# alexfrom0815/IR-BPP

Hardware: AMD Instinct MI355X
Metric: env steps/sec (placements/sec) across N parallel bins (higher is better)
Workload: dtype f64

## Files before the change

include/irbpp.h:

```cpp
#ifndef IRBPP_H
#define IRBPP_H

#include <stdint.h>

#ifdef __cplusplus
extern "C" {
#endif

typedef struct irbpp_env irbpp_env;

typedef enum {
    IRBPP_OK = 0,
    IRBPP_ERR_ARG = -1,
    IRBPP_ERR_HIP = -2,
    IRBPP_ERR_STATE = -3,
    IRBPP_ERR_DEVICE = -4,
    IRBPP_ERR_NOMEM = -5
} irbpp_status;

typedef struct {
    int32_t num_bins;
    int32_t n_rot;
    int32_t selected;
    int32_t buffer_size;
    double  resolution_a;
    double  resolution_h;
    double  resolution_z;
    double  bin[3];
    double  scale_z;
    int32_t traj_start;
    int32_t global_offset;
    int32_t global_bins;
    int32_t device;
    int32_t stability;
    int32_t tuning;
    int32_t item_stream;
} irbpp_config;

#define IRBPP_TUNE_NO_BLOCK_PATH  1
#define IRBPP_TUNE_WIDE_KERNEL    2
#define IRBPP_TUNE_NARROW_KERNEL  4
#define IRBPP_TUNE_NO_BOX_PATH    8
#define IRBPP_TUNE_NO_ITEM_ORDER 16
#define IRBPP_TUNE_TRACE_CPW64   32
#define IRBPP_TUNE_TRACE_CPW32   64
#define IRBPP_TUNE_TRACE_CPW16  128
#define IRBPP_TUNE_INLINE_POLYGON 256
#define IRBPP_TUNE_NO_HEAVY_FIRST 512
#define IRBPP_TUNE_FUSED_APPLY 2048
#define IRBPP_TUNE_SPLIT_APPLY 4096
#define IRBPP_TUNE_BLOCK_EMIT 8192
#define IRBPP_TUNE_WAVE_EMIT 16384
#define IRBPP_TUNE_GRAPH 32768
#define IRBPP_TUNE_WG512 65536
#define IRBPP_TUNE_NO_WG512 131072
#define IRBPP_TUNE_TRACE_REFILL 262144
#define IRBPP_TUNE_NO_MIXED_PATH 524288
#define IRBPP_TUNE_CHAIN 1048576
#define IRBPP_TUNE_WG128 2097152
#define IRBPP_TUNE_RECT 4194304
#define IRBPP_TUNE_NO_SPECIALISED 1024

typedef struct {
    double*  reward_dev;
    uint8_t* done_dev;
    int32_t* counter_dev;
    double*  ratio_dev;
    double*  ep_reward_dev;
    int32_t* ep_len_dev;
    uint8_t* stable_dev;
    int32_t* err_dev;
} irbpp_step_out;

const char* irbpp_status_string(int status);
int irbpp_version(void);
const char* irbpp_source_hash(void);

int irbpp_create(const irbpp_config* cfg, irbpp_env** out);
int irbpp_destroy(irbpp_env* env);

int irbpp_load_shapes(irbpp_env* env, int32_t n_shapes,
                      const double* extents, const double* volumes,
                      const int32_t* dims, const int64_t* offsets, int64_t pool_len,
                      const double* height_top, const double* height_bottom,
                      const double* mask_top, const double* mask_bottom);

int irbpp_load_sequences(irbpp_env* env, const int32_t* ids, int32_t n_traj, int32_t length);

int irbpp_obs_len(const irbpp_env* env, int32_t which);

int irbpp_reset(irbpp_env* env, float* obs_dev, void* stream);

int irbpp_reset_bins(irbpp_env* env, const int32_t* bins_dev, int32_t count, float* obs_dev, void* stream);

int irbpp_step(irbpp_env* env, const int32_t* actions_dev, float* obs_dev,
               const irbpp_step_out* out, void* stream);

int irbpp_step_cells(irbpp_env* env, const int32_t* cells_dev, float* obs_dev,
                     const irbpp_step_out* out, void* stream);

int irbpp_heuristic_step(irbpp_env* env, int32_t method, int32_t dir_idx, float* obs_dev,
                         const irbpp_step_out* out, void* stream);

int irbpp_get_action_candidates(irbpp_env* env, const int32_t* order_actions_dev,
                                float* loc_obs_dev, void* stream);

int irbpp_get_all_possible_observation(irbpp_env* env, float* loc_obs_dev, void* stream);

int irbpp_policy_minz(irbpp_env* env, const float* loc_obs_dev, int32_t obs_stride,
                      int32_t* actions_dev, void* stream);

int irbpp_set_auto_policy(irbpp_env* env, int32_t* actions_dev);

int irbpp_register_obs_buffer(irbpp_env* env, float* obs_dev);
int irbpp_unregister_obs_buffer(irbpp_env* env, float* obs_dev);
int irbpp_invalidate_obs_buffer(irbpp_env* env, float* obs_dev, void* stream);

int irbpp_stream_cursors(irbpp_env* env, int32_t* cursors_dev, int32_t set, void* stream);
int irbpp_stream_write(irbpp_env* env, const int32_t* ids_dev, const int32_t* first_dev, const int32_t* count_dev,
                       int32_t width, void* stream);

typedef struct irbpp_itemgen irbpp_itemgen;
int irbpp_itemgen_create(uint32_t seed, int32_t n_groups, const int32_t* group_offsets, const int32_t* members,
                         int32_t n_members, irbpp_itemgen** out);
int irbpp_itemgen_draw(irbpp_itemgen* gen, int32_t count, int32_t* out_host);
int irbpp_itemgen_destroy(irbpp_itemgen* gen);


int irbpp_possible_position(irbpp_env* env, const int32_t* item_ids_dev,
                            double* posz_dev, uint8_t* mask_dev, void* stream);

int irbpp_heuristic_action(irbpp_env* env, int32_t method, int32_t dir_idx, int32_t* out_dev, void* stream);

int irbpp_shot_item(const double* verts_dev, const int32_t* faces_dev, int32_t n_faces, int32_t fx, int32_t fy,
                    double resolution_h, double shift, double extent_z, double* top_dev, double* bottom_dev,
                    double* mask_top_dev, double* mask_bottom_dev, int32_t* scratch_dev, void* stream);

int irbpp_convex_hull_actions(irbpp_env* env, int32_t n_grids, const double* posz_valid_dev,
                              const uint8_t* mask_dev, uint32_t* vertex_rows_dev, void* stream);

int irbpp_get_heightmaps(irbpp_env* env, double* hm_dev, void* stream);
int irbpp_set_heightmaps(irbpp_env* env, const double* hm_dev, void* stream);

int irbpp_episode_totals(irbpp_env* env, double* out_dev, void* stream);

typedef struct {
    int64_t key;
    double  r;
    double  ratio;
    int32_t counter;
    int32_t reserved;
} irbpp_episode_entry;
typedef struct {
    irbpp_episode_entry* ring_dev;
    irbpp_episode_entry* snapshot_dev;
    int32_t* rows_dev;
    int32_t* state_dev;
    int32_t window;
    int32_t history;
} irbpp_episode_window;
int irbpp_set_episode_window(irbpp_env* env, const irbpp_episode_window* window);
int irbpp_episode_metrics(const irbpp_episode_window* parts, int32_t n_parts, int32_t first_step, int32_t n_steps,
                          double* out_dev, void* stream);

int irbpp_set_placement_log(irbpp_env* env, uint32_t* meta_dev, double* z_dev, int32_t capacity);

int irbpp_sumtree_find(const float* tree_dev, int32_t n_env, int32_t capacity, const float* values_dev, int32_t draws,
                       float* prob_dev, int64_t* data_idx_dev, int64_t* tree_idx_dev, void* stream);
int irbpp_sumtree_sample(const float* tree_dev, const int64_t* index_dev, int32_t n_env, int32_t capacity, int32_t draws,
                         int32_t n_step, uint64_t seed, int32_t max_tries, float* prob_dev, int64_t* data_idx_dev,
                         int64_t* tree_idx_dev, int32_t* failed_dev, void* stream);

int irbpp_sumtree_update(float* tree_dev, float* max_dev, int32_t n_env, int32_t capacity, const int64_t* tree_idx_dev,
                         const float* priority_dev, int32_t leaves, const uint8_t* env_mask_dev, void* stream);
typedef struct {
    const float* states_dev; const int64_t* actions_dev; const float* rewards_dev; const uint8_t* nonterminals_dev;
    const float* tree_dev; const int64_t* index_dev; const uint8_t* full_dev; const float* scaling_dev;
    int32_t n_env, capacity, obs_len, n_step;
} irbpp_replay_view;
int irbpp_replay_gather(const irbpp_replay_view* view, int32_t draws, float beta, const int64_t* data_idx_dev,
                        const float* prob_dev, float* state_dev, int64_t* action_dev, float* return_dev,
                        float* next_state_dev, float* nonterminal_dev, float* weight_dev, void* stream);
typedef struct {
    float* states_dev; int64_t* actions_dev; float* rewards_dev; uint8_t* nonterminals_dev; int32_t* timesteps_dev;
    float* tree_dev; float* max_dev; int64_t* index_dev; uint8_t* full_dev; int32_t* t_dev;
    int32_t n_env, capacity, obs_len;
} irbpp_replay_store;
int irbpp_replay_append(const irbpp_replay_store* store, const float* state_dev, int64_t state_stride, const void* action_dev,
                        int32_t action_bytes, const void* reward_dev, int32_t reward_bytes, const uint8_t* terminal_dev,
                        const uint8_t* valid_dev, void* stream);
int irbpp_masked_argmax(const float* q_dev, int32_t q_stride, const float* obs_dev, int32_t obs_stride, int32_t selected,
                        int32_t n_env, int64_t* action_dev, void* stream);

int irbpp_debug_phase_cycles(irbpp_env* env, int64_t* cycles_dev);

int irbpp_debug_kernel_info(const irbpp_env* env, int32_t* lds_bytes, const char** kernel_name);
int irbpp_overlap_path(const irbpp_env* env);
int irbpp_debug_kernel_timing(irbpp_env* env, int32_t capacity);
int irbpp_debug_kernel_timing_every(irbpp_env* env, int32_t every);
int irbpp_debug_kernel_times(irbpp_env* env, float* ms_host, int32_t max_count, int32_t* count);

int irbpp_device_error(irbpp_env* env, void* stream, int32_t* flags_out);

#define IRBPP_DEVERR_LEVEL_RANGE   1
#define IRBPP_DEVERR_TRACE_GUARD   2
#define IRBPP_DEVERR_BAD_ITEM      4
#define IRBPP_DEVERR_BAD_BIN       8
#define IRBPP_DEVERR_CAPACITY     16
#define IRBPP_DEVERR_BAD_ACTION   64
#define IRBPP_DEVERR_STREAM_DRY   32

#ifdef __cplusplus
}
#endif
// ... 2 lines not shown
```

irbpp_amd/_lib.py:

```python
from __future__ import annotations

import ctypes as C
import os

from .build import LIB_PATH

c_i32_p = C.POINTER(C.c_int32)
c_f64_p = C.POINTER(C.c_double)


class IrbppConfig(C.Structure):
    _fields_ = [
        ("num_bins", C.c_int32), ("n_rot", C.c_int32), ("selected", C.c_int32), ("buffer_size", C.c_int32),
        ("resolution_a", C.c_double), ("resolution_h", C.c_double), ("resolution_z", C.c_double),
        ("bin", C.c_double * 3), ("scale_z", C.c_double),
        ("traj_start", C.c_int32), ("global_offset", C.c_int32), ("global_bins", C.c_int32),
        ("device", C.c_int32), ("stability", C.c_int32), ("tuning", C.c_int32), ("item_stream", C.c_int32),
    ]


TUNE_NO_BLOCK_PATH, TUNE_WIDE_KERNEL, TUNE_NARROW_KERNEL, TUNE_NO_BOX_PATH, TUNE_NO_ITEM_ORDER = 1, 2, 4, 8, 16
TUNE_TRACE_CPW64, TUNE_TRACE_CPW32, TUNE_TRACE_CPW16, TUNE_INLINE_POLYGON, TUNE_NO_HEAVY_FIRST = 32, 64, 128, 256, 512
TUNE_NO_SPECIALISED, TUNE_FUSED_APPLY, TUNE_SPLIT_APPLY, TUNE_BLOCK_EMIT, TUNE_WAVE_EMIT = 1024, 2048, 4096, 8192, 16384
TUNE_GRAPH, TUNE_WG512, TUNE_NO_WG512, TUNE_TRACE_REFILL, TUNE_NO_MIXED_PATH = 32768, 65536, 131072, 262144, 524288
TUNE_CHAIN, TUNE_WG128, TUNE_RECT = 1048576, 2097152, 4194304


class IrbppReplayView(C.Structure):
    _fields_ = [("states_dev", C.c_void_p), ("actions_dev", C.c_void_p), ("rewards_dev", C.c_void_p),
                ("nonterminals_dev", C.c_void_p), ("tree_dev", C.c_void_p), ("index_dev", C.c_void_p),
                ("full_dev", C.c_void_p), ("scaling_dev", C.c_void_p),
                ("n_env", C.c_int32), ("capacity", C.c_int32), ("obs_len", C.c_int32), ("n_step", C.c_int32)]


class IrbppReplayStore(C.Structure):
    _fields_ = [("states_dev", C.c_void_p), ("actions_dev", C.c_void_p), ("rewards_dev", C.c_void_p),
                ("nonterminals_dev", C.c_void_p), ("timesteps_dev", C.c_void_p), ("tree_dev", C.c_void_p),
                ("max_dev", C.c_void_p), ("index_dev", C.c_void_p), ("full_dev", C.c_void_p), ("t_dev", C.c_void_p),
                ("n_env", C.c_int32), ("capacity", C.c_int32), ("obs_len", C.c_int32)]


class IrbppEpisodeWindow(C.Structure):
    _fields_ = [("ring_dev", C.c_void_p), ("snapshot_dev", C.c_void_p), ("rows_dev", C.c_void_p), ("state_dev", C.c_void_p),
                ("window", C.c_int32), ("history", C.c_int32)]


class IrbppStepOut(C.Structure):
    _fields_ = [("reward_dev", C.c_void_p), ("done_dev", C.c_void_p), ("counter_dev", C.c_void_p),
                ("ratio_dev", C.c_void_p), ("ep_reward_dev", C.c_void_p), ("ep_len_dev", C.c_void_p),
                ("stable_dev", C.c_void_p), ("err_dev", C.c_void_p)]


SIGNATURES = {
    "irbpp_status_string": (C.c_char_p, [C.c_int]),
    "irbpp_version": (C.c_int, []),
    "irbpp_source_hash": (C.c_char_p, []),
    "irbpp_overlap_path": (C.c_int, [C.c_void_p]),
    "irbpp_create": (C.c_int, [C.POINTER(IrbppConfig), C.POINTER(C.c_void_p)]),
    "irbpp_destroy": (C.c_int, [C.c_void_p]),
    "irbpp_load_shapes": (C.c_int, [C.c_void_p, C.c_int32, c_f64_p, c_f64_p, c_i32_p, C.POINTER(C.c_int64),
                                    C.c_int64, c_f64_p, c_f64_p, c_f64_p, c_f64_p]),
    "irbpp_load_sequences": (C.c_int, [C.c_void_p, c_i32_p, C.c_int32, C.c_int32]),
    "irbpp_obs_len": (C.c_int, [C.c_void_p, C.c_int32]),
    "irbpp_reset": (C.c_int, [C.c_void_p, C.c_void_p, C.c_void_p]),
    "irbpp_reset_bins": (C.c_int, [C.c_void_p, C.c_void_p, C.c_int32, C.c_void_p, C.c_void_p]),
    "irbpp_step": (C.c_int, [C.c_void_p, C.c_void_p, C.c_void_p, C.POINTER(IrbppStepOut), C.c_void_p]),
    "irbpp_step_cells": (C.c_int, [C.c_void_p, C.c_void_p, C.c_void_p, C.POINTER(IrbppStepOut), C.c_void_p]),
    "irbpp_heuristic_step": (C.c_int, [C.c_void_p, C.c_int32, C.c_int32, C.c_void_p, C.POINTER(IrbppStepOut), C.c_void_p]),
    "irbpp_get_action_candidates": (C.c_int, [C.c_void_p, C.c_void_p, C.c_void_p, C.c_void_p]),
    "irbpp_get_all_possible_observation": (C.c_int, [C.c_void_p, C.c_void_p, C.c_void_p]),
    "irbpp_policy_minz": (C.c_int, [C.c_void_p, C.c_void_p, C.c_int32, C.c_void_p, C.c_void_p]),
    "irbpp_set_auto_policy": (C.c_int, [C.c_void_p, C.c_void_p]),
    "irbpp_register_obs_buffer": (C.c_int, [C.c_void_p, C.c_void_p]),
    "irbpp_unregister_obs_buffer": (C.c_int, [C.c_void_p, C.c_void_p]),
    "irbpp_invalidate_obs_buffer": (C.c_int, [C.c_void_p, C.c_void_p, C.c_void_p]),
    "irbpp_stream_cursors": (C.c_int, [C.c_void_p, C.c_void_p, C.c_int32, C.c_void_p]),
    "irbpp_stream_write": (C.c_int, [C.c_void_p, C.c_void_p, C.c_void_p, C.c_void_p, C.c_int32, C.c_void_p]),
    "irbpp_itemgen_create": (C.c_int, [C.c_uint32, C.c_int32, c_i32_p, c_i32_p, C.c_int32, C.POINTER(C.c_void_p)]),
    "irbpp_itemgen_draw": (C.c_int, [C.c_void_p, C.c_int32, c_i32_p]),
    "irbpp_itemgen_destroy": (C.c_int, [C.c_void_p]),
    "irbpp_possible_position": (C.c_int, [C.c_void_p, C.c_void_p, C.c_void_p, C.c_void_p, C.c_void_p]),
    "irbpp_heuristic_action": (C.c_int, [C.c_void_p, C.c_int32, C.c_int32, C.c_void_p, C.c_void_p]),
    "irbpp_shot_item": (C.c_int, [C.c_void_p, C.c_void_p, C.c_int32, C.c_int32, C.c_int32, C.c_double, C.c_double,
                                  C.c_double, C.c_void_p, C.c_void_p, C.c_void_p, C.c_void_p, C.c_void_p, C.c_void_p]),
    "irbpp_convex_hull_actions": (C.c_int, [C.c_void_p, C.c_int32, C.c_void_p, C.c_void_p, C.c_void_p, C.c_void_p]),
    "irbpp_get_heightmaps": (C.c_int, [C.c_void_p, C.c_void_p, C.c_void_p]),
    "irbpp_set_heightmaps": (C.c_int, [C.c_void_p, C.c_void_p, C.c_void_p]),
    "irbpp_episode_totals": (C.c_int, [C.c_void_p, C.c_void_p, C.c_void_p]),
    "irbpp_set_placement_log": (C.c_int, [C.c_void_p, C.c_void_p, C.c_void_p, C.c_int32]),
    "irbpp_set_episode_window": (C.c_int, [C.c_void_p, C.POINTER(IrbppEpisodeWindow)]),
    "irbpp_episode_metrics": (C.c_int, [C.POINTER(IrbppEpisodeWindow), C.c_int32, C.c_int32, C.c_int32, C.c_void_p, C.c_void_p]),
    "irbpp_sumtree_sample": (C.c_int, [C.c_void_p, C.c_void_p, C.c_int32, C.c_int32, C.c_int32, C.c_int32, C.c_uint64, C.c_int32,
                                       C.c_void_p, C.c_void_p, C.c_void_p, C.c_void_p, C.c_void_p]),
    "irbpp_sumtree_find": (C.c_int, [C.c_void_p, C.c_int32, C.c_int32, C.c_void_p, C.c_int32, C.c_void_p, C.c_void_p,
                                     C.c_void_p, C.c_void_p]),
    "irbpp_sumtree_update": (C.c_int, [C.c_void_p, C.c_void_p, C.c_int32, C.c_int32, C.c_void_p, C.c_void_p, C.c_int32,
                                       C.c_void_p, C.c_void_p]),
    "irbpp_replay_gather": (C.c_int, [C.POINTER(IrbppReplayView), C.c_int32, C.c_float, C.c_void_p, C.c_void_p, C.c_void_p,
                                      C.c_void_p, C.c_void_p, C.c_void_p, C.c_void_p, C.c_void_p, C.c_void_p]),
    "irbpp_replay_append": (C.c_int, [C.POINTER(IrbppReplayStore), C.c_void_p, C.c_int64, C.c_void_p, C.c_int32, C.c_void_p,
                                      C.c_int32, C.c_void_p, C.c_void_p, C.c_void_p]),
    "irbpp_masked_argmax": (C.c_int, [C.c_void_p, C.c_int32, C.c_void_p, C.c_int32, C.c_int32, C.c_int32, C.c_void_p,
                                      C.c_void_p]),
    "irbpp_debug_phase_cycles": (C.c_int, [C.c_void_p, C.c_void_p]),
    "irbpp_debug_kernel_info": (C.c_int, [C.c_void_p, C.POINTER(C.c_int32), C.POINTER(C.c_char_p)]),
    "irbpp_debug_kernel_timing": (C.c_int, [C.c_void_p, C.c_int32]),
    "irbpp_debug_kernel_timing_every": (C.c_int, [C.c_void_p, C.c_int32]),
    "irbpp_debug_kernel_times": (C.c_int, [C.c_void_p, C.POINTER(C.c_float), C.c_int32, C.POINTER(C.c_int32)]),
    "irbpp_device_error": (C.c_int, [C.c_void_p, C.c_void_p, c_i32_p]),
}

_lib = None


def load(path: str = "") -> C.CDLL:
    global _lib
    if _lib is not None:
        return _lib
    explicit = bool(path) or bool(os.environ.get("IRBPP_LIBRARY"))
    path = path or os.environ.get("IRBPP_LIBRARY", "") or LIB_PATH
    if not os.path.exists(path):
        raise RuntimeError(
            f"{path} not found: build it with `python -c 'import __graft_entry__ as g; g.build()'` "
            "(hipcc --offload-arch=gfx950). irbpp_amd has no CPU fallback.")
    import torch
    lib = C.CDLL(path)
    for name, (res, args) in SIGNATURES.items():
        fn = getattr(lib, name)
        fn.restype = res
        fn.argtypes = args
    if not explicit and not os.environ.get("IRBPP_ALLOW_STALE_LIBRARY"):
        from . import build
        have = lib.irbpp_source_hash().decode()
        try:
            want = build.source_hash()
        except OSError:
            want = have
        if have != want:
            raise RuntimeError(
                f"{path} was built from sources {have}, the sources in {build.CSRC} hash to {want}: rebuild with "
                "`python -c 'import __graft_entry__ as g; g.build()'` (IRBPP_ALLOW_STALE_LIBRARY=1 overrides)")
    _lib = lib
    return lib


class IrbppError(RuntimeError):
    pass


DEVERR_BITS = {1: "LEVEL_RANGE", 2: "TRACE_GUARD", 4: "BAD_ITEM", 8: "BAD_BIN", 16: "CAPACITY", 32: "STREAM_DRY", 64: "BAD_ACTION"}


def deverr_names(flags: int) -> str:
    return "|".join(name for bit, name in DEVERR_BITS.items() if flags & bit) or "0"


def check(status: int, what: str = "") -> None:
    if status != 0:
        msg = load().irbpp_status_string(status).decode()
        raise IrbppError(f"{what}: {msg} (status {status})")
```

irbpp_amd/build.py:

```python
from __future__ import annotations

import os
import shutil
import subprocess

PKG_DIR = os.path.dirname(os.path.abspath(__file__))
CSRC = os.path.join(PKG_DIR, "csrc")
LIB_PATH = os.path.join(PKG_DIR, "libirbpp_hip.so")
SOURCES = ["irbpp_capi.hip", "irbpp_kernels.hip", "irbpp_wide.hip", "irbpp_replay.hip", "irbpp_metrics.hip", "irbpp_metrics.h", "irbpp_device.h", "contours_device.h", "irbpp_itemgen.h",
           os.path.join("..", "..", "include", "irbpp.h")]
HIPCC_FLAGS = ["--offload-arch=gfx950", "-O3", "-std=c++17", "-ffp-contract=off", "-fno-honor-nans",
               "-shared", "-fPIC", "-Wno-unused-value"]


def source_hash() -> str:
    import hashlib
    h = hashlib.sha256(" ".join(HIPCC_FLAGS).encode())
    for name in sorted(SOURCES):
        with open(os.path.join(CSRC, name), "rb") as f:
            h.update(f.read())
    return h.hexdigest()[:16]


def _hipcc() -> str:
    for cand in (shutil.which("hipcc"), "/opt/rocm/bin/hipcc"):
        if cand and os.path.exists(cand):
            return cand
    raise RuntimeError("hipcc not found: the HIP library cannot be built on this machine")


def built_hash(path: str = LIB_PATH) -> str:
    try:
        with open(path, "rb") as f:
            blob = f.read()
    except OSError:
        return ""
    i = blob.find(b"irbpp-source-hash:")
    return blob[i + 18:i + 34].decode("ascii", "replace") if i >= 0 else ""


def needs_build(path: str = LIB_PATH) -> bool:
    return built_hash(path) != source_hash()


def build(force: bool = False, verbose: bool = False) -> str:
    out = LIB_PATH
    if not force and not needs_build(out):
        return out
    cmd = [_hipcc()] + HIPCC_FLAGS + [f'-DIRBPP_SOURCE_HASH="{source_hash()}"', os.path.join(CSRC, "irbpp_capi.hip"), "-o", out]
    if verbose:
        print(" ".join(cmd))
    res = subprocess.run(cmd, capture_output=True, text=True)
    if res.returncode != 0:
        raise RuntimeError("hipcc failed:\n" + res.stdout + res.stderr)
    from . import asmcheck
    try:
        chk = asmcheck.check_library(out)
    except (RuntimeError, OSError, subprocess.CalledProcessError) as e:
        if verbose:
            print(f"asmcheck skipped: {e}")
        return out
    if verbose:
        print(f"asmcheck: {chk['scalar_loads']} scalar loads in {chk['functions']} kernels, {len(chk['problems'])} hazards")
    if chk["problems"]:
        os.replace(out, out + ".rejected")
        raise RuntimeError("scalar-load hazard in the built library (kept as " + out + ".rejected):\n" + "\n".join(chk["problems"]))
    return out
```

irbpp_amd/csrc/irbpp_capi.hip:

```cpp
#include <hip/hip_runtime.h>
#include <math.h>
#include <stdint.h>
#include <stdio.h>
#include <stdlib.h>
#include <string.h>

#include <new>
#include <utility>
#include <vector>

#include "../../include/irbpp.h"
#include "irbpp_device.h"
#include "irbpp_kernels.hip"
#include "irbpp_wide.hip"
#include "irbpp_replay.hip"
#include "irbpp_metrics.hip"
#include "irbpp_itemgen.h"

using namespace irbpp;

struct irbpp_env {
    irbpp_config cfg;
    Params P;
    Tables T;
    State S;
    bool shapes_loaded = false, seq_loaded = false, was_reset = false;
    bool item_order = false;
    long long* phase_cycles = nullptr;
    int32_t* auto_actions = nullptr;
    int heavy_turn = 0;
    int32_t* err_mirror = nullptr;
    std::vector<std::pair<const float*, int32_t*>> obs_buffers;
    std::vector<hipEvent_t> timing;
    size_t timing_next = 0, timing_used = 0;
    int timing_every = 1, timing_phase = 0;
    std::vector<void*> allocs;
    char kernel_names[256] = {0};
    struct GraphEntry { std::vector<uint8_t> key; hipGraphExec_t exec; hipGraph_t graph; uint64_t used; };
    std::vector<GraphEntry> graphs;
    hipStream_t cap_stream = nullptr;
    uint64_t graph_clock = 0, graph_replays = 0;
    int obs_epoch = 0;
    irbpp_episode_window window{};
    int32_t* heur_cells = nullptr;
    bool grids_current = false;
};

#define HIP_TRY(expr)                                   \
    do {                                                \
        hipError_t _e = (expr);                         \
        if (_e != hipSuccess) return IRBPP_ERR_HIP;     \
    } while (0)

namespace {

template <typename T>
int dev_alloc(irbpp_env* env, T** out, size_t count) {
    void* p = nullptr;
    if (hipMalloc(&p, count * sizeof(T) > 0 ? count * sizeof(T) : sizeof(T)) != hipSuccess) return IRBPP_ERR_NOMEM;
    if (hipMemset(p, 0, count * sizeof(T)) != hipSuccess) { hipFree(p); return IRBPP_ERR_HIP; }
    env->allocs.push_back(p);
    *out = (T*)p;
    return IRBPP_OK;
}

template <typename T>
int dev_upload(irbpp_env* env, const T** out, const T* host, size_t count) {
    T* p = nullptr;
    int rc = dev_alloc(env, &p, count);
    if (rc != IRBPP_OK) return rc;
    if (count && hipMemcpy(p, host, count * sizeof(T), hipMemcpyHostToDevice) != hipSuccess) return IRBPP_ERR_HIP;
    *out = p;
    return IRBPP_OK;
}

inline double round6_host(double x) { return nearbyint(x * 1e6) / 1e6; }
constexpr int TRACE_SMALL_GRID = 8192;
constexpr int TRACE_CPW16_BINS = 0;
constexpr int TRACE_CPW32_BINS = 1024;
void layout_lds_host(Params& P) {
    int pad = 0;
#ifdef IRBPP_ABLATE
    if (const char* e = getenv("IRBPP_LDS_PAD")) pad = atoi(e);
#endif
    irbpp::layout_lds(P, pad);
}

int raise_lds_limits() {
    const void* kernels[] = {(const void*)irbpp_env_kernel_wide, (const void*)irbpp_env_kernel, (const void*)irbpp_env_kernel_box,
                             (const void*)irbpp_env_kernel_box8, (const void*)irbpp_env_kernel_generic,
                             (const void*)irbpp_env_kernel_generic8, (const void*)irbpp_env_kernel_mixed8, (const void*)irbpp_hull_kernel,
                             (const void*)irbpp_env_kernel_chain, (const void*)irbpp_wide_kernel,
#if !defined(IRBPP_NO_SPEC)
                             (const void*)irbpp_env_kernel_s1, (const void*)irbpp_env_kernel_s2, (const void*)irbpp_env_kernel_s3,
                             (const void*)irbpp_env_kernel_s4, (const void*)irbpp_env_kernel_s5, (const void*)irbpp_emit_kernel_s5,
                             (const void*)irbpp_env_kernel_chain_s1, (const void*)wg128::irbpp_env_kernel_s1_w128,
                             (const void*)irbpp_emit_kernel_s1, (const void*)irbpp_emit_kernel_s2,
                             (const void*)irbpp_emit_kernel_s3, (const void*)irbpp_emit_kernel_s4,
                             (const void*)irbpp_emit_wave_kernel_s1, (const void*)irbpp_emit_wave_kernel_s2, (const void*)irbpp_emit_wave_kernel_s5,
                             (const void*)wg512::irbpp_env_kernel_s4_w512, (const void*)wg512::irbpp_env_kernel_s4_w512c,
#endif
                             (const void*)wg512::irbpp_env_kernel_generic_w512,
                             (const void*)irbpp_emit_wave_kernel,
                             (const void*)irbpp_emit_kernel, (const void*)irbpp_heuristic_kernel};
    for (const void* k : kernels)
        if (hipFuncSetAttribute(k, hipFuncAttributeMaxDynamicSharedMemorySize, 160 * 1024) != hipSuccess) return IRBPP_ERR_HIP;
    return IRBPP_OK;
}

}

static int chain_extra_lds(const Params& P) {
    int npad = 64;
    while (npad < P.S) npad <<= 1;
    return align16(10 * npad > 1024 ? 10 * npad : 1024);
}
static bool all_block(const Params& P) { return P.block_b > 0 && P.block_rots == (1 << P.R) - 1; }
static bool lattice_or_box(const Params& P) { return all_block(P) || P.box != 0; }
static bool lattice_images(const Params& P) { return P.block_b > 0 || P.box != 0; }

static int trace_grid_cap(int N) {
    const int small = 4 * N < TRACE_SMALL_GRID ? 4 * N : TRACE_SMALL_GRID;
    return N > small ? N : small;
}

extern "C" {

const char* irbpp_status_string(int status) {
    switch (status) {
        case IRBPP_OK: return "ok";
        case IRBPP_ERR_ARG: return "bad argument or unsupported configuration";
        case IRBPP_ERR_HIP: return "HIP runtime error";
        case IRBPP_ERR_STATE: return "call out of order (load shapes and sequences, reset, then step)";
        case IRBPP_ERR_DEVICE: return "device-side error word set";
        case IRBPP_ERR_NOMEM: return "out of device memory";
        default: return "unknown status";
    }
}

int irbpp_version(void) { return 600; }

#ifndef IRBPP_SOURCE_HASH
#define IRBPP_SOURCE_HASH "unstamped"
#endif
const char* irbpp_source_hash(void) { static const char stamp[] = "irbpp-source-hash:" IRBPP_SOURCE_HASH; return stamp + 18; }

int irbpp_create(const irbpp_config* cfg, irbpp_env** out) {
    if (!cfg || !out) return IRBPP_ERR_ARG;
    if (cfg->num_bins > MAX_BINS) return IRBPP_ERR_ARG;
    if (cfg->num_bins < 1 || cfg->n_rot < 1 || cfg->n_rot > 8 || cfg->selected < 1 || cfg->selected > 1024 ||
        cfg->buffer_size < 1 || cfg->buffer_size > 16)
        return IRBPP_ERR_ARG;
    if (!(cfg->resolution_a > 0) || !(cfg->resolution_h > 0) || !(cfg->resolution_z > 0)) return IRBPP_ERR_ARG;
    irbpp_env* env = new (std::nothrow) irbpp_env();
    if (!env) return IRBPP_ERR_NOMEM;
    env->cfg = *cfg;
    memset(&env->T, 0, sizeof(Tables));
    memset(&env->S, 0, sizeof(State));
    Params& P = env->P;
    memset(&P, 0, sizeof(Params));
    P.N = cfg->num_bins;
    P.R = cfg->n_rot;
    P.S = cfg->selected;
    P.K = cfg->buffer_size;
    P.res_a = cfg->resolution_a;
    P.res_h = cfg->resolution_h;
    P.res_z = cfg->resolution_z;
    P.inv_res_z = 1.0 / cfg->resolution_z;
    for (int k = 0; k < 32; ++k) P.txs[k] = round6_host((double)k * cfg->resolution_a);
    P.bin_x = cfg->bin[0];
    P.bin_y = cfg->bin[1];
    P.bin_z = cfg->bin[2];
    P.bin_vol = cfg->bin[0] * cfg->bin[1] * cfg->bin[2];
    P.scale_z = cfg->scale_z;
    P.ibin_z = round6_host(cfg->bin[2] * cfg->scale_z);
    P.step = (int)(cfg->resolution_a / cfg->resolution_h);
    if ((double)P.step != cfg->resolution_a / cfg->resolution_h || P.step < 1) { delete env; return IRBPP_ERR_ARG; }
    P.Hx = (int)ceil(cfg->bin[0] / cfg->resolution_h);
    P.Hy = (int)ceil(cfg->bin[1] / cfg->resolution_h);
    P.Ax = (int)ceil(cfg->bin[0] / cfg->resolution_a);
    P.Ay = (int)ceil(cfg->bin[1] / cfg->resolution_a);
    P.Hc = P.Hx * P.Hy;
    P.AC = P.Ax * P.Ay;
    if (P.Ax > 32 || P.Ay > 32 || P.Ax < 1 || P.Ay < 1 || P.Hc > 128 * 128) { delete env; return IRBPP_ERR_ARG; }
    const double levels = floor(cfg->bin[2] / cfg->resolution_z + 1e-9);
    if (!(levels <= (double)MAX_LEVELS)) { delete env; return IRBPP_ERR_ARG; }
    const bool deep = levels > (double)TUNED_MAX_LEVELS;
    P.wide = (P.Ax > 16 || P.Ay > 16 || deep) ? 1 : 0;
    P.vrow = P.wide ? WIDE_VROW : 16;
    if (P.wide && (P.Hc > 64 * 64 || cfg->stability != 0)) { delete env; return IRBPP_ERR_ARG; }
    if (P.Hx != P.Ax * P.step || P.Hy != P.Ay * P.step) { delete env; return IRBPP_ERR_ARG; }
    P.traj_start = cfg->traj_start;
    P.goff = cfg->global_offset;
    P.gbins = cfg->global_bins > 0 ? cfg->global_bins : cfg->num_bins;
    P.obs_len1 = 5 * P.S + 9 + P.Hc;
    P.obs_len0 = P.K > 1 ? P.K + P.Hc : P.obs_len1;
#ifdef IRBPP_ABLATE
    if (const char* rep = getenv("IRBPP_DEBUG_REPEAT")) P.dbg_repeat = atoi(rep);
#endif
    P.split = 1;
    P.stability = cfg->stability < 0 ? 0 : (cfg->stability > 2 ? 2 : cfg->stability);
    P.rect = (cfg->tuning & IRBPP_TUNE_RECT) ? 1 : 0;
    P.wimg = P.R * (deep ? (((int)levels + 33 + 31) & ~31) : 64);
    P.seg_cap = P.wide ? 64 : 2 * ((P.N + NXCD - 1) / NXCD) * P.R * P.AC;
    P.round_cap = P.wide ? 16 : (P.N / NXCD + 64) * 16;
    layout_lds_host(P);
    if (P.lds_bytes_full > 160 * 1024 || (P.wide && wide_layout(P).bytes > 160 * 1024)) { delete env; return IRBPP_ERR_ARG; }

    if (hipSetDevice(cfg->device) != hipSuccess) { delete env; return IRBPP_ERR_HIP; }
    if (raise_lds_limits() != IRBPP_OK) { delete env; return IRBPP_ERR_HIP; }
    State& S = env->S;
    const size_t N = (size_t)P.N;
    int rc = IRBPP_OK;
#define ALLOC(field, count) if (rc == IRBPP_OK) rc = dev_alloc(env, &S.field, (count))
    ALLOC(hm, N * P.Hc);
    ALLOC(queue, N * P.K);
    ALLOC(cand, N * P.S);
    ALLOC(bs, N);
    ALLOC(totals, N * 4);
    ALLOC(order, N);
    ALLOC(err, 1);
    ALLOC(w_posz, N * P.R * P.AC);
    ALLOC(w_valid, N * P.R * P.vrow);
    ALLOC(w_vmask, N * P.R * 16);
    ALLOC(w_meta, N * WMETA);
    ALLOC(w_img, P.wide ? 16 : N * P.wimg * 16);
    ALLOC(w_imgrot, P.wide ? 16 : N * P.wimg);
    ALLOC(w_cand, (size_t)NXCD * P.seg_cap);
    ALLOC(w_big, P.wide ? N * wide_scratch_bytes(P) : (size_t)trace_grid_cap(P.N) * TRACE_WAVE_BYTES);
    ALLOC(w_total, NXCD * XCD_STRIDE);
    ALLOC(w_nround, NXCD * XCD_STRIDE);
    ALLOC(w_round, (size_t)NXCD * P.round_cap * ROUND_BYTES);
    P.heavy_cap = P.N >= 64 ? P.N / 8 : 0;
    P.heavy_thr = (P.S * 3) / 5;
    ALLOC(w_heavy, 2 * (size_t)(XCD_STRIDE + P.heavy_cap));
#undef ALLOC
    if (rc == IRBPP_OK) rc = dev_alloc(env, &env->heur_cells, N * 3);
    if (rc != IRBPP_OK) { irbpp_destroy(env); return rc; }
    {
        std::vector<int32_t> ident(N);
        for (size_t i = 0; i < N; ++i) ident[i] = (int32_t)i;
        if (hipMemcpy(S.order, ident.data(), N * sizeof(int32_t), hipMemcpyHostToDevice) != hipSuccess) { irbpp_destroy(env); return IRBPP_ERR_HIP; }
    }
    *out = env;
    return IRBPP_OK;
}

int irbpp_destroy(irbpp_env* env) {
    if (!env) return IRBPP_OK;
// ... 17 lines not shown
    const Params& P = env->P;
    HIP_TRY(hipSetDevice(env->cfg.device));
    const int R = P.R;
    std::vector<ShapeRot> sr((size_t)n_shapes * R);
    std::vector<Cell> bcell, tcell, blkcell;
    std::vector<GCell> gcell;
    for (int64_t i = 0; i < (int64_t)n_shapes * R; ++i) {
        const int64_t fx = dims[i * 2], fy = dims[i * 2 + 1];
        if (fx < 1 || fy < 1 || fx > 4096 || fy > 4096 || offsets[i] < 0 || offsets[i] + fx * fy > pool_len) return IRBPP_ERR_ARG;
    }
    int block_b = 0, block_rots = 0;
    if (!(env->cfg.tuning & IRBPP_TUNE_NO_BLOCK_PATH) && !P.wide) {
        int best_count = 0;
        for (int b = 8; b >= 2; --b) {
            if (b % P.step != 0 || (P.Hx - b) % P.step != 0 || (P.Hy - b) % P.step != 0) continue;
            int mask = 0;
            for (int r = 0; r < R; ++r) {
                bool ok = true;
                for (int64_t k = 0; k < n_shapes && ok; ++k) {
                    const int64_t i = k * R + r;
                    const int fx = dims[i * 2], fy = dims[i * 2 + 1];
                    if (fx % b != 0 || fy % b != 0) { ok = false; break; }
                    for (int ti = 0; ti < fx / b && ok; ++ti)
                        for (int tj = 0; tj < fy / b && ok; ++tj) {
                            const int64_t e0 = offsets[i] + (int64_t)(ti * b) * fy + tj * b;
                            for (int u = 0; u < b && ok; ++u)
                                for (int v = 0; v < b && ok; ++v) {
                                    const int64_t e = offsets[i] + (int64_t)(ti * b + u) * fy + tj * b + v;
                                    if (mask_bottom[e] != mask_bottom[e0] ||
                                        (mask_bottom[e0] != 0.0 && height_bottom[e] != height_bottom[e0]))
                                        ok = false;
                                }
                        }
                }
                if (ok) mask |= 1 << r;
            }
            const int count = __builtin_popcount((unsigned)mask);
            if (count > best_count) { best_count = count; block_b = b; block_rots = mask; }
            if (count == R) break;
        }
        if (block_rots != (1 << R) - 1 && (2 * best_count < R || (env->cfg.tuning & IRBPP_TUNE_NO_MIXED_PATH))) { block_b = 0; block_rots = 0; }
    }
    const bool mixed = block_b > 0 && block_rots != (1 << R) - 1;
    bool box = block_b == 0 && !(env->cfg.tuning & IRBPP_TUNE_NO_BOX_PATH) && !P.wide;
    for (int64_t i = 0; i < (int64_t)n_shapes * R && box; ++i) {
        const int fx = dims[i * 2], fy = dims[i * 2 + 1];
        const double* mb = mask_bottom + offsets[i];
        const double* hb = height_bottom + offsets[i];
        int bx = 0, by = 0;
        while (bx < fx && mb[(int64_t)bx * fy] != 0.0) ++bx;
        while (by < fy && mb[by] != 0.0) ++by;
        if (bx == 0 || by == 0) { box = false; break; }
        for (int ci = 0; ci < fx && box; ++ci)
            for (int cj = 0; cj < fy && box; ++cj) {
                const bool in = ci < bx && cj < by;
                if ((mb[(int64_t)ci * fy + cj] != 0.0) != in || (in && hb[(int64_t)ci * fy + cj] != hb[0])) box = false;
            }
    }
    const int mb_h = block_b ? (P.Hx - block_b) / P.step + 1 : 0, mb_w = block_b ? (P.Hy - block_b) / P.step + 1 : 0;
    for (int k = 0; k < n_shapes; ++k) {
        for (int r = 0; r < R; ++r) {
            const size_t i = (size_t)k * R + r;
            ShapeRot& s = sr[i];
            memset(&s, 0, sizeof(s));
            s.ext_x = extents[i * 3 + 0];
            s.ext_y = extents[i * 3 + 1];
            s.ext_z = extents[i * 3 + 2];
            const double bx = round6_host(s.ext_x), by = round6_host(s.ext_y);
            s.ext_z_r = round6_host(s.ext_z);
            s.fx = (int32_t)ceil(bx / P.res_h);
            s.fy = (int32_t)ceil(by / P.res_h);
            s.ax = (int32_t)ceil(bx / P.res_a);
            s.ay = (int32_t)ceil(by / P.res_a);
            const int64_t off = offsets[i];
            if (s.fx != dims[i * 2] || s.fy != dims[i * 2 + 1]) return IRBPP_ERR_ARG;
            if (s.fx < 1 || s.fy < 1 || s.fx > s.ax * P.step || s.fy > s.ay * P.step) return IRBPP_ERR_ARG;
            if (off < 0 || off + (int64_t)s.fx * s.fy > pool_len) return IRBPP_ERR_ARG;
            s.ob = (int32_t)bcell.size();
            s.ot = (int32_t)tcell.size();
            for (int ci = 0; ci < s.fx; ++ci) {
                for (int cj = 0; cj < s.fy; ++cj) {
                    const int64_t e = off + (int64_t)ci * s.fy + cj;
                    const double mt = mask_top[e], mb = mask_bottom[e];
                    if ((mt != 0.0 && mt != 1.0) || (mb != 0.0 && mb != 1.0)) return IRBPP_ERR_ARG;
                    const int32_t ij = ci | (cj << 16);
                    if (mb != 0.0) bcell.push_back(Cell{height_bottom[e], ij, ci * s.fy + cj});
                    else s.has_out = 1;
                    if (mt != 0.0) tcell.push_back(Cell{height_top[e], ij, ci * s.fy + cj});
                }
            }
            s.nb = (int32_t)bcell.size() - s.ob;
            s.nt = (int32_t)tcell.size() - s.ot;
            {
                double mass = 0.0, mx = 0.0, my = 0.0;
                for (int ci = 0; ci < s.fx; ++ci)
                    for (int cj = 0; cj < s.fy; ++cj) {
                        const int64_t e = off + (int64_t)ci * s.fy + cj;
                        if (mask_top[e] != 0.0 && mask_bottom[e] != 0.0) {
                            const double w = height_top[e] - height_bottom[e] > 0.0 ? height_top[e] - height_bottom[e] : 0.0;
                            mass += w; mx += w * (ci + 0.5); my += w * (cj + 0.5);
                        }
                    }
                s.com_x = mass > 0.0 ? mx / mass : 0.5 * s.fx;
                s.com_y = mass > 0.0 ? my / mass : 0.5 * s.fy;
            }
            s.oblk = (int32_t)blkcell.size();
            if (block_b && ((block_rots >> r) & 1))
                for (int ti = 0; ti < s.fx / block_b; ++ti)
                    for (int tj = 0; tj < s.fy / block_b; ++tj) {
                        const int64_t e0 = off + (int64_t)(ti * block_b) * s.fy + tj * block_b;
                        if (mask_bottom[e0] != 0.0)
                            blkcell.push_back(Cell{height_bottom[e0], (ti * block_b / P.step) * mb_w + tj * block_b / P.step, 0});
                    }
            s.nblk = (int32_t)blkcell.size() - s.oblk;
            if (!box && (!block_b || mixed))
                for (int e = 0; e < s.nb; ++e) {
                    const Cell& c = bcell[s.ob + e];
                    const int ci = c.ij & 0xFFFF, cj = c.ij >> 16;
                    const int off = ((ci % P.step) * P.step + cj % P.step) * P.AC + (ci / P.step) * P.Ay + cj / P.step;
                    gcell.push_back(GCell{c.v, off * 8, 0});
                }
            if (box) {
                while (s.bx < s.fx && mask_bottom[off + (int64_t)s.bx * s.fy] != 0.0) ++s.bx;
                while (s.by < s.fy && mask_bottom[off + s.by] != 0.0) ++s.by;
                s.bc = height_bottom[off];
            }
            if (s.nb == 0 && !s.has_out) return IRBPP_ERR_ARG;
        }
    }
    if (bcell.empty()) bcell.push_back(Cell{0.0, 0, 0});
    if (tcell.empty()) tcell.push_back(Cell{0.0, 0, 0});
    if (blkcell.empty()) blkcell.push_back(Cell{0.0, 0, 0});
    if (gcell.empty()) gcell.push_back(GCell{0.0, 0, 0});
    for (int i = 0; i < 8; ++i) gcell.push_back(GCell{0.0, 0, 0});
    Tables& T = env->T;
    int rc = dev_upload(env, &T.sr, sr.data(), sr.size());
    if (rc == IRBPP_OK) rc = dev_upload(env, &T.bcell, (const Cell*)bcell.data(), bcell.size());
    if (rc == IRBPP_OK) rc = dev_upload(env, &T.tcell, (const Cell*)tcell.data(), tcell.size());
    if (rc == IRBPP_OK) rc = dev_upload(env, &T.blkcell, (const Cell*)blkcell.data(), blkcell.size());
    if (rc == IRBPP_OK) rc = dev_upload(env, &T.gcell, (const GCell*)gcell.data(), gcell.size());
    if (rc == IRBPP_OK) rc = dev_upload(env, &T.volume, volumes, (size_t)n_shapes);
    if (rc != IRBPP_OK) return rc;
    T.n_shapes = n_shapes;
    if (block_b || box) {
        env->P.block_b = block_b;
        env->P.block_rots = block_rots;
        env->P.mb_h = mb_h;
        env->P.mb_w = mb_w;
        env->P.box = box ? 1 : 0;
        layout_lds_host(env->P);
        if (env->P.lds_bytes_full > 160 * 1024) return IRBPP_ERR_ARG;
        if (raise_lds_limits() != IRBPP_OK) return IRBPP_ERR_HIP;
    }
    env->item_order = (!block_b || mixed) && !box && gcell.size() * sizeof(GCell) > (size_t)8 << 20 && env->P.N % NXCD == 0 &&
                      env->P.N >= 64 * NXCD && env->P.K == 1 && !(env->cfg.tuning & IRBPP_TUNE_NO_ITEM_ORDER);
    env->shapes_loaded = true;
    return IRBPP_OK;
}

int irbpp_load_sequences(irbpp_env* env, const int32_t* ids, int32_t n_traj, int32_t length) {
    if (!env || !ids || n_traj < 1 || length < 1) return IRBPP_ERR_ARG;
    if (env->seq_loaded) return IRBPP_ERR_STATE;
    HIP_TRY(hipSetDevice(env->cfg.device));
    int rc = dev_upload(env, &env->T.seq, ids, (size_t)n_traj * length);
    if (rc != IRBPP_OK) return rc;
    env->T.n_traj = n_traj;
    env->T.seq_len = length;
    env->T.stream = env->cfg.item_stream ? 1 : 0;
    env->seq_loaded = true;
    return IRBPP_OK;
}

int irbpp_stream_cursors(irbpp_env* env, int32_t* cursors_dev, int32_t set, void* stream) {
    if (!env || !cursors_dev) return IRBPP_ERR_ARG;
    if (!env->cfg.item_stream || !env->seq_loaded) return IRBPP_ERR_STATE;
    hipLaunchKernelGGL(irbpp_stream_cursor_kernel, dim3((env->P.N + 255) / 256), dim3(256), 0, (hipStream_t)stream, env->S.bs,
                       cursors_dev, env->P.N, set);
    return hipGetLastError() == hipSuccess ? IRBPP_OK : IRBPP_ERR_HIP;
}

int irbpp_stream_write(irbpp_env* env, const int32_t* ids_dev, const int32_t* first_dev, const int32_t* count_dev, int32_t width,
                       void* stream) {
    if (!env || !ids_dev || !first_dev || !count_dev || width < 0) return IRBPP_ERR_ARG;
    if (!env->cfg.item_stream || !env->seq_loaded) return IRBPP_ERR_STATE;
    if (width > env->T.seq_len) return IRBPP_ERR_ARG;
    if (width == 0) return IRBPP_OK;
    env->err_mirror = nullptr;
    const long long n = (long long)env->T.n_traj * width;
    hipLaunchKernelGGL(irbpp_stream_write_kernel, dim3((unsigned)((n + 255) / 256)), dim3(256), 0, (hipStream_t)stream,
                       const_cast<int32_t*>(env->T.seq), env->T.n_traj, env->T.seq_len, ids_dev, first_dev, count_dev, width);
    return hipGetLastError() == hipSuccess ? IRBPP_OK : IRBPP_ERR_HIP;
}

int irbpp_obs_len(const irbpp_env* env, int32_t which) {
    if (!env) return IRBPP_ERR_ARG;
    return which == 0 ? env->P.obs_len0 : env->P.obs_len1;
}

typedef void (*env_kernel_fn)(const Params, const Tables, const State, const StepIO, const int);
struct EnvKernel { env_kernel_fn fn; const char* name; int threads = 256; };
static int pick_spec(const irbpp_env* env) {
#if defined(IRBPP_NO_SPEC) || defined(IRBPP_ABLATE)
    return 0;
#else
    if (env->cfg.tuning & (IRBPP_TUNE_NO_SPECIALISED | IRBPP_TUNE_WIDE_KERNEL | IRBPP_TUNE_NARROW_KERNEL)) return 0;
    static const Params spec[N_SPECS] = {Params{}, spec_params(SPEC_KEYS[1]), spec_params(SPEC_KEYS[2]), spec_params(SPEC_KEYS[3]),
                                         spec_params(SPEC_KEYS[4]), spec_params(SPEC_KEYS[5])};
    static_assert(N_SPECS == 6, "one table entry and one kernel per SPEC_KEYS row");
    for (int i = 1; i < N_SPECS; ++i)
        if (spec_matches(env->P, spec[i])) return i;
    return 0;
#endif
}

static bool split_apply(const irbpp_env* env, int n) {
    if (env->P.stability != 0 || (env->cfg.tuning & IRBPP_TUNE_FUSED_APPLY)) return false;
    if (env->cfg.tuning & IRBPP_TUNE_SPLIT_APPLY) return true;
    if (env->P.K > 1) return true;
    const int per_cu = (160 * 1024) / (env->P.lds_bytes > 0 ? env->P.lds_bytes : 1);
    if (per_cu < 8) return false;
    const bool lists = !lattice_or_box(env->P);
    return n >= (lists ? 4 : 2) * 256 * 8;
}

static EnvKernel pick_env_kernel(const irbpp_env* env) {
    const Params& P = env->P;
    const int t = env->cfg.tuning;
    const bool lds_allows_8 = 8 * P.lds_bytes <= 160 * 1024;
    const bool generic = P.block_b == 0 && !P.box;
    const bool mixed = P.block_b > 0 && !all_block(P);
#if !defined(IRBPP_NO_SPEC) && !defined(IRBPP_ABLATE)
    if (generic && (t & IRBPP_TUNE_NARROW_KERNEL) && (t & IRBPP_TUNE_WG512) && spec_matches(P, spec_params(SPEC_KEYS[4])))
        return {wg512::irbpp_env_kernel_s4_w512c, "irbpp_env_kernel_s4_w512c", 512};
#endif
    const bool wg512 = generic && !(t & (IRBPP_TUNE_NO_WG512 | IRBPP_TUNE_WIDE_KERNEL | IRBPP_TUNE_NARROW_KERNEL)) &&
                       ((t & IRBPP_TUNE_WG512) || 5 * P.lds_bytes > 160 * 1024);
#if !defined(IRBPP_NO_SPEC) && !defined(IRBPP_ABLATE)
    if (wg512 && pick_spec(env) == 4)
        return P.N >= 4096 ? EnvKernel{wg512::irbpp_env_kernel_s4_w512c, "irbpp_env_kernel_s4_w512c", 512}
                           : EnvKernel{wg512::irbpp_env_kernel_s4_w512, "irbpp_env_kernel_s4_w512", 512};
#endif
    if (wg512 && (pick_spec(env) == 0 || (t & IRBPP_TUNE_WG512)))
        return {wg512::irbpp_env_kernel_generic_w512, "irbpp_env_kernel_generic_w512", 512};
#if !defined(IRBPP_NO_SPEC) && !defined(IRBPP_ABLATE)
    if ((t & IRBPP_TUNE_WG128) && pick_spec(env) == 1)
        return {wg128::irbpp_env_kernel_s1_w128, "irbpp_env_kernel_s1_w128", 128};
    switch (pick_spec(env)) {
        case 1: return {irbpp_env_kernel_s1, "irbpp_env_kernel_s1"};
        case 2: return {irbpp_env_kernel_s2, "irbpp_env_kernel_s2"};
        case 3: return {irbpp_env_kernel_s3, "irbpp_env_kernel_s3"};
        case 4: return {irbpp_env_kernel_s4, "irbpp_env_kernel_s4"};
        case 5: return {irbpp_env_kernel_s5, "irbpp_env_kernel_s5"};
        default: break;
    }
#endif
    if (mixed) return (t & IRBPP_TUNE_WIDE_KERNEL) ? EnvKernel{irbpp_env_kernel_wide, "irbpp_env_kernel_wide"} : EnvKernel{irbpp_env_kernel_mixed8, "irbpp_env_kernel_mixed8"};
    if (P.block_b > 0) {
        if ((t & IRBPP_TUNE_WIDE_KERNEL) || 6 * P.lds_bytes > 150 * 1024) return {irbpp_env_kernel_wide, "irbpp_env_kernel_wide"};
        return {irbpp_env_kernel, "irbpp_env_kernel"};
    }
    if (P.box) {
        if (t & IRBPP_TUNE_WIDE_KERNEL) return {irbpp_env_kernel_box, "irbpp_env_kernel_box"};
        if ((t & IRBPP_TUNE_NARROW_KERNEL) || lds_allows_8) return {irbpp_env_kernel_box8, "irbpp_env_kernel_box8"};
        return {irbpp_env_kernel_box, "irbpp_env_kernel_box"};
    }
    if (t & IRBPP_TUNE_WIDE_KERNEL) return {irbpp_env_kernel_generic, "irbpp_env_kernel_generic"};
    if ((t & IRBPP_TUNE_NARROW_KERNEL) || lds_allows_8) return {irbpp_env_kernel_generic8, "irbpp_env_kernel_generic8"};
    return {irbpp_env_kernel_generic, "irbpp_env_kernel_generic"};
}

static int pick_trace_cpw(const irbpp_env* env, int n) {
    const int t = env->cfg.tuning;
    if (t & IRBPP_TUNE_TRACE_CPW64) return 64;
    if (t & IRBPP_TUNE_TRACE_CPW32) return 32;
    if (t & IRBPP_TUNE_TRACE_CPW16) return 16;
    if (t & IRBPP_TUNE_TRACE_REFILL) return TRACE_REFILL_BATCH;
    return n <= TRACE_CPW16_BINS ? 16 : (n <= TRACE_CPW32_BINS ? 32 : 64);
}

static bool chain_launch(const irbpp_env* env, int n) {
    const int t = env->cfg.tuning;
    (void)n;
    if (!(t & IRBPP_TUNE_CHAIN) || env->P.stability != 0) return false;
    if (t & (IRBPP_TUNE_TRACE_CPW64 | IRBPP_TUNE_TRACE_CPW32 | IRBPP_TUNE_TRACE_CPW16 | IRBPP_TUNE_TRACE_REFILL | IRBPP_TUNE_INLINE_POLYGON |
             IRBPP_TUNE_BLOCK_EMIT | IRBPP_TUNE_WAVE_EMIT | IRBPP_TUNE_SPLIT_APPLY | IRBPP_TUNE_GRAPH | IRBPP_TUNE_WG512 | IRBPP_TUNE_NARROW_KERNEL))
        return false;
    if (env->P.lds_bytes > 32 * 1024) return false;
    return true;
}

static void launch_apply(irbpp_env* env, StepIO io, int mode, hipStream_t st, int n, int key) {
    if (key == KEY_HEUR && io.heur_method == 4) {
        StepIO sel = io;
        sel.heur_out = env->heur_cells;
        hipLaunchKernelGGL(irbpp_heuristic_kernel, dim3(env->P.N), dim3(256), env->P.lds_bytes_full, st, env->P, env->T, env->S, sel);
        io.actions = env->heur_cells;
        key = KEY_CELLS;
    }
    const bool wg = env->P.K > 1 && n < 2048;
    env_kernel_fn fn = wg ? irbpp_apply_wg_kernel : irbpp_apply_kernel;
    if (key == KEY_CELLS) fn = wg ? irbpp_apply_cells_wg_kernel : irbpp_apply_cells_kernel;
    if (key == KEY_HEUR) fn = wg ? irbpp_apply_heur_wg_kernel : irbpp_apply_heur_kernel;
    hipLaunchKernelGGL(fn, wg ? dim3(n) : dim3((n + 3) / 4), dim3(256), 0, st, env->P, env->T, env->S, io, mode);
}

static void launch_group(irbpp_env* env, StepIO io, int mode, hipStream_t st, int first, int n, int key = KEY_CAND) {
    io.block_off = first;
    io.n_slots = n;
    io.auto_action = env->auto_actions;
    io.use_order = 0;
    if (mode == MODE_STEP && env->item_order && first == 0 && n == env->P.N) {
        hipLaunchKernelGGL(irbpp_item_order_kernel, dim3(1), dim3(1024), 0, st, env->T, env->S, n);
        io.use_order = 1;
    }
    io.obs_rows = nullptr;
    const bool observes = mode == MODE_CANDS || ((mode == MODE_RESET || mode == MODE_STEP) && env->P.K == 1);
    for (auto& rb : env->obs_buffers)
        if (rb.first == io.obs) {
            if (observes && !(mode == MODE_RESET && io.bin_list != nullptr)) io.obs_rows = rb.second;
            else hipMemsetAsync(rb.second, 0xFF, (size_t)env->P.N * sizeof(int32_t), st);
        }
    if (env->P.wide) {
        int wmode = mode;
        if (mode == MODE_STEP) {
            launch_apply(env, io, mode, st, n, key);
            if (env->P.K > 1) return;
            wmode = MODE_OBSERVE;
        }
        hipLaunchKernelGGL(irbpp_wide_kernel, dim3(n), dim3(256), wide_layout(env->P).bytes, st, env->P, env->T, env->S, io, wmode);
        return;
    }
    const bool chain = observes && mode != MODE_POSSIBLE && chain_launch(env, n);
    const bool split = env->P.split && observes && !chain;
    const bool heavy_first = split && env->P.heavy_cap > 0 && !lattice_images(env->P) && io.bin_list == nullptr &&
                             !(env->cfg.tuning & IRBPP_TUNE_NO_HEAVY_FIRST);
    io.heavy_turn = heavy_first ? env->heavy_turn : -1;
    if (heavy_first) env->heavy_turn ^= 1;
    int env_mode = mode;
    if (chain && !(mode == MODE_STEP && env->P.K > 1)) {
        const bool s1 = pick_spec(env) == 1;
        hipLaunchKernelGGL(s1 ? irbpp_env_kernel_chain_s1 : irbpp_env_kernel_chain, dim3(n), dim3(256), env->P.lds_bytes + chain_extra_lds(env->P), st,
                           env->P, env->T, env->S, io, mode);
        return;
    }
    if (mode == MODE_STEP && (key != KEY_CAND || split_apply(env, n))) {
        launch_apply(env, io, mode, st, n, key);
        env_mode = MODE_OBSERVE;
    }
    if (!(env_mode == MODE_OBSERVE && env->P.K > 1)) {
        const EnvKernel ek = pick_env_kernel(env);
        hipLaunchKernelGGL(ek.fn, dim3(n), dim3(ek.threads), env->P.lds_bytes, st, env->P, env->T, env->S, io, env_mode);
    }
    if (split) {
        const int cpw = pick_trace_cpw(env, n), pgrid = 2 * n;
        const int tune = env->cfg.tuning;
        const bool inline_polygon = (tune & IRBPP_TUNE_INLINE_POLYGON) != 0;
        Params Pt = env->P;
        if (inline_polygon) Pt.round_cap = 0;
        int tgrid = cpw > 64 ? (n * 64 + cpw - 1) / cpw : n * (64 / cpw);
        if (tgrid > trace_grid_cap(env->P.N)) tgrid = trace_grid_cap(env->P.N);
        auto trace_fn = cpw > 64 ? irbpp_trace_kernel_refill : cpw == 64 ? irbpp_trace_kernel : (cpw == 32 ? irbpp_trace_kernel_c32 : irbpp_trace_kernel_c16);
        hipLaunchKernelGGL(trace_fn, dim3(tgrid), dim3(64), 0, st, Pt, env->S, env->phase_cycles);
#ifdef IRBPP_AB_POLY_ACCOUNT
        if (!inline_polygon) hipLaunchKernelGGL(irbpp_polygon_kernel, dim3(pgrid), dim3(64), 0, st, env->P, env->S, env->phase_cycles);
#else
        if (!inline_polygon) hipLaunchKernelGGL(irbpp_polygon_kernel, dim3(pgrid), dim3(64), 0, st, env->P, env->S);
#endif
        const bool wave_emit = lattice_images(env->P) && !heavy_first && !(env->cfg.tuning & IRBPP_TUNE_BLOCK_EMIT) &&
                               (n >= 2048 || (env->cfg.tuning & IRBPP_TUNE_WAVE_EMIT));
        env_kernel_fn emit_fn = wave_emit ? irbpp_emit_wave_kernel : irbpp_emit_kernel;
#if !defined(IRBPP_NO_SPEC) && !defined(IRBPP_ABLATE)
        switch (pick_spec(env)) {
            case 1: emit_fn = wave_emit ? irbpp_emit_wave_kernel_s1 : irbpp_emit_kernel_s1; break;
            case 2: emit_fn = wave_emit ? irbpp_emit_wave_kernel_s2 : irbpp_emit_kernel_s2; break;
            case 3: emit_fn = irbpp_emit_kernel_s3; break;
            case 4: emit_fn = irbpp_emit_kernel_s4; break;
            case 5: emit_fn = wave_emit ? irbpp_emit_wave_kernel_s5 : irbpp_emit_kernel_s5; break;
            default: break;
        }
#endif
        const int egrid = wave_emit ? (n + 3) / 4 : n + (heavy_first ? env->P.heavy_cap : 0);
        hipLaunchKernelGGL(emit_fn, dim3(egrid), dim3(256), env->P.emit_lds_bytes, st, env->P, env->T, env->S, io, mode);
    }
}

constexpr int GRAPH_CACHE = 24;
static void drop_graphs(irbpp_env* env) {
    for (auto& g : env->graphs) { if (g.exec) hipGraphExecDestroy(g.exec); if (g.graph) hipGraphDestroy(g.graph); }
    env->graphs.clear();
}
static bool graph_wanted(const irbpp_env* env, int) { return (env->cfg.tuning & IRBPP_TUNE_GRAPH) != 0; }

static int launch_env(irbpp_env* env, StepIO io, int mode, void* stream, int grid = 0, int key = KEY_CAND) {
    if (grid <= 0) grid = env->P.N;
    if (key == KEY_HEUR && grid != env->P.N) return IRBPP_ERR_ARG;
    io.phase_cycles = env->phase_cycles;
    hipStream_t st = (hipStream_t)stream;
    size_t pairs = env->timing.size() / 2;
    const size_t slot = env->timing_next;
    if (pairs && (env->timing_phase++ % env->timing_every) != 0) pairs = 0;
    if (pairs) hipEventRecord(env->timing[2 * slot], st);
    bool launched = false;
    if (graph_wanted(env, grid) && (mode == MODE_STEP || mode == MODE_CANDS) && key == KEY_CAND) {
        hipStreamCaptureStatus cs = hipStreamCaptureStatusNone;
        if (hipStreamIsCapturing(st, &cs) != hipSuccess) cs = hipStreamCaptureStatusActive;
        if (cs == hipStreamCaptureStatusNone) {
            struct Key { StepIO io; int mode, grid, heavy_turn, obs_epoch; int32_t* auto_actions; } k;
            memset(&k, 0, sizeof k);
            k.io = io; k.mode = mode; k.grid = grid; k.heavy_turn = env->heavy_turn; k.obs_epoch = env->obs_epoch;
            k.auto_actions = env->auto_actions;
            const uint8_t* kb = (const uint8_t*)&k;
            irbpp_env::GraphEntry* hit = nullptr;
            for (auto& g : env->graphs)
                if (g.key.size() == sizeof k && memcmp(g.key.data(), kb, sizeof k) == 0) { hit = &g; break; }
            if (hit == nullptr) {
                if (env->graphs.size() >= (size_t)GRAPH_CACHE) {
                    size_t lru = 0;
                    for (size_t i = 1; i < env->graphs.size(); ++i) if (env->graphs[i].used < env->graphs[lru].used) lru = i;
                    if (env->graphs[lru].exec) hipGraphExecDestroy(env->graphs[lru].exec);
                    if (env->graphs[lru].graph) hipGraphDestroy(env->graphs[lru].graph);
                    env->graphs.erase(env->graphs.begin() + lru);
                }
                env->graphs.push_back({std::vector<uint8_t>(kb, kb + sizeof k), nullptr, nullptr, ++env->graph_clock});
            } else {
                hit->used = ++env->graph_clock;
                const int turn_before = env->heavy_turn;
                if (hit->exec == nullptr) {
                    if (env->cap_stream == nullptr && hipStreamCreateWithFlags(&env->cap_stream, hipStreamNonBlocking) != hipSuccess)
                        env->cap_stream = nullptr;
                    if (env->cap_stream != nullptr && hipStreamBeginCapture(env->cap_stream, hipStreamCaptureModeRelaxed) == hipSuccess) {
                        launch_group(env, io, mode, env->cap_stream, 0, grid);
                        hipGraph_t graph = nullptr;
                        if (hipStreamEndCapture(env->cap_stream, &graph) == hipSuccess && graph != nullptr &&
                            hipGraphInstantiate(&hit->exec, graph, nullptr, nullptr, 0) == hipSuccess) {
                            hit->graph = graph;
                        } else {
                            if (graph) hipGraphDestroy(graph);
                            hit->exec = nullptr;
                        }
                        env->heavy_turn = turn_before;
                        (void)hipGetLastError();
                    }
                }
                if (hit->exec != nullptr && hipGraphLaunch(hit->exec, st) == hipSuccess) {
                    launched = true;
                    ++env->graph_replays;
                    const bool observes = mode == MODE_CANDS || (mode == MODE_STEP && env->P.K == 1);
                    const bool heavy_first = env->P.split && observes && env->P.heavy_cap > 0 && !lattice_images(env->P) &&
                                             io.bin_list == nullptr && !(env->cfg.tuning & IRBPP_TUNE_NO_HEAVY_FIRST);
                    if (heavy_first) env->heavy_turn ^= 1;
                }
            }
        }
    }
    if (!launched) launch_group(env, io, mode, st, 0, grid, key);
    if (pairs) {
        hipEventRecord(env->timing[2 * slot + 1], st);
        env->timing_next = (slot + 1) % pairs;
        if (env->timing_used < pairs) env->timing_used++;
    }
    if (hipGetLastError() != hipSuccess) return IRBPP_ERR_HIP;
    if (io.bin_list == nullptr && mode != MODE_POSSIBLE)
        env->grids_current = mode == MODE_CANDS || env->P.K == 1;
    return IRBPP_OK;
}

int irbpp_reset(irbpp_env* env, float* obs_dev, void* stream) {
    if (!env || !obs_dev) return IRBPP_ERR_ARG;
    if (!env->shapes_loaded || !env->seq_loaded) return IRBPP_ERR_STATE;
    StepIO io;
    memset(&io, 0, sizeof(io));
    io.obs = obs_dev;
    io.obs_stride = env->P.obs_len0;
    io.reset_next = env->was_reset ? 1 : 0;
    env->err_mirror = nullptr;
    const int rc = launch_env(env, io, MODE_RESET, stream);
    if (rc == IRBPP_OK) env->was_reset = true;
    return rc;
}

int irbpp_reset_bins(irbpp_env* env, const int32_t* bins_dev, int32_t count, float* obs_dev, void* stream) {
    if (!env || count < 0 || count > env->P.N || (count > 0 && (!bins_dev || !obs_dev))) return IRBPP_ERR_ARG;
    if (!env->was_reset) return IRBPP_ERR_STATE;
    if (count == 0) return IRBPP_OK;
    StepIO io;
    memset(&io, 0, sizeof(io));
    io.obs = obs_dev;
    io.obs_stride = env->P.obs_len0;
    io.bin_list = bins_dev;
    env->err_mirror = nullptr;
    return launch_env(env, io, MODE_RESET, stream, count);
}

static int step_common(irbpp_env* env, const int32_t* actions_dev, float* obs_dev, const irbpp_step_out* out, void* stream, int key,
                       int method = 0, int dir_idx = 0) {
    const bool windowed = env->window.window > 0;
    if (windowed && (!out || !out->done_dev || !out->ep_reward_dev || !out->ratio_dev || !out->counter_dev)) return IRBPP_ERR_ARG;
    StepIO io;
    memset(&io, 0, sizeof(io));
    io.actions = actions_dev;
    io.heur_method = method;
    io.heur_dir = dir_idx;
    io.obs = obs_dev;
    io.obs_stride = env->P.obs_len0;
    if (out) {
        io.reward = out->reward_dev;
        io.done = out->done_dev;
        io.counter = out->counter_dev;
        io.ratio = out->ratio_dev;
        io.ep_reward = out->ep_reward_dev;
        io.ep_len = out->ep_len_dev;
        io.stable = out->stable_dev;
        io.err_out = out->err_dev;
        if (out->err_dev != env->err_mirror) {
            if (out->err_dev != nullptr)
                HIP_TRY(hipMemcpyAsync(out->err_dev, env->S.err, sizeof(int32_t), hipMemcpyDeviceToDevice, (hipStream_t)stream));
            env->err_mirror = out->err_dev;
        }
    } else {
        env->err_mirror = nullptr;
    }
    const int rc = launch_env(env, io, MODE_STEP, stream, 0, key);
    if (rc != IRBPP_OK || !windowed) return rc;
    const irbpp_episode_window& w = env->window;
    hipLaunchKernelGGL(irbpp_window_update_kernel, dim3(1), dim3(WINDOW_UPDATE_THREADS), 0, (hipStream_t)stream, out->done_dev,
                       out->ep_reward_dev, out->ratio_dev, out->counter_dev, env->P.N, env->cfg.global_offset, w.ring_dev,
                       w.snapshot_dev, w.rows_dev, w.state_dev, w.window, w.history);
    return hipGetLastError() == hipSuccess ? IRBPP_OK : IRBPP_ERR_HIP;
}

int irbpp_step(irbpp_env* env, const int32_t* actions_dev, float* obs_dev, const irbpp_step_out* out, void* stream) {
    if (!env || !actions_dev || !obs_dev) return IRBPP_ERR_ARG;
    if (!env->was_reset) return IRBPP_ERR_STATE;
    return step_common(env, actions_dev, obs_dev, out, stream, KEY_CAND);
}

static bool applies_in_transition(const irbpp_env* env) {
    return env->P.stability != 0 || (env->cfg.tuning & IRBPP_TUNE_FUSED_APPLY) || chain_launch(env, env->P.N);
}

int irbpp_step_cells(irbpp_env* env, const int32_t* cells_dev, float* obs_dev, const irbpp_step_out* out, void* stream) {
    if (!env || !cells_dev || !obs_dev || applies_in_transition(env)) return IRBPP_ERR_ARG;
    if (!env->was_reset) return IRBPP_ERR_STATE;
    return step_common(env, cells_dev, obs_dev, out, stream, KEY_CELLS);
}

int irbpp_heuristic_step(irbpp_env* env, int32_t method, int32_t dir_idx, float* obs_dev, const irbpp_step_out* out, void* stream) {
    if (!env || !obs_dev || method < 1 || method > 4 || dir_idx < 0 || dir_idx > 3 || applies_in_transition(env)) return IRBPP_ERR_ARG;
    if (method == 4 && env->P.wide) return IRBPP_ERR_ARG;
    if (!env->was_reset || !env->grids_current) return IRBPP_ERR_STATE;
    return step_common(env, nullptr, obs_dev, out, stream, KEY_HEUR, method, dir_idx);
}

int irbpp_get_action_candidates(irbpp_env* env, const int32_t* order_actions_dev, float* loc_obs_dev, void* stream) {
    if (!env || !order_actions_dev || !loc_obs_dev) return IRBPP_ERR_ARG;
    if (!env->was_reset) return IRBPP_ERR_STATE;
    if (env->P.K < 2) return IRBPP_ERR_ARG;
    StepIO io;
    memset(&io, 0, sizeof(io));
    io.actions = order_actions_dev;
    io.obs = loc_obs_dev;
    io.obs_stride = env->P.obs_len1;
    io.err_out = env->err_mirror;
    return launch_env(env, io, MODE_CANDS, stream);
}

int irbpp_get_all_possible_observation(irbpp_env* env, float* loc_obs_dev, void* stream) {
    if (!env || !loc_obs_dev) return IRBPP_ERR_ARG;
    if (!env->was_reset) return IRBPP_ERR_STATE;
    if (env->P.K < 2) return IRBPP_ERR_ARG;
    for (int j = 0; j < env->P.K; ++j) {
        StepIO io;
        memset(&io, 0, sizeof(io));
        io.fixed_slot = j + 1;
        io.obs = loc_obs_dev + (size_t)j * env->P.obs_len1;
        io.obs_stride = env->P.K * env->P.obs_len1;
        io.err_out = env->err_mirror;
        const int rc = launch_env(env, io, MODE_CANDS, stream);
        if (rc != IRBPP_OK) return rc;
    }
    return IRBPP_OK;
}

int irbpp_policy_minz(irbpp_env* env, const float* loc_obs_dev, int32_t obs_stride, int32_t* actions_dev, void* stream) {
    if (!env || !loc_obs_dev || !actions_dev || obs_stride < 5 * env->P.S) return IRBPP_ERR_ARG;
    const int waves_per_block = 4;
    const int grid = (env->P.N + waves_per_block - 1) / waves_per_block;
    hipLaunchKernelGGL(irbpp_policy_minz_kernel, dim3(grid), dim3(256), 0, (hipStream_t)stream, loc_obs_dev,
                       obs_stride, env->P.S, env->P.N, actions_dev);
    return hipGetLastError() == hipSuccess ? IRBPP_OK : IRBPP_ERR_HIP;
}

int irbpp_set_auto_policy(irbpp_env* env, int32_t* actions_dev) {
    if (!env) return IRBPP_ERR_ARG;
    env->auto_actions = actions_dev;
    return IRBPP_OK;
}

int irbpp_register_obs_buffer(irbpp_env* env, float* obs_dev) {
    if (!env || !obs_dev) return IRBPP_ERR_ARG;
    HIP_TRY(hipSetDevice(env->cfg.device));
    env->obs_epoch++;
    for (auto& rb : env->obs_buffers)
        if (rb.first == obs_dev) {
            HIP_TRY(hipMemset(rb.second, 0xFF, (size_t)env->P.N * sizeof(int32_t)));
            return IRBPP_OK;
        }
    int32_t* rows = nullptr;
    for (auto& rb : env->obs_buffers)
        if (rb.first == nullptr && rows == nullptr) { rows = rb.second; rb.first = obs_dev; }
    if (rows == nullptr) {
        if (env->obs_buffers.size() >= 8) return IRBPP_ERR_ARG;
        int rc = dev_alloc(env, &rows, (size_t)env->P.N);
        if (rc != IRBPP_OK) return rc;
        env->obs_buffers.emplace_back(obs_dev, rows);
    }
    HIP_TRY(hipMemset(rows, 0xFF, (size_t)env->P.N * sizeof(int32_t)));
    return IRBPP_OK;
}

int irbpp_unregister_obs_buffer(irbpp_env* env, float* obs_dev) {
    if (!env || !obs_dev) return IRBPP_ERR_ARG;
    env->obs_epoch++;
    for (auto& rb : env->obs_buffers)
        if (rb.first == obs_dev) { rb.first = nullptr; return IRBPP_OK; }
    return IRBPP_ERR_ARG;
}

int irbpp_invalidate_obs_buffer(irbpp_env* env, float* obs_dev, void* stream) {
    if (!env) return IRBPP_ERR_ARG;
    bool found = obs_dev == nullptr;
    for (auto& rb : env->obs_buffers)
        if (rb.first != nullptr && (obs_dev == nullptr || rb.first == obs_dev)) {
            HIP_TRY(hipMemsetAsync(rb.second, 0xFF, (size_t)env->P.N * sizeof(int32_t), (hipStream_t)stream));
            found = true;
        }
    return found ? IRBPP_OK : IRBPP_ERR_ARG;
}

int irbpp_possible_position(irbpp_env* env, const int32_t* item_ids_dev, double* posz_dev, uint8_t* mask_dev, void* stream) {
    if (!env || !item_ids_dev || !posz_dev || !mask_dev || env->P.wide) return IRBPP_ERR_ARG;
    if (!env->shapes_loaded) return IRBPP_ERR_STATE;
    StepIO io;
    memset(&io, 0, sizeof(io));
    io.actions = item_ids_dev;
    io.posz_out = posz_dev;
    io.mask_out = mask_dev;
    return launch_env(env, io, MODE_POSSIBLE, stream);
}

int irbpp_heuristic_action(irbpp_env* env, int32_t method, int32_t dir_idx, int32_t* out_dev, void* stream) {
    if (!env || !out_dev || method < 1 || method > 4 || dir_idx < 0 || dir_idx > 3 || env->P.wide) return IRBPP_ERR_ARG;
    if (!env->was_reset) return IRBPP_ERR_STATE;
    StepIO io;
    memset(&io, 0, sizeof(io));
    io.heur_out = out_dev;
    io.heur_method = method;
    io.heur_dir = dir_idx;
    hipLaunchKernelGGL(irbpp_heuristic_kernel, dim3(env->P.N), dim3(256), env->P.lds_bytes_full, (hipStream_t)stream, env->P,
                       env->T, env->S, io);
    return hipGetLastError() == hipSuccess ? IRBPP_OK : IRBPP_ERR_HIP;
}

int irbpp_shot_item(const double* verts_dev, const int32_t* faces_dev, int32_t n_faces, int32_t fx, int32_t fy,
                    double resolution_h, double shift, double extent_z, double* top_dev, double* bottom_dev,
                    double* mask_top_dev, double* mask_bottom_dev, int32_t* scratch_dev, void* stream) {
    if (!verts_dev || !faces_dev || n_faces < 1 || fx < 1 || fy < 1 || !top_dev || !bottom_dev || !mask_top_dev ||
        !mask_bottom_dev || !scratch_dev)
        return IRBPP_ERR_ARG;
    HIP_TRY(hipMemsetAsync(scratch_dev, 0, sizeof(int32_t), (hipStream_t)stream));
    const int n = fx * fy, grid = (n + 255) / 256;
    hipLaunchKernelGGL(irbpp_shot_item_kernel, dim3(grid), dim3(256), 0, (hipStream_t)stream, verts_dev, faces_dev,
                       n_faces, fx, fy, resolution_h, shift, top_dev, bottom_dev, mask_top_dev, mask_bottom_dev,
                       scratch_dev);
    hipLaunchKernelGGL(irbpp_shot_item_fallback_kernel, dim3(grid), dim3(256), 0, (hipStream_t)stream, n, extent_z,
                       top_dev, bottom_dev, mask_top_dev, mask_bottom_dev, scratch_dev);
    return hipGetLastError() == hipSuccess ? IRBPP_OK : IRBPP_ERR_HIP;
}

int irbpp_convex_hull_actions(irbpp_env* env, int32_t n_grids, const double* posz_valid_dev, const uint8_t* mask_dev,
                              uint32_t* vertex_rows_dev, void* stream) {
    if (!env || n_grids < 1 || !posz_valid_dev || !mask_dev || !vertex_rows_dev || env->P.wide) return IRBPP_ERR_ARG;
    hipLaunchKernelGGL(irbpp_hull_kernel, dim3(n_grids), dim3(256), env->P.lds_bytes, (hipStream_t)stream, env->P,
                       env->S, posz_valid_dev, mask_dev, vertex_rows_dev);
    return hipGetLastError() == hipSuccess ? IRBPP_OK : IRBPP_ERR_HIP;
}

int irbpp_get_heightmaps(irbpp_env* env, double* hm_dev, void* stream) {
    if (!env || !hm_dev) return IRBPP_ERR_ARG;
    HIP_TRY(hipMemcpyAsync(hm_dev, env->S.hm, (size_t)env->P.N * env->P.Hc * sizeof(double), hipMemcpyDeviceToDevice,
                           (hipStream_t)stream));
    return IRBPP_OK;
}

int irbpp_set_heightmaps(irbpp_env* env, const double* hm_dev, void* stream) {
    if (!env || !hm_dev) return IRBPP_ERR_ARG;
    HIP_TRY(hipMemcpyAsync(env->S.hm, hm_dev, (size_t)env->P.N * env->P.Hc * sizeof(double), hipMemcpyDeviceToDevice,
                           (hipStream_t)stream));
    HIP_TRY(hipMemsetAsync(env->S.w_valid, 0, (size_t)env->P.N * env->P.R * env->P.vrow * sizeof(uint32_t), (hipStream_t)stream));
    env->grids_current = false;
    return IRBPP_OK;
}

int irbpp_episode_totals(irbpp_env* env, double* out_dev, void* stream) {
    if (!env || !out_dev) return IRBPP_ERR_ARG;
    hipLaunchKernelGGL(irbpp_totals_kernel, dim3(1), dim3(256), 0, (hipStream_t)stream, env->S.totals, env->P.N, out_dev);
    return hipGetLastError() == hipSuccess ? IRBPP_OK : IRBPP_ERR_HIP;
}

int irbpp_set_placement_log(irbpp_env* env, uint32_t* meta_dev, double* z_dev, int32_t capacity) {
    if (!env || capacity < 0 || ((meta_dev == nullptr) != (z_dev == nullptr))) return IRBPP_ERR_ARG;
    drop_graphs(env);
    env->S.log_meta = meta_dev;
    env->S.log_z = z_dev;
    env->S.log_cap = meta_dev ? capacity : 0;
    return IRBPP_OK;
}

int irbpp_set_episode_window(irbpp_env* env, const irbpp_episode_window* w) {
    if (!env) return IRBPP_ERR_ARG;
    if (w == nullptr) { env->window = irbpp_episode_window{}; return IRBPP_OK; }
    if (!w->ring_dev || !w->snapshot_dev || !w->rows_dev || !w->state_dev || w->window < 1 || w->window > WINDOW_MAX ||
        w->history < 1)
        return IRBPP_ERR_ARG;
    env->window = *w;
    return IRBPP_OK;
}

int irbpp_episode_metrics(const irbpp_episode_window* parts, int32_t n_parts, int32_t first_step, int32_t n_steps,
                          double* out_dev, void* stream) {
    if (!parts || !out_dev || n_parts < 1 || n_parts > WINDOW_PARTS_MAX || first_step < 1) return IRBPP_ERR_ARG;
    WindowParts wp;
    memset(&wp, 0, sizeof wp);
    wp.P = n_parts;
    wp.W = parts[0].window;
    wp.H = parts[0].history;
    if (wp.W < 1 || wp.W > WINDOW_MAX || wp.H < 1 || n_steps < 1 || n_steps > wp.H) return IRBPP_ERR_ARG;
    for (int p = 0; p < n_parts; ++p) {
        if (!parts[p].snapshot_dev || !parts[p].rows_dev || !parts[p].state_dev || parts[p].window != wp.W ||
            parts[p].history != wp.H)
            return IRBPP_ERR_ARG;
        wp.snap[p] = parts[p].snapshot_dev;
        wp.rows[p] = parts[p].rows_dev;
        wp.state[p] = parts[p].state_dev;
    }
    hipLaunchKernelGGL(irbpp_window_metrics_kernel, dim3(n_steps), dim3(64), (size_t)3 * wp.W * sizeof(double), (hipStream_t)stream,
                       wp, first_step, out_dev);
    return hipGetLastError() == hipSuccess ? IRBPP_OK : IRBPP_ERR_HIP;
}

int irbpp_sumtree_find(const float* tree_dev, int32_t n_env, int32_t capacity, const float* values_dev, int32_t draws,
                       float* prob_dev, int64_t* data_idx_dev, int64_t* tree_idx_dev, void* stream) {
    if (!tree_dev || !values_dev || !prob_dev || !data_idx_dev || !tree_idx_dev || n_env < 1 || capacity < 1 || draws < 1)
        return IRBPP_ERR_ARG;
    const int n = n_env * draws;
    hipLaunchKernelGGL(irbpp_sumtree_find_kernel, dim3((n + 255) / 256), dim3(256), 0, (hipStream_t)stream, tree_dev, n_env,
                       capacity, values_dev, draws, prob_dev, data_idx_dev, tree_idx_dev);
    return hipGetLastError() == hipSuccess ? IRBPP_OK : IRBPP_ERR_HIP;
}

int irbpp_sumtree_sample(const float* tree_dev, const int64_t* index_dev, int32_t n_env, int32_t capacity, int32_t draws,
                         int32_t n_step, uint64_t seed, int32_t max_tries, float* prob_dev, int64_t* data_idx_dev,
                         int64_t* tree_idx_dev, int32_t* failed_dev, void* stream) {
    if (!tree_dev || !index_dev || !prob_dev || !data_idx_dev || !tree_idx_dev || !failed_dev || n_env < 1 || capacity < 1 ||
        draws < 1 || n_step < 0 || max_tries < 1)
        return IRBPP_ERR_ARG;
    const int n = n_env * draws;
    hipLaunchKernelGGL(irbpp_sumtree_sample_kernel, dim3((n + 255) / 256), dim3(256), 0, (hipStream_t)stream, tree_dev, index_dev,
                       n_env, capacity, draws, n_step, seed, max_tries, prob_dev, data_idx_dev, tree_idx_dev, failed_dev);
    return hipGetLastError() == hipSuccess ? IRBPP_OK : IRBPP_ERR_HIP;
}

int irbpp_sumtree_update(float* tree_dev, float* max_dev, int32_t n_env, int32_t capacity, const int64_t* tree_idx_dev,
                         const float* priority_dev, int32_t leaves, const uint8_t* env_mask_dev, void* stream) {
    if (!tree_dev || !max_dev || !tree_idx_dev || !priority_dev || n_env < 1 || capacity < 1 || leaves < 1) return IRBPP_ERR_ARG;
    if (2 * capacity - 1 > SUMTREE_LDS) return IRBPP_ERR_ARG;
    hipLaunchKernelGGL(irbpp_sumtree_update_kernel, dim3(n_env), dim3(64), (size_t)(2 * capacity - 1) * sizeof(float), (hipStream_t)stream, tree_dev, max_dev, capacity,
                       tree_idx_dev, priority_dev, leaves, env_mask_dev);
    return hipGetLastError() == hipSuccess ? IRBPP_OK : IRBPP_ERR_HIP;
}

int irbpp_masked_argmax(const float* q_dev, int32_t q_stride, const float* obs_dev, int32_t obs_stride, int32_t selected,
                        int32_t n_env, int64_t* action_dev, void* stream) {
    if (!q_dev || !obs_dev || !action_dev || n_env < 1 || selected < 1 || q_stride < selected || obs_stride < 5 * selected)
        return IRBPP_ERR_ARG;
    hipLaunchKernelGGL(irbpp_masked_argmax_kernel, dim3((n_env + 3) / 4), dim3(256), 0, (hipStream_t)stream, q_dev, q_stride,
                       obs_dev, obs_stride, selected, n_env, action_dev);
    return hipGetLastError() == hipSuccess ? IRBPP_OK : IRBPP_ERR_HIP;
}

int irbpp_replay_gather(const irbpp_replay_view* v, int32_t draws, float beta, const int64_t* data_idx_dev, const float* prob_dev,
                        float* state_dev, int64_t* action_dev, float* return_dev, float* next_state_dev, float* nonterminal_dev,
                        float* weight_dev, void* stream) {
    if (!v || !v->states_dev || !v->actions_dev || !v->rewards_dev || !v->nonterminals_dev || !v->tree_dev || !v->index_dev ||
        !v->full_dev || !v->scaling_dev || v->n_env < 1 || v->capacity < 1 || v->obs_len < 1 || v->n_step < 1 || draws < 1 ||
        draws > 256 || !data_idx_dev || !prob_dev || !state_dev || !action_dev || !return_dev || !next_state_dev ||
        !nonterminal_dev || !weight_dev)
        return IRBPP_ERR_ARG;
    hipLaunchKernelGGL(irbpp_replay_gather_kernel, dim3(v->n_env), dim3(256), 0, (hipStream_t)stream, v->states_dev, v->actions_dev,
                       v->rewards_dev, v->nonterminals_dev, v->tree_dev, v->index_dev, v->full_dev, v->scaling_dev, v->capacity,
                       v->obs_len, v->n_step, draws, beta, data_idx_dev, prob_dev, state_dev, action_dev, return_dev,
                       next_state_dev, nonterminal_dev, weight_dev);
    return hipGetLastError() == hipSuccess ? IRBPP_OK : IRBPP_ERR_HIP;
}

int irbpp_replay_append(const irbpp_replay_store* m, const float* state_dev, int64_t state_stride, const void* action_dev,
                        int32_t action_bytes, const void* reward_dev, int32_t reward_bytes, const uint8_t* terminal_dev,
                        const uint8_t* valid_dev, void* stream) {
    if (!m || !m->states_dev || !m->actions_dev || !m->rewards_dev || !m->nonterminals_dev || !m->timesteps_dev || !m->tree_dev ||
        !m->max_dev || !m->index_dev || !m->full_dev || !m->t_dev || m->n_env < 1 || m->capacity < 1 || m->obs_len < 1 ||
        !state_dev || state_stride < m->obs_len || !action_dev || (action_bytes != 4 && action_bytes != 8) || !reward_dev ||
        (reward_bytes != 4 && reward_bytes != 8) || !terminal_dev)
        return IRBPP_ERR_ARG;
    hipLaunchKernelGGL(irbpp_replay_append_kernel, dim3(m->n_env), dim3(256), 0, (hipStream_t)stream, m->states_dev, m->actions_dev,
                       m->rewards_dev, m->nonterminals_dev, m->timesteps_dev, m->tree_dev, m->max_dev, m->index_dev, m->full_dev,
                       m->t_dev, m->capacity, m->obs_len, state_dev, (long long)state_stride, action_dev, action_bytes, reward_dev,
                       reward_bytes, terminal_dev, valid_dev);
    return hipGetLastError() == hipSuccess ? IRBPP_OK : IRBPP_ERR_HIP;
}

int irbpp_debug_phase_cycles(irbpp_env* env, int64_t* cycles_dev) {
    if (!env) return IRBPP_ERR_ARG;
    drop_graphs(env);
    env->phase_cycles = (long long*)cycles_dev;
    return IRBPP_OK;
}

int irbpp_debug_kernel_info(const irbpp_env* env, int32_t* lds_bytes, const char** kernel_name) {
    if (!env || !lds_bytes || !kernel_name) return IRBPP_ERR_ARG;
    *lds_bytes = env->P.lds_bytes;
    const int n = env->P.N, spec = pick_spec(env);
    const bool lattice = lattice_images(env->P);
    const bool wave_emit = lattice && !(env->cfg.tuning & IRBPP_TUNE_BLOCK_EMIT) && (n >= 2048 || (env->cfg.tuning & IRBPP_TUNE_WAVE_EMIT));
    const int cpw = pick_trace_cpw(env, n);
    char emit[48];
    snprintf(emit, sizeof emit, "%s%s", wave_emit ? "irbpp_emit_wave_kernel" : "irbpp_emit_kernel",
             spec == 1 ? "_s1" : spec == 2 ? "_s2" : (spec == 3 && !wave_emit) ? "_s3" : (spec == 4 && !wave_emit) ? "_s4" : spec == 5 ? "_s5" : "");
    snprintf(const_cast<irbpp_env*>(env)->kernel_names, sizeof env->kernel_names, "%s + irbpp_trace_kernel%s + irbpp_polygon_kernel + %s%s",
             pick_env_kernel(env).name, cpw > 64 ? "_refill" : cpw == 64 ? "" : (cpw == 32 ? "_c32" : "_c16"), emit,
             !split_apply(env, n) ? "" : (env->P.K > 1 ? (n < 2048 ? " (step: irbpp_apply_wg_kernel alone)" : " (step: irbpp_apply_kernel alone)")
                                                       : " (step: irbpp_apply_kernel in front, transition kernel in MODE_OBSERVE)"));
    if (env->P.wide) {
        const int levels = (int)floor(env->P.bin_z / env->P.res_z + 1e-9);
        char why[48] = "";
        if (levels > TUNED_MAX_LEVELS) snprintf(why, sizeof why, ", %d height levels", levels);
        snprintf(const_cast<irbpp_env*>(env)->kernel_names, sizeof env->kernel_names, "irbpp_wide_kernel alone (action grid of %d x %d cells%s)%s", env->P.Ax,
                 env->P.Ay, why, env->P.K > 1 ? " (step: the apply kernel alone)" : " (step: irbpp_apply_kernel in front)");
    }
    else if (chain_launch(env, n)) {
        const bool s1 = spec == 1;
        snprintf(const_cast<irbpp_env*>(env)->kernel_names, sizeof env->kernel_names, "%s alone (observation finished in the bin's workgroup)%s",
                 s1 ? "irbpp_env_kernel_chain_s1" : "irbpp_env_kernel_chain", env->P.K > 1 ? " (step: irbpp_apply_wg_kernel alone)" : "");
    }
// ... 54 lines not shown
```

irbpp_amd/csrc/irbpp_device.h:

```cpp
#pragma once
#include <hip/hip_runtime.h>
#include <stdint.h>

namespace irbpp {

#ifndef IRBPP_CONTOUR_IPT
#define IRBPP_CONTOUR_IPT 2
#endif
constexpr int CONTOUR_IPT = IRBPP_CONTOUR_IPT;

constexpr int WMETA = 8;
constexpr int NXCD = 8;
constexpr int XCD_STRIDE = 64;
#ifndef IRBPP_TRACE_P
#define IRBPP_TRACE_P 2
#endif
constexpr int ROUND_POINTS = 64 * IRBPP_TRACE_P, ROUND_BYTES = ROUND_POINTS * 7;
constexpr int MAX_BINS = 1 << 20;
constexpr int TUNED_MAX_LEVELS = 31;
constexpr int MAX_LEVELS = 222;

struct ShapeRot {
    int32_t fx, fy;
    int32_t ax, ay;
    int32_t nb, nt;
    int32_t ob, ot;
    int32_t has_out;
    int32_t pad;
    int32_t nblk, oblk;
    int32_t bx, by;
    double bc;
    double ext_x, ext_y, ext_z;
    double ext_z_r;
    double com_x, com_y;
};

struct Cell {
    double v;
    int32_t ij;
    int32_t pad;
};

struct alignas(16) GCell { double b; int32_t off; int32_t pad; };

struct Tables {
    const ShapeRot* sr;
    const Cell* bcell;
    const Cell* tcell;
    const Cell* blkcell;
    const GCell* gcell;
    const double* volume;
    const int32_t* seq;
    int32_t n_shapes, n_traj, seq_len;
    int32_t stream;
};

struct alignas(64) BinState {
    int32_t cursor;
    int32_t episode;
    int32_t cur_item;
    int32_t nvalid;
    int32_t order_action;
    int32_t item_idx;
    int32_t ep_len;
    int32_t traj_row;
    double ratio_acc;
    double ep_reward;
    int32_t nrows;
    int32_t pad0;
    double pad1[1];
};

struct State {
    double* hm;
    int32_t* queue;
    uint32_t* cand;
    BinState* bs;
    double* totals;
    uint32_t* log_meta;
    double* log_z;
    int32_t log_cap;
    int32_t* order;
    int32_t* err;
    double* w_posz;
    uint32_t* w_valid;
    uint32_t* w_vmask;
    int32_t* w_meta;
    uint16_t* w_img;
    uint8_t* w_imgrot;
    uint2* w_cand;
    uint8_t* w_big;
    uint8_t* w_round;
    int32_t* w_nround;
    int32_t* w_heavy;
    int32_t* w_total;
};

struct Params {
    int32_t N, Hx, Hy, Hc, Ax, Ay, AC, step, R, S, K;
    double res_a, res_h, res_z, inv_res_z;
    double txs[32];
    double bin_x, bin_y, bin_z, bin_vol;
    double scale_z, ibin_z;
    int32_t traj_start, goff, gbins;
    int32_t obs_len0, obs_len1;
    int32_t pp, LX, LY, PL, tile_words;
    uint32_t mg_pp, mg_ly;
    int32_t g_ysh;
    int32_t box, o_m1;
    int32_t o_vbits;
    int32_t o_sr;
    int32_t o_hm, o_posz, o_lev, o_present, o_taskidx, o_tasklist, o_img, o_clist, o_vmask, o_scratch, o_red, o_dps;
    int32_t nslot, slot_cap, slot_bytes, scratch_bytes, lds_bytes;
    int32_t lds_bytes_full;
    int32_t e_vmask, e_red, e_hist, e_keys, emit_lds_bytes;
    int32_t ew_bytes, e_need;
    int32_t big_slot_bytes;
    int32_t block_b, mb_w, mb_h, o_mb, o_c2;
    int32_t block_rots;
    uint32_t mg_hy, mg_step, mg_ay, mg_ax, mg_ac, mg_mbw;
    int32_t dbg_repeat;
    int32_t split;
    int32_t wimg;
    int32_t seg_cap;
    int32_t round_cap;
    int32_t heavy_cap, heavy_thr;
    int32_t stability;
    int32_t wide;
    int32_t vrow;
    int32_t rect;
};

constexpr int32_t align16(int32_t v) { return (v + 15) & ~15; }
constexpr uint32_t div_magic(int32_t d) { return d >= 2 ? (uint32_t)((1ull << 32) / (uint64_t)d + 1ull) : 0u; }

constexpr void layout_lds(Params& P, int32_t pad = 0) {
    P.mg_hy = div_magic(P.Hy);
    P.mg_step = div_magic(P.step);
    P.mg_ay = div_magic(P.Ay);
    P.mg_ax = div_magic(P.Ax);
    P.mg_ac = div_magic(P.AC);
    P.mg_mbw = div_magic(P.mb_w);
    P.pp = P.step;
    P.LX = P.Ax;
    P.LY = P.Ay;
    P.PL = P.LX * P.LY;
    P.tile_words = P.pp * P.pp * P.PL;
    P.mg_pp = div_magic(P.pp);
    P.mg_ly = div_magic(P.LY);
    P.g_ysh = 0;
    while ((1 << P.g_ysh) < P.Ay) ++P.g_ysh;
    P.nslot = 64;
    P.slot_cap = 64;
    P.slot_bytes = P.slot_cap + 4;
    int32_t off = 0;
    P.o_sr = off;        off += align16(P.R * (int32_t)sizeof(ShapeRot));
    P.o_lev = off;       off += align16(P.R * P.AC);
    P.o_present = off;   off += align16(P.R * 8);
    P.o_taskidx = off;   off += align16(P.R * 64 * 2);
    P.o_tasklist = off;  off += align16(P.R * 64 * 2);
    const int32_t img_bytes = align16(2 * CONTOUR_IPT * 16 * 16 * 2);
    P.o_img = off;       off += img_bytes;
    const int32_t mb_bytes = align16(P.mb_w * P.mb_h * 8);
    if (mb_bytes <= img_bytes) P.o_mb = P.o_img;
    else { P.o_mb = off; off += mb_bytes; }
    P.o_c2 = off;        off += mb_bytes ? align16(P.AC * 8) : 0;
    P.o_vmask = off;     off += align16(P.R * 16 * 4);
    P.o_vbits = P.o_taskidx;
    P.o_m1 = off;        off += P.box ? align16(P.Hx * P.Ay * 8) : 0;
    P.o_red = off;       off += 256;
    const int32_t slots = align16(P.nslot * P.slot_bytes);
    const int32_t dps = 4 * 64 * 4 + 4 * 64;
    int32_t scratch = slots + dps + 512;
    const int32_t keys = (P.R * P.AC + P.S) * 4 + 64;
    if (scratch < keys) scratch = keys;
    if (scratch < P.tile_words * 8) scratch = P.tile_words * 8;
    if (scratch < 2 * CONTOUR_IPT * 16 * 16 * 2 + 512) scratch = 2 * CONTOUR_IPT * 16 * 16 * 2 + 512;
    P.scratch_bytes = align16(scratch);
    P.o_hm = off;
    P.o_scratch = off;
    P.o_dps = off + slots;
    P.o_clist = off + P.scratch_bytes - 512;
    P.big_slot_bytes = P.scratch_bytes - 512;
    off += P.scratch_bytes;
    off += align16(pad);
    P.lds_bytes = off;
    P.o_posz = off;
    P.lds_bytes_full = off + align16(P.R * P.AC * 8);
    int32_t e = 0;
    P.e_vmask = e;  e += align16(P.R * 16 * 4);
    P.e_red = e;    e += 256;
    {
        int32_t npad = 64;
        while (npad < P.S) npad <<= 1;
        P.e_hist = e;   e += align16(10 * npad > 1024 ? 10 * npad : 1024);
    }
    P.e_keys = e;   e += align16(keys);
    P.ew_bytes = align16((P.R * 16 + P.S + 64) * 4);
    if (e < 4 * P.ew_bytes) e = 4 * P.ew_bytes;
    P.e_need = e;   e += 16;
    P.emit_lds_bytes = e;
}

struct SpecKey { int32_t Ax, Ay, step, R, S, block_b, box, block_rots; };
constexpr Params spec_params(const SpecKey& k) {
    Params P{};
    P.Ax = k.Ax; P.Ay = k.Ay; P.step = k.step; P.R = k.R; P.S = k.S;
    P.Hx = k.Ax * k.step; P.Hy = k.Ay * k.step; P.Hc = P.Hx * P.Hy; P.AC = k.Ax * k.Ay;
    P.block_b = k.block_b; P.box = k.box; P.block_rots = k.block_rots;
    P.mb_h = k.block_b ? (P.Hx - k.block_b) / k.step + 1 : 0;
    P.mb_w = k.block_b ? (P.Hy - k.block_b) / k.step + 1 : 0;
    P.split = 1;
    P.stability = 0;
    P.wide = 0;
    P.vrow = 16;
    P.dbg_repeat = 0;
    P.wimg = k.R * 64;
    P.heavy_thr = (k.S * 3) / 5;
    P.obs_len1 = 5 * k.S + 9 + P.Hc;
    layout_lds(P);
    return P;
}
#define IRBPP_PINNED_FIELDS(X)                                                                                          \
    X(Hx) X(Hy) X(Hc) X(Ax) X(Ay) X(AC) X(step) X(R) X(S) X(pp) X(LX) X(LY) X(PL) X(tile_words) X(mg_pp) X(mg_ly)      \
    X(g_ysh) X(box) X(o_m1) X(o_vbits) X(o_sr) X(o_hm) X(o_posz) X(o_lev) X(o_present) X(o_taskidx) X(o_tasklist)      \
    X(o_img) X(o_clist) X(o_vmask) X(o_scratch) X(o_red) X(o_dps) X(nslot) X(slot_cap) X(slot_bytes) X(scratch_bytes)  \
    X(lds_bytes) X(lds_bytes_full) X(e_vmask) X(e_red) X(e_hist) X(e_keys) X(emit_lds_bytes) X(ew_bytes) X(e_need) X(big_slot_bytes)         \
    X(block_b) X(block_rots) X(mb_w) X(mb_h) X(o_mb) X(o_c2) X(mg_hy) X(mg_step) X(mg_ay) X(mg_ax) X(mg_ac) X(mg_mbw) X(dbg_repeat)  \
    X(split) X(wimg) X(heavy_thr) X(stability) X(obs_len1) X(wide) X(vrow)
constexpr bool spec_matches(const Params& P, const Params& C) {
#define IRBPP_X(f) if (P.f != C.f) return false;
    IRBPP_PINNED_FIELDS(IRBPP_X)
#undef IRBPP_X
    return true;
}
constexpr SpecKey SPEC_KEYS[] = {
    {0, 0, 0, 0, 0, 0, 0, 0},
    {16, 16, 2, 4, 500, 4, 0, 0x0F},
    {16, 16, 2, 2, 500, 0, 1, 0},
    {16, 16, 2, 8, 500, 0, 0, 0},
    {16, 16, 4, 8, 500, 0, 0, 0},
    {16, 16, 2, 8, 500, 4, 0, 0x0F},
};
constexpr int N_SPECS = (int)(sizeof(SPEC_KEYS) / sizeof(SPEC_KEYS[0]));
template <int SPEC>
__host__ __device__ __forceinline__ Params specialise(const Params& P) {
    if constexpr (SPEC == 0) {
        return P;
    } else {
        constexpr Params C = spec_params(SPEC_KEYS[SPEC]);
        Params Q = P;
#define IRBPP_X(f) Q.f = C.f;
        IRBPP_PINNED_FIELDS(IRBPP_X)
#undef IRBPP_X
        return Q;
    }
}

enum Mode : int32_t {
    MODE_RESET = 0,
    MODE_STEP = 1,
    MODE_CANDS = 2,
    MODE_POSSIBLE = 3,
    MODE_OBSERVE = 4
};

struct StepIO {
    const int32_t* actions;
    float* obs;
    int32_t obs_stride;
    double* reward;
    uint8_t* done;
    int32_t* counter;
    double* ratio;
    double* ep_reward;
    int32_t* ep_len;
    uint8_t* stable;
    double* posz_out;
    uint8_t* mask_out;
    long long* phase_cycles;
    int32_t* heur_out;
    int32_t heur_method;
    int32_t heur_dir;
    const int32_t* bin_list;
    int32_t reset_next;
    int32_t* obs_rows;
    int32_t* auto_action;
    int32_t* err_out;
    int32_t use_order;
    int32_t block_off;
    int32_t heavy_turn;
    int32_t n_slots;
    int32_t fixed_slot;
};

}
```

irbpp_amd/csrc/irbpp_kernels.hip:

```cpp
#include <hip/hip_runtime.h>
#include <math.h>
#include <stdint.h>

#include "contours_device.h"
#include "irbpp_device.h"
#include "../../include/irbpp.h"

#ifndef IRBPP_PASS
#define IRBPP_PASS 1
#endif

#undef IRBPP_HERE
#undef IRBPP_PASS_NS
#if IRBPP_PASS == 1
#define IRBPP_HERE ::irbpp::
#elif IRBPP_PASS == 2
#define IRBPP_HERE ::irbpp::wg512::
#define IRBPP_PASS_NS wg512
#else
#define IRBPP_HERE ::irbpp::wg128::
#define IRBPP_PASS_NS wg128
#endif

namespace irbpp {
// ... 532 lines not shown
            --sp;
            continue;
        }
        int n2 = cn / 2;
        n2 -= n2 % 8;
        if (cp == 2) {
            ret = cl + ret;
            --sp;
            continue;
        }
        const int child = cp == 0 ? n2 : cn - n2;
#pragma unroll
        for (int d = 0; d < DEPTH; ++d) {
            if (d == sp) { phase[d] = cp + 1; if (cp == 1) left[d] = ret; }
            if (d == sp + 1) { fn[d] = child; phase[d] = 0; }
        }
        ++sp;
    }
    return ret;
}

__device__ inline double heuristic_score(const Params& P, const Tables& T, const StepIO& io, const Lds& L,
                                         const ShapeRot& sr, int r, int X, int Y) {
    const double z = L.posz[r * P.AC + X * P.Ay + Y];
    if (!(z < 1e3)) return 1e6;
    const bool xf = (io.heur_dir & 2) != 0, yf = (io.heur_dir & 1) != 0;
    const double cx = xf ? (double)(P.Ax - X) : (double)X, cy = yf ? (double)(P.Ay - Y) : (double)Y;
    double score;
    switch (io.heur_method) {
        case 1: score = z; break;
        case 2: score = (cx + cy) * P.res_a + 100.0 * z; break;
        case 3: score = cx + cy; break;
        default: {
            score = (cx + cy) * P.res_a;
            const Cell* top = T.tcell + sr.ot;
            const int fy = sr.fy, nt = sr.nt;
            int e = 0, i = 0, j = 0, cur = 0;
            int next_in = nt > 0 ? top[0].pad : -1;
            auto next = [&]() -> double {
                const double h = L.hm[tile_rc(P, X * P.step + i, Y * P.step + j)];
                double v = 0.0;
                if (e == next_in) {
                    v = top[cur].v + z;
                    ++cur;
                    next_in = cur < nt ? top[cur].pad : -1;
                }
                ++e;
                if (++j == fy) { j = 0; ++i; }
                return fmax(v, h);
            };
            score += np_pairwise_sum(next, sr.fx * sr.fy) * 100.0;
        }
    }
    return round6(score);
}

__device__ __forceinline__ uint32_t wave_or_to_lane63(uint32_t x) {
    int v = (int)x;
    v |= __builtin_amdgcn_update_dpp(0, v, 0x111, 0xF, 0xF, false);
    v |= __builtin_amdgcn_update_dpp(0, v, 0x112, 0xF, 0xF, false);
    v |= __builtin_amdgcn_update_dpp(0, v, 0x114, 0xF, 0xF, false);
    v |= __builtin_amdgcn_update_dpp(0, v, 0x118, 0xF, 0xF, false);
    v |= __builtin_amdgcn_update_dpp(0, v, 0x142, 0xA, 0xF, false);
    v |= __builtin_amdgcn_update_dpp(0, v, 0x143, 0xC, 0xF, false);
    return (uint32_t)v;
}

typedef int32_t gcell_words __attribute__((ext_vector_type(4)));
typedef const __attribute__((address_space(4))) gcell_words* ConstGCellPtr;
__device__ __forceinline__ double gcell_b(const gcell_words c) { return __hiloint2double(c.y, c.x); }

enum OverlapPath : int { PATH_ANY = 0, PATH_BLOCK = 1, PATH_BOX = 2, PATH_GENERIC = 3,
                         PATH_MIXED = 4 };
constexpr int GENERIC_TICKET = 40;
typedef int32_t gcell_quad __attribute__((ext_vector_type(16)));
__device__ __forceinline__ gcell_quad gcell_request(ConstGCellPtr p) {
    gcell_quad q;
    asm volatile("s_load_dwordx16 %0, %1, 0x0" : "=&s"(q) : "s"(p));
    return q;
}
template <int G>
__device__ __forceinline__ void gcell_await(gcell_quad& q, double (&a0)[G], double (&a1)[G]) {
    if (G == 1) asm volatile("s_waitcnt lgkmcnt(0)" : "+s"(q), "+v"(a0[0]), "+v"(a1[0]));
    else if (G == 2) asm volatile("s_waitcnt lgkmcnt(0)" : "+s"(q), "+v"(a0[0]), "+v"(a1[0]), "+v"(a0[G > 1 ? 1 : 0]), "+v"(a1[G > 1 ? 1 : 0]));
    else asm volatile("s_waitcnt lgkmcnt(0)" : "+s"(q), "+v"(a0[0]), "+v"(a1[0]), "+v"(a0[G > 1 ? 1 : 0]), "+v"(a1[G > 1 ? 1 : 0]),
                      "+v"(a0[G > 2 ? 2 : 0]), "+v"(a1[G > 2 ? 2 : 0]));
}
template <int G, int STRIDE>
__device__ __forceinline__ double gcell_height(const char* const (&hb)[G], int g, int off) {
#if defined(__HIP_DEVICE_COMPILE__)
    if (STRIDE > 0) {
        typedef const volatile __attribute__((address_space(3))) double* LdsF64;
        return *(LdsF64)((uint32_t)(uintptr_t)hb[0] + off + g * STRIDE);
    }
#endif
    return *(const double*)(hb[STRIDE > 0 ? 0 : g] + off + (STRIDE > 0 ? g * STRIDE : 0));
}
template <int G, int STRIDE>
__device__ __forceinline__ void gcell_quad_apply(const gcell_quad& q, const char* const (&hb)[G], double (&a0)[G], double (&a1)[G]) {
    double h0[G], h1[G], h2[G], h3[G];
#pragma unroll
    for (int g = 0; g < G; ++g) {
        h0[g] = gcell_height<G, STRIDE>(hb, g, q[2]); h1[g] = gcell_height<G, STRIDE>(hb, g, q[6]);
        h2[g] = gcell_height<G, STRIDE>(hb, g, q[10]); h3[g] = gcell_height<G, STRIDE>(hb, g, q[14]);
    }
#pragma unroll
    for (int g = 0; g < G; ++g) {
        a0[g] = fmax(a0[g], h0[g] - __hiloint2double(q[1], q[0]));
        a1[g] = fmax(a1[g], h1[g] - __hiloint2double(q[5], q[4]));
    }
#pragma unroll
    for (int g = 0; g < G; ++g) {
        a0[g] = fmax(a0[g], h2[g] - __hiloint2double(q[9], q[8]));
        a1[g] = fmax(a1[g], h3[g] - __hiloint2double(q[13], q[12]));
    }
}
template <int G, int STRIDE>
__device__ inline void gcell_walk(ConstGCellPtr gc, int nb, const char* const (&hb)[G], double init, double (&z)[G]) {
    double a0[G], a1[G];
#pragma unroll
    for (int g = 0; g < G; ++g) a0[g] = a1[g] = init;
    gcell_quad A = gcell_request(gc), B;
    gcell_await<G>(A, a0, a1);
    int e = 0;
    bool in_a = true;
    while (e + 4 <= nb) {
        B = gcell_request(gc + e + 4);
        gcell_quad_apply<G, STRIDE>(A, hb, a0, a1);
        gcell_await<G>(B, a0, a1);
        e += 4;
        in_a = false;
        if (e + 4 > nb) break;
        A = gcell_request(gc + e + 4);
        gcell_quad_apply<G, STRIDE>(B, hb, a0, a1);
        gcell_await<G>(A, a0, a1);
        e += 4;
        in_a = true;
    }
    if (e < nb) {
        const gcell_quad q = in_a ? A : B;
        const int left = nb - e;
#pragma unroll
        for (int g = 0; g < G; ++g) {
            a0[g] = fmax(a0[g], gcell_height<G, STRIDE>(hb, g, q[2]) - __hiloint2double(q[1], q[0]));
            if (left > 1) a1[g] = fmax(a1[g], gcell_height<G, STRIDE>(hb, g, q[6]) - __hiloint2double(q[5], q[4]));
            if (left > 2) a0[g] = fmax(a0[g], gcell_height<G, STRIDE>(hb, g, q[10]) - __hiloint2double(q[9], q[8]));
        }
    }
#pragma unroll
    for (int g = 0; g < G; ++g) z[g] = fmax(a0[g], a1[g]);
}

#endif
template <int PATH>
__device__ inline int overlap_test(const Params& P, const Tables& T, const State& S, const StepIO& io,
                                   const Lds& L, int b, int item, bool debug_out, double* zdst, bool sr_staged, bool dense) {
    const bool use_block = PATH == PATH_BLOCK || PATH == PATH_MIXED || (PATH == PATH_ANY && P.block_b > 0);
    const bool use_box = PATH == PATH_BOX || (PATH == PATH_ANY && P.box != 0);
    const uint32_t rots_all = (1u << P.R) - 1u;
    const uint32_t brots = PATH == PATH_BLOCK ? rots_all : ((PATH == PATH_MIXED || PATH == PATH_ANY) ? (uint32_t)P.block_rots : 0u);
    const bool use_lists = PATH == PATH_GENERIC || PATH == PATH_MIXED || (PATH == PATH_ANY && !use_box && brots != rots_all);
    const int tid = threadIdx.x;
    const int R = P.R, AC = P.AC, Ax = P.Ax, Ay = P.Ay;
    constexpr int SRW = sizeof(ShapeRot) / 4;
    int* srw = L.sr;
    if (item >= 0 && !sr_staged)
#pragma unroll 1
        for (int t = tid; t < R * SRW; t += BLOCK) srw[t] = ((const int*)(T.sr + (size_t)item * R))[t];
    for (int rep = 0; rep < IRBPP_REPS(13); ++rep) {
    if (tid < R) L.present[tid] = 0ull;
    if (tid == 0) L.redi[GENERIC_TICKET] = WAVES;
#pragma unroll 1
    for (int i = tid; i < R * 16; i += BLOCK) { L.vmask[i] = 0u; L.vbits[i] = 0u; }
#pragma unroll 1
    for (int i = tid; i < (R * AC + 3) / 4; i += BLOCK) ((uint32_t*)L.lev)[i] = 0xFFFFFFFFu;
    }
    if (dense) for (int i = tid; i < R * AC; i += BLOCK) zdst[i] = 1e3;
    int bl_first = 0, bl_total = 0;
    Cell bl_entry = {};
    if (use_block)
    for (int rep = 0; rep < IRBPP_REPS(6); ++rep) {
        if (rep) __syncthreads();
        const int planes = P.pp * P.pp, mq = P.block_b / P.step;
#pragma unroll 1
        for (int t = tid; t < AC; t += BLOCK) {
            double m = L.hm[t];
            for (int pl = 1; pl < planes; ++pl) m = fmax(m, L.hm[pl * P.PL + t]);
            L.c2[t] = m;
        }
        __syncthreads();
        if (rep == 0 && item >= 0) {
            const ShapeRot* sa = (const ShapeRot*)srw;
            bl_first = __builtin_amdgcn_readfirstlane(sa->oblk);
            bl_total = __builtin_amdgcn_readfirstlane(sa[R - 1].oblk) + __builtin_amdgcn_readfirstlane(sa[R - 1].nblk) - bl_first;
            if (bl_total <= AC / 2 && tid < bl_total) bl_entry = T.blkcell[bl_first + tid];
        }
#pragma unroll 1
        for (int t = tid; t < P.mb_h * P.mb_w; t += BLOCK) {
            const int pi = fdiv(t, P.mb_w, P.mg_mbw), pj = t - pi * P.mb_w;
            const double* c = L.c2 + pi * Ay + pj;
            double m = -1e300;
            for (int i = 0; i < mq; ++i)
                for (int j = 0; j < mq; ++j) m = fmax(m, c[i * Ay + j]);
            L.mb[t] = m;
        }
    }
    __syncthreads();
    const bool bl_lds = use_block && item >= 0 && bl_total <= AC / 2;
    typedef int32_t bl_words __attribute__((ext_vector_type(4)));
    bl_words* const bl = (bl_words*)L.c2;
    if (bl_lds) {
        if (tid < bl_total) {
            bl_words w;
            w.x = __double2loint(bl_entry.v); w.y = __double2hiint(bl_entry.v); w.z = bl_entry.ij * 8; w.w = 0;
            bl[tid] = w;
        }
        __syncthreads();
    }

    const int lane = tid & 63, wave = __builtin_amdgcn_readfirstlane(tid >> 6);
    int my_valid = 0;
    if (use_block || use_box) {
    constexpr int CELLS = BLOCK >= 256 ? 1 : 256 / BLOCK;
    if (CELLS > 1 && use_box) __builtin_trap();
#pragma unroll 1
    for (int ci = 0; ci < CELLS; ++ci) {
    const int cell = CELLS == 1 ? tid : tid + ci * BLOCK;
    const int X = fdiv(cell, Ay, P.mg_ay), Y = cell - X * Ay;
    double zs[8];
    bool vs[8];
    if (use_box) {
        double* const m1 = L.m1;
#pragma unroll
        for (int r = 0; r < 8; ++r) {
            zs[r] = 1e3;
            vs[r] = false;
            if (r >= R || item < 0) continue;
            const ShapeRot* sp = (const ShapeRot*)srw + r;
            const int s_ax = __builtin_amdgcn_readfirstlane(sp->ax), s_ay = __builtin_amdgcn_readfirstlane(sp->ay);
            const int bx = __builtin_amdgcn_readfirstlane(sp->bx), by = __builtin_amdgcn_readfirstlane(sp->by);
            const int has_out = __builtin_amdgcn_readfirstlane(sp->has_out);
            const double ext_z_r = sp->ext_z_r, bc = sp->bc;
            for (int idx = tid; idx < P.Hx * Ay; idx += BLOCK) {
                const int i = fdiv(idx, Ay, P.mg_ay), yy = idx - i * Ay;
                if (yy <= Ay - s_ay) {
                    const double* rowp = L.hm + tile_row_part(P, i);
                    double m = -1e300;
                    for (int j = 0; j < by; ++j) m = fmax(m, rowp[tile_col_part(P, yy * P.step + j)]);
                    m1[idx] = m;
                }
            }
            __syncthreads();
            const bool in_range = cell < AC && X <= Ax - s_ax && Y <= Ay - s_ay;
            if (in_range) {
                const double* colp = m1 + X * P.step * Ay + Y;
                double m = -1e300;
                for (int i = 0; i < bx; ++i) m = fmax(m, colp[i * Ay]);
                m = m - bc;
                if (has_out) m = fmax(m, 0.0);
                zs[r] = m;
                vs[r] = round6_scaled(m + ext_z_r - P.bin_z) <= 0.0;
            }
            __syncthreads();
        }
    } else {
    int ncell_next = 0, off_next = 0;
    Cell pre = {};
    if (bl_lds) {
    for (int rep = 0; rep < IRBPP_REPS(2); ++rep) {
#pragma unroll
    for (int r = 0; r < 8; ++r) {
        zs[r] = 1e3;
        vs[r] = false;
        if (r >= R || !((brots >> r) & 1u)) continue;
        const ShapeRot* sp = (const ShapeRot*)srw + r;
        const int s_ax = __builtin_amdgcn_readfirstlane(sp->ax), s_ay = __builtin_amdgcn_readfirstlane(sp->ay);
        const int has_out = __builtin_amdgcn_readfirstlane(sp->has_out);
        const int ne = __builtin_amdgcn_readfirstlane(sp->nblk), e0 = __builtin_amdgcn_readfirstlane(sp->oblk) - bl_first;
        const double ext_z_r = sp->ext_z_r;
        const bool in_range = cell < AC && X <= Ax - s_ax && Y <= Ay - s_ay;
        if (in_range) {
            const char* const hb = (const char*)(L.mb + X * P.mb_w + Y);
            const bl_words* const be = bl + e0;
            double m = has_out ? 0.0 : -1e300;
            int u = 0;
            for (; u + 4 <= ne; u += 4) {
                bl_words q[4];
                double hv[4];
#pragma unroll
                for (int k = 0; k < 4; ++k) q[k] = be[u + k];
#pragma unroll
                for (int k = 0; k < 4; ++k) hv[k] = *(const double*)(hb + q[k].z);
#pragma unroll
                for (int k = 0; k < 4; ++k) m = fmax(m, hv[k] - __hiloint2double(q[k].y, q[k].x));
            }
            for (; u < ne; ++u) {
                const bl_words q = be[u];
                m = fmax(m, *(const double*)(hb + q.z) - __hiloint2double(q.y, q.x));
            }
            zs[r] = m;
            vs[r] = round6_scaled(m + ext_z_r - P.bin_z) <= 0.0;
        }
    }
    }
    } else
    for (int rep = 0; rep < IRBPP_REPS(2); ++rep) {
    if (item >= 0) {
        const ShapeRot* s0 = (const ShapeRot*)srw;
        ncell_next = __builtin_amdgcn_readfirstlane(s0->nblk);
        off_next = __builtin_amdgcn_readfirstlane(s0->oblk);
        const Cell* c0 = T.blkcell + off_next;
        if (ncell_next > 0) pre = c0[lane < ncell_next ? lane : ncell_next - 1];
    }
#pragma unroll
    for (int r = 0; r < 8; ++r) {
        zs[r] = 1e3;
        vs[r] = false;
        if (r >= R || item < 0) continue;
        const ShapeRot* sp = (const ShapeRot*)srw + r;
        const int s_ax = __builtin_amdgcn_readfirstlane(sp->ax), s_ay = __builtin_amdgcn_readfirstlane(sp->ay);
        const int has_out = __builtin_amdgcn_readfirstlane(sp->has_out);
        const double ext_z_r = sp->ext_z_r;
        const int ncell = ((brots >> r) & 1u) ? ncell_next : 0, off0 = off_next;
        Cell c = pre;
        if (r + 1 < R) {
            const ShapeRot* sn = sp + 1;
            ncell_next = __builtin_amdgcn_readfirstlane(sn->nblk);
            off_next = __builtin_amdgcn_readfirstlane(sn->oblk);
            const Cell* cn = T.blkcell + off_next;
            if (ncell_next > 0) pre = cn[lane < ncell_next ? lane : ncell_next - 1];
        }
        const bool in_range = cell < AC && X <= Ax - s_ax && Y <= Ay - s_ay;
        const double* h0 = L.mb + X * P.mb_w + Y;
        double m = has_out ? 0.0 : -1e300;
        const Cell* cells = T.blkcell + off0;
        for (int base = 0; base < ncell; base += 64) {
            if (base > 0) {
                const int idx = base + lane < ncell ? base + lane : ncell - 1;
                c = cells[idx];
            }
            const int cnt = ncell - base < 64 ? ncell - base : 64;
// ... 63 lines not shown
        if (rows_align) {
            const unsigned long long bal = __ballot(valid && cell < AC);
            if (Y == 0 && cell < AC) L.vbits[r * 16 + X] = (uint32_t)(bal >> (lane & ~(Ay - 1))) & ((1u << Ay) - 1u);
        }
    }
#pragma unroll
    for (int r = 0; r < 8; ++r) {
        if (r >= R || (!use_box && !((brots >> r) & 1u))) continue;
        const int code = level_code[r];
        unsigned long long todo = __ballot(code != 255), bits = 0ull;
        while (todo) {
            const int c = __builtin_amdgcn_readlane(code, __ffsll((long long)todo) - 1);
            bits |= 1ull << c;
            todo &= ~__ballot(code == c);
        }
        if ((tid & 63) == 0 && bits) atomicOr(&L.present[r], bits);
    }
    }
    }
    }
    if (use_lists) {
    const int ysh = P.g_ysh, rpw = 64 >> ysh;
    const int rs = lane >> ysh, Y = lane & ((1 << ysh) - 1);
    const bool rows_whole = (1 << ysh) == Ay;
    int my_grp = 0;
    if (lane < R && item >= 0 && !((brots >> lane) & 1u)) {
        const ShapeRot* sp = (const ShapeRot*)srw + lane;
        const int wx = Ax - sp->ax + 1, wy = Ay - sp->ay + 1;
        if (wx > 0 && wy > 0) my_grp = (wx + rpw - 1) >> (6 - ysh);
    }
    const int t3 = my_grp > 3 ? 2 : (my_grp > 0 ? 1 : 0), t2 = (my_grp + 1) >> 1;
    const int n3 = __builtin_amdgcn_readlane(wave_inclusive_sum(t3), 63), n2 = __builtin_amdgcn_readlane(wave_inclusive_sum(t2), 63);
    const int gmax = n3 >= WAVES ? 3 : (n2 >= WAVES ? 2 : 1);
    const int my_tasks = gmax == 3 ? t3 : (gmax == 2 ? t2 : my_grp);
    const int my_incl = wave_inclusive_sum(my_tasks), my_first = my_incl - my_tasks;
    const int ntask = __builtin_amdgcn_readlane(my_incl, 63);
    auto task_rotation = [&](int t) {
        return __popcll(__ballot(lane >= 1 && lane < 8 && t >= my_first));
    };
    int pref = 0;
    uint32_t task_lo = 0u, task_hi = 0u;
    auto task_finish = [&](int r, int X, int s_ax, int s_ay, double ext_z_r, double z) {
        const bool in_range = X <= Ax - s_ax && Y <= Ay - s_ay;
        const bool valid = in_range && round6_scaled(z + ext_z_r - P.bin_z) <= 0.0;
        const int cell = X * Ay + Y;
        if (debug_out && in_range) {
            const KernArgsPtr ka = cold_args();
            ka->io.posz_out[((size_t)b * R + r) * AC + cell] = z;
            ka->io.mask_out[((size_t)b * R + r) * AC + cell] = valid ? 1 : 0;
        }
        uint32_t bits_lo = 0u, bits_hi = 0u;
        if (valid) {
            if (!debug_out) zdst[r * AC + cell] = z;
            const int li = np_floor_divide_int(z, P.res_z, P.inv_res_z);
            if (li != -1) {
                const int idx = li + 32;
                if (idx < 0 || idx > 63) raise_error(S, IRBPP_DEVERR_LEVEL_RANGE);
                else {
                    L.lev[r * AC + cell] = (uint8_t)idx;
                    if (idx < 32) bits_lo = 1u << idx; else bits_hi = 1u << (idx - 32);
                }
            }
            ++my_valid;
        }
        const unsigned long long bal = __ballot(valid);
        if (Y == 0 && X < Ax) L.vbits[r * 16 + X] = (uint32_t)(bal >> (rs << ysh)) & ((1u << Ay) - 1u);
        task_lo |= bits_lo;
        task_hi |= bits_hi;
    };
    auto task_presence = [&](int r) {
        const uint32_t lo = wave_or_to_lane63(task_lo), hi = wave_or_to_lane63(task_hi);
        if (lane == 63) {
            uint32_t* pw = (uint32_t*)&L.present[r];
            if (lo) atomicOr(pw, lo);
            if (hi) atomicOr(pw + 1, hi);
        }
        task_lo = task_hi = 0u;
    };
    auto prefetch_list = [&](int ob, int nb) {
        const char* lv = (const char*)(T.gcell + ob);
        for (int o = lane * 128; o < nb * 16; o += 64 * 128) pref |= *(const int*)(lv + o);
    };
    for (int t = wave, mine = 0; ; ++mine) {
        if (mine > 0) {
            int tk = 0;
            if (lane == 0) tk = atomicAdd(&L.redi[GENERIC_TICKET], 1);
            t = __builtin_amdgcn_readfirstlane(tk);
        }
        if (t >= ntask) break;
        const int r = task_rotation(t);
        const int tq = t - __builtin_amdgcn_readlane(my_first, r), ng = __builtin_amdgcn_readlane(my_grp, r);
        const int nt = __builtin_amdgcn_readlane(my_tasks, r);
        const int base = nt == 1 ? ng : (nt == ng ? 1 : ng >> 1), rem = ng - base * nt;
        const int G = base + (tq < rem ? 1 : 0), g0 = tq * base + (tq < rem ? tq : rem);
        const ShapeRot* sp = (const ShapeRot*)srw + r;
        const int s_ax = __builtin_amdgcn_readfirstlane(sp->ax), s_ay = __builtin_amdgcn_readfirstlane(sp->ay);
        const int has_out = __builtin_amdgcn_readfirstlane(sp->has_out);
        const int nb = __builtin_amdgcn_readfirstlane(sp->nb), ob = __builtin_amdgcn_readfirstlane(sp->ob);
        const double ext_z_r = sp->ext_z_r;
        const ConstGCellPtr gc = (ConstGCellPtr)(unsigned long long)(T.gcell + ob);
        if (mine == 0) prefetch_list(ob, nb);
        if (t + WAVES < ntask) {
            const int rn = task_rotation(t + WAVES);
            if (rn != r) {
                const ShapeRot* sn = (const ShapeRot*)srw + rn;
                prefetch_list(__builtin_amdgcn_readfirstlane(sn->ob), __builtin_amdgcn_readfirstlane(sn->nb));
            }
        }
        const double init = has_out ? 0.0 : -1e300;
        const int yc = Y < Ay ? Y : Ay - 1;
        const int X0 = g0 * rpw + rs;
        auto lane_base = [&](int X) { return (const char*)(L.hm + (X < Ax ? X : Ax - 1) * Ay + yc); };
        double z[3];
        if (rows_whole) {
            const char* h1[1] = {(const char*)(L.hm + X0 * Ay + Y)};
            const char* h2[2] = {h1[0], nullptr};
            const char* h3[3] = {h1[0], nullptr, nullptr};
            if (G == 1) gcell_walk<1, 512>(gc, nb, h1, init, (double(&)[1])z[0]);
            else if (G == 2) gcell_walk<2, 512>(gc, nb, h2, init, (double(&)[2])z[0]);
            else gcell_walk<3, 512>(gc, nb, h3, init, z);
        } else {
            const char* h1[1] = {lane_base(X0)};
            const char* h2[2] = {h1[0], lane_base(X0 + rpw)};
            const char* h3[3] = {h1[0], h2[1], lane_base(X0 + 2 * rpw)};
            if (G == 1) gcell_walk<1, 0>(gc, nb, h1, init, (double(&)[1])z[0]);
            else if (G == 2) gcell_walk<2, 0>(gc, nb, h2, init, (double(&)[2])z[0]);
            else gcell_walk<3, 0>(gc, nb, h3, init, z);
        }
        task_finish(r, X0, s_ax, s_ay, ext_z_r, z[0]);
        if (G > 1) task_finish(r, X0 + rpw, s_ax, s_ay, ext_z_r, z[1]);
        if (G > 2) task_finish(r, X0 + 2 * rpw, s_ax, s_ay, ext_z_r, z[2]);
        task_presence(r);
    }
    asm volatile("" :: "v"(pref));
    if (debug_out)
        for (int i = tid; i < R * AC; i += BLOCK) {
            const int r = fdiv(i, AC, P.mg_ac), cell = i - r * AC, X = fdiv(cell, Ay, P.mg_ay), Y = cell - X * Ay;
            const ShapeRot* sp = (const ShapeRot*)srw + r;
            if (((brots >> r) & 1u) == 0u && (item < 0 || X > Ax - sp->ax || Y > Ay - sp->ay)) {
                const KernArgsPtr ka = cold_args();
                ka->io.posz_out[((size_t)b * R + r) * AC + cell] = 1e3;
                ka->io.mask_out[((size_t)b * R + r) * AC + cell] = 0;
            }
        }
    }
    return block_sum_int(my_valid, L.redi);
}

__device__ inline void emit_observation(const Params& P, const State& S, const StepIO& io, const Lds& L, int b, int item,
                                        int nvalid, float* obs, const double* zsrc, const uint32_t* gvalid);
template <int IPT>
__device__ inline void split_handover(const Params& P, const State& S, const Lds& L, int b, int slot, int item, int nvalid);

template <int PATH, bool CHAIN = false>
__device__ inline void observe_location(const Params& P, const Tables& T, const State& S, const StepIO& io,
                                        const Lds& L, int b, int item, float* obs, bool debug_out, bool sr_staged,
                                        unsigned char* chain_lds = nullptr) {
    item = __builtin_amdgcn_readfirstlane(item);
    const int tid = threadIdx.x;
    const int R = P.R, AC = P.AC, Ax = P.Ax, Ay = P.Ay;
    const int X = fdiv(tid, Ay, P.mg_ay), Y = tid - X * Ay;
    const int nvalid = IRBPP_HERE overlap_test<PATH>(P, T, S, io, L, b, item, debug_out, S.w_posz + (size_t)b * R * AC, sr_staged, false);
    if (debug_out) return;
    if (tid < 9) obs[5 * P.S + tid] = tid == 0 ? (float)item : 0.0f;
    for (int rep = 0; rep < IRBPP_REPS(8); ++rep)
    for (TileWalk w = IRBPP_HERE tile_walk_begin(P, tid); w.lin < P.Hc; tile_walk_next(w)) obs[5 * P.S + 9 + w.lin] = (float)L.hm[tile_walk_index(P, w)];
    __syncthreads();
    stamp(io, b, 2);

    if (io.phase_cycles && tid == 0)
        for (int k = 5; k < PHASE_ROW; ++k)
            if (k < 8 || k > 10) io.phase_cycles[(size_t)b * PHASE_ROW + k] = 0;
    if constexpr (CHAIN) {
        {
            uint32_t* gb = S.w_valid + (size_t)b * P.R * 16;
#pragma unroll 1
            for (int i = tid; i < P.R * 16; i += BLOCK) gb[i] = L.vbits[i];
        }
        __syncthreads();
        ::irbpp::contour_stage(P, S, L, nullptr);
        __builtin_amdgcn_fence(__ATOMIC_RELEASE, "workgroup");
        __syncthreads();
        __builtin_amdgcn_fence(__ATOMIC_ACQUIRE, "workgroup");
        Lds Le = L;
        Le.img = (uint16_t*)chain_lds;
        ::irbpp::emit_observation(P, S, io, Le, b, item, nvalid, obs, S.w_posz + (size_t)b * R * AC, S.w_valid + (size_t)b * R * 16);
        return;
    }
    IRBPP_HERE split_handover<(CONTOUR_IPT * 256) / BLOCK>(P, S, L, b, (int)blockIdx.x + io.block_off, item, nvalid);
    if (io.phase_cycles && tid == 0)
        io.phase_cycles[(size_t)b * PHASE_ROW + 5] = (long long)clock64() - io.phase_cycles[(size_t)b * PHASE_ROW + 2];
}

#if IRBPP_PASS == 1
__device__ __forceinline__ unsigned long long sortable_f64(double v) {
    const unsigned long long b = (unsigned long long)__double_as_longlong(v);
    return (b >> 63) ? ~b : (b | 0x8000000000000000ull);
}
constexpr int SEL_PER_THREAD = (8 * 256 + BLOCK - 1) / BLOCK;

template <typename KEY>
__device__ inline void select_smallest(const Params& P, const Lds& L, const double* zsrc, const uint32_t* vbits, int n, int want,
                                       const KEY& key, uint32_t* out, uint32_t* sel, uint32_t* hist) {
    const int tid = threadIdx.x;
    auto value = [&](uint32_t k) {
        const uint32_t r = k >> 16, x = (k >> 8) & 255u, y = k & 255u;
        if (vbits != nullptr && !((vbits[r * 16 + x] >> y) & 1u)) return 1e3;
        return zsrc[r * P.AC + x * P.Ay + y];
    };
    unsigned long long sk[SEL_PER_THREAD];
    uint32_t ky[SEL_PER_THREAD];
#pragma unroll
    for (int k = 0; k < SEL_PER_THREAD; ++k) {
        const int e = tid + k * BLOCK;
        ky[k] = e < n ? key(e) : 0u;
        sk[k] = e < n ? sortable_f64(value(ky[k])) : ~0ull;
    }
    unsigned long long prefix = 0ull;
    int remaining = want;
    for (int d = 7; d >= 0; --d) {
        hist[tid] = 0u;
        __syncthreads();
#pragma unroll
        for (int k = 0; k < SEL_PER_THREAD; ++k) {
            if (k * BLOCK >= n) continue;
            const int e = tid + k * BLOCK;
            const bool in = e < n && (d == 7 || (sk[k] >> (8 * (d + 1))) == prefix);
            const int digit = (int)((uint32_t)(sk[k] >> (8 * d)) & 255u);
            const unsigned long long act = __ballot(in);
            if (act == 0ull) continue;
            const int c0 = __builtin_amdgcn_readlane(digit, __ffsll((long long)act) - 1);
            if (__ballot(in && digit != c0) == 0ull) {
                if ((tid & 63) == __ffsll((long long)act) - 1) atomicAdd(&hist[c0], (uint32_t)__popcll(act));
            } else if (in) {
                atomicAdd(&hist[digit], 1u);
            }
        }
        __syncthreads();
        if (tid < 64) {
            int c[4], sum = 0;
#pragma unroll
            for (int i = 0; i < 4; ++i) { c[i] = (int)hist[tid * 4 + i]; sum += c[i]; }
            const int incl = wave_inclusive_sum(sum);
            int run = incl - sum;
            if (run < remaining && remaining <= incl) {
#pragma unroll
                for (int i = 0; i < 4; ++i) {
                    if (run < remaining && remaining <= run + c[i]) { L.redi[32] = tid * 4 + i; L.redi[33] = remaining - run; }
                    run += c[i];
                }
            }
        }
        __syncthreads();
        prefix = (prefix << 8) | (unsigned long long)(uint32_t)L.redi[32];
        remaining = L.redi[33];
    }
    int nsel = 0, neq = 0;
#pragma unroll
    for (int k = 0; k < SEL_PER_THREAD; ++k) {
        if (k * BLOCK < n) {
            const int e = tid + k * BLOCK;
            const bool eq = e < n && sk[k] == prefix;
            int teq;
            const int eqb = block_scan_flag(eq, L.redi, teq);
            const bool take = e < n && (sk[k] < prefix || (eq && neq + eqb < remaining));
            int tsel;
            const int pos = block_scan_flag(take, L.redi, tsel);
            if (take) sel[nsel + pos] = ky[k];
            nsel += tsel;
            neq += teq;
        }
    }
    __syncthreads();
    int npad = 64;
    while (npad < want) npad <<= 1;
    uint32_t* const khi = hist;
    uint32_t* const klo = hist + npad;
    uint16_t* const kps = (uint16_t*)(hist + 2 * npad);
    for (int i = tid; i < npad; i += BLOCK) {
        unsigned long long v = ~0ull;
        if (i < want) v = sortable_f64(value(sel[i]));
        khi[i] = (uint32_t)(v >> 32);
        klo[i] = (uint32_t)v;
        kps[i] = (uint16_t)(i < want ? i : 0xFFFF);
    }
    __syncthreads();
    for (int k = 2; k <= npad; k <<= 1)
        for (int j = k >> 1; j > 0; j >>= 1) {
            const int sh = __ffs(j) - 1;
            for (int t = tid; t < (npad >> 1); t += BLOCK) {
                const int i = ((t >> sh) << (sh + 1)) | (t & (j - 1)), l = i | j;
                const uint32_t ah = khi[i], al = klo[i], bh = khi[l], bl = klo[l];
                const uint32_t ap = kps[i], bp = kps[l];
                const bool a_gt_b = ah > bh || (ah == bh && (al > bl || (al == bl && ap > bp)));
                if (a_gt_b == ((i & k) == 0)) {
                    khi[i] = bh; klo[i] = bl; kps[i] = (uint16_t)bp;
                    khi[l] = ah; klo[l] = al; kps[l] = (uint16_t)ap;
                }
            }
            const int j_next = j > 1 ? (j >> 1) : k;
            if (j >= 128 || j_next >= 128 || (j == 1 && k == npad)) __syncthreads();
            else IRBPP_WAVE_SYNC();
        }
    for (int r = tid; r < want; r += BLOCK) out[r] = sel[kps[r]];
    __syncthreads();
}

#ifdef IRBPP_AB_EMIT_ACCOUNT
#define IRBPP_EMIT_STAMP(k) do { if (io.phase_cycles && threadIdx.x == 0) io.phase_cycles[(size_t)b * PHASE_ROW + (k)] = (long long)clock64(); } while (0)
#else
#define IRBPP_EMIT_STAMP(k) do {} while (0)
#endif
__device__ inline void emit_observation(const Params& P, const State& S, const StepIO& io, const Lds& L, int b, int item,
                                        int nvalid, float* obs, const double* zsrc, const uint32_t* gvalid) {
    const int tid = threadIdx.x;
    const int R = P.R, AC = P.AC, Ax = P.Ax, Ay = P.Ay;
    const int X = fdiv(tid, Ay, P.mg_ay), Y = tid - X * Ay;
    const int prev_rows = io.obs_rows != nullptr ? io.obs_rows[b] : -1;
    if (tid == 0) ((unsigned long long*)L.redd)[7] = ~0ull;
    uint32_t* keys = (uint32_t*)L.scratch;
// ... 795 lines not shown
                ++n_dp;
            }
            if (inline_dp && n_rounds > 0 && at < round_cap) {
                const int lim = at + n_rounds < round_cap ? n_rounds : round_cap - at;
                for (int i = 0; i < lim; ++i)
#pragma unroll
                    for (int u = 0; u < PP; ++u) rec0[(size_t)i * ROUND_BYTES + 64 * PP + u * 64 + lane] = 0;
            }
            n_dp_total += n_dp;
            IRBPP_WAVE_SYNC();
        };
        prefetch();
        int guard = 16384;
        for (;;) {
            const unsigned long long walking = __ballot(w.run != 0u);
            const int idle = 64 - __popcll(walking);
            if ((idle >= THR && nxt < nb) || walking == 0ull) {
                flush();
                if (nxt >= nb) break;
                const int rank = (int)__builtin_amdgcn_mbcnt_hi((uint32_t)(~walking >> 32), __builtin_amdgcn_mbcnt_lo((uint32_t)~walking, 0u));
                const bool take = w.run == 0u && nxt + rank < nb;
                const uint32_t ex = (uint32_t)__shfl((int)pf_e.x, rank), ey = (uint32_t)__shfl((int)pf_e.y, rank);
                const uint32_t rot = (uint32_t)__shfl((int)pf_rot, rank);
                uint32_t wd[8];
                wd[0] = (uint32_t)__shfl((int)pf0.x, rank); wd[1] = (uint32_t)__shfl((int)pf0.y, rank);
                wd[2] = (uint32_t)__shfl((int)pf0.z, rank); wd[3] = (uint32_t)__shfl((int)pf0.w, rank);
                wd[4] = (uint32_t)__shfl((int)pf1.x, rank); wd[5] = (uint32_t)__shfl((int)pf1.y, rank);
                wd[6] = (uint32_t)__shfl((int)pf1.z, rank); wd[7] = (uint32_t)__shfl((int)pf1.w, rank);
                if (take) {
                    x0 = (int)(ey & 15u);
                    y0 = (int)((ey >> 4) & 15u);
                    rk = (int)ex * P.R + (int)rot;
                    uint32_t r[16], c[16];
#pragma unroll
                    for (int q = 0; q < 8; ++q) {
                        r[2 * q] = c[2 * q] = wd[q] & 0xFFFFu;
                        r[2 * q + 1] = c[2 * q + 1] = wd[q] >> 16;
                    }
                    transpose16(c);
                    frames_store(fr, r, c);
                    walk_start(w, fr, x0, y0, my_slot, LCAP, true, WT);
                }
                nxt += idle < nb - nxt ? idle : nb - nxt;
                ++refills;
                if (nxt < nb) prefetch();
                continue;
            }
            if (w.run != 0u) walk_iter(w, fr, my_slot, LCAP, my_spill, TRACE_SPILL, WT);
            if (--guard == 0) { if (lane == 0) atomicOr(S.err, IRBPP_DEVERR_TRACE_GUARD); break; }
        }
        if (prof && lane == 0) {
            const int b0 = (int)cl[0].x;
            long long* row = prof + (size_t)b0 * PHASE_ROW;
            const long long t_end = (long long)clock64();
            row[11] = t_end - t_start;
            row[12] = 0;
            row[13] = t_end - t_start;
            row[14] = (long long)refills | ((long long)(16384 - guard) << 16);
            row[15] = 1 | ((long long)n_dp_total << 20) | ((long long)nb << 40);
        }
        IRBPP_WAVE_SYNC();
    }
}
extern "C" __global__ void __launch_bounds__(64) irbpp_trace_kernel_refill(const Params P, const State S, long long* prof) {
    trace_refill_body<TRACE_REFILL_BATCH, TRACE_REFILL_THR>(P, S, prof);
}

extern "C" __global__ void __launch_bounds__(64) irbpp_trace_kernel(const Params P, const State S, long long* prof) { trace_body<64>(P, S, prof); }
extern "C" __global__ void __launch_bounds__(64) irbpp_trace_kernel_c32(const Params P, const State S, long long* prof) { trace_body<32>(P, S, prof); }
extern "C" __global__ void __launch_bounds__(64) irbpp_trace_kernel_c16(const Params P, const State S, long long* prof) { trace_body<16>(P, S, prof); }

extern "C" __global__ void __launch_bounds__(64)
irbpp_polygon_kernel(const Params P, const State S
#ifdef IRBPP_AB_POLY_ACCOUNT
                     , long long* prof
#endif
                     ) {
    constexpr int PP = TRACE_P;
#ifdef IRBPP_AB_POLY_ACCOUNT
    long long acct[8] = {0, 0, 0, 0, 0, 0, 0, 0};
    long long* const ac = prof ? acct : nullptr;
    const long long t_begin = (long long)clock64(), w_begin = (long long)wall_clock64();
    long long t_first_loaded = 0, cyc_hops = 0, cyc_dp = 0, cyc_rank = 0, cyc_tail = 0, rounds_done = 0;
#endif
    __shared__ uint32_t dps[64 * PP];
    __shared__ uint8_t dpscratch[64 * PP];
    __shared__ __attribute__((aligned(16))) uint8_t lpts[64 * PP];
    const int lane = threadIdx.x;
    const int round_cap = P.round_cap;
    int seg_n[NXCD], seg_first[NXCD + 1];
    seg_first[0] = 0;
#pragma unroll
    for (int s = 0; s < NXCD; ++s) {
        const int n = S.w_nround[s * XCD_STRIDE];
        seg_n[s] = n < round_cap ? n : round_cap;
        seg_first[s + 1] = seg_first[s] + seg_n[s];
    }
    for (int rd = blockIdx.x; rd < seg_first[NXCD]; rd += gridDim.x) {
        int seg = 0;
#pragma unroll
        for (int s = 1; s < NXCD; ++s) seg += rd >= seg_first[s] ? 1 : 0;
        int first = 0;
#pragma unroll
        for (int s = 0; s < NXCD; ++s) if (s == seg) first = seg_first[s];
        const uint8_t* const rec = S.w_round + ((size_t)seg * round_cap + (rd - first)) * ROUND_BYTES;
        bool live[PP];
        int pv[PP], jj[PP], nn[PP], sbq[PP], prk[PP];
        const uint8_t* pts[PP];
#pragma unroll
        for (int u = 0; u < PP; ++u) {
            const int q = u * 64 + lane;
            pv[u] = rec[q];
            nn[u] = rec[64 * PP + q];
            sbq[u] = rec[2 * 64 * PP + q];
            prk[u] = (int)((const uint32_t*)(rec + 3 * 64 * PP))[q];
            lpts[q] = (uint8_t)pv[u];
        }
        IRBPP_WAVE_SYNC();
#pragma unroll
        for (int u = 0; u < PP; ++u) {
            live[u] = nn[u] > 0;
            jj[u] = u * 64 + lane - sbq[u];
            if (!live[u]) { nn[u] = 1; sbq[u] = 0; jj[u] = 0; pv[u] = 0; }
            pts[u] = lpts + sbq[u];
        }
#ifdef IRBPP_AB_POLY_ACCOUNT
        const long long t_in = (long long)clock64();
        if (rounds_done == 0) t_first_loaded = t_in - t_begin;
        acct[1] = acct[2] = acct[3] = 0;
        approx_convex_segmented<PP>(lane, live, pv, jj, nn, sbq, pts, prk, dps, dpscratch, S.w_vmask, ac);
        const long long t_out = (long long)clock64();
        cyc_hops += acct[1] - t_in; cyc_dp += acct[2] - acct[1]; cyc_rank += acct[3] - acct[2]; cyc_tail += t_out - acct[3];
        ++rounds_done;
#else
        approx_convex_segmented<PP>(lane, live, pv, jj, nn, sbq, pts, prk, dps, dpscratch, S.w_vmask);
#endif
        IRBPP_WAVE_SYNC();
    }
#ifdef IRBPP_AB_POLY_ACCOUNT
    if (prof && lane == 0 && (int)blockIdx.x < P.N) {
        long long* row = prof + (size_t)blockIdx.x * PHASE_ROW;
        row[11] = (long long)clock64() - t_begin;
        row[12] = t_first_loaded | (((long long)(__builtin_amdgcn_s_getreg((31 << 11) | 20) & (NXCD - 1))) << 32);
        row[10] = w_begin;
        row[9] = (long long)wall_clock64();
        row[13] = cyc_hops | (cyc_dp << 32);
        row[14] = cyc_rank | (cyc_tail << 32);
        row[15] = rounds_done | (acct[5] << 8) | (acct[6] << 24);
    }
#endif
}

#endif
template <int PATH, int SPEC, bool FUSED, bool CHAIN = false>
__device__ __forceinline__ void env_transition(const Params& P_run, const Tables& T, const State& S, const StepIO& io,
                                               const int mode, unsigned char* smem);

#if IRBPP_PASS == 1
#ifndef IRBPP_ENV_WAVES
#define IRBPP_ENV_WAVES 8
#endif
#define IRBPP_ENV_KERNEL(NAME, PATH, SPEC, ATTR)                                                                        \
    extern "C" __global__ void __launch_bounds__(BLOCK) ATTR                                                           \
    NAME(const Params P, const Tables T, const State S, const StepIO io, const int mode) {                             \
        extern __shared__ __attribute__((aligned(16))) unsigned char smem[];                                           \
        env_transition<PATH, SPEC, true>(P, T, S, io, mode, smem);                                                     \
    }
#define IRBPP_CAPPED __attribute__((amdgpu_waves_per_eu(IRBPP_ENV_WAVES, IRBPP_ENV_WAVES)))
IRBPP_ENV_KERNEL(irbpp_env_kernel, PATH_BLOCK, 0, IRBPP_CAPPED)
IRBPP_ENV_KERNEL(irbpp_env_kernel_box8, PATH_BOX, 0, IRBPP_CAPPED)
IRBPP_ENV_KERNEL(irbpp_env_kernel_box, PATH_BOX, 0, )
IRBPP_ENV_KERNEL(irbpp_env_kernel_generic8, PATH_GENERIC, 0, IRBPP_CAPPED)
IRBPP_ENV_KERNEL(irbpp_env_kernel_generic, PATH_GENERIC, 0, )
IRBPP_ENV_KERNEL(irbpp_env_kernel_wide, PATH_ANY, 0, )
IRBPP_ENV_KERNEL(irbpp_env_kernel_mixed8, PATH_MIXED, 0, IRBPP_CAPPED)
#define IRBPP_ENV_KERNEL_CHAIN(NAME, PATH, SPEC)                                                                        \
    extern "C" __global__ void __launch_bounds__(BLOCK)                                                                \
    NAME(const Params P, const Tables T, const State S, const StepIO io, const int mode) {                             \
        extern __shared__ __attribute__((aligned(16))) unsigned char smem[];                                           \
        env_transition<PATH, SPEC, true, true>(P, T, S, io, mode, smem);                                               \
    }
IRBPP_ENV_KERNEL_CHAIN(irbpp_env_kernel_chain, PATH_ANY, 0)
#ifndef IRBPP_NO_SPEC
IRBPP_ENV_KERNEL(irbpp_env_kernel_s1, PATH_BLOCK, 1, IRBPP_CAPPED)
IRBPP_ENV_KERNEL(irbpp_env_kernel_s2, PATH_BOX, 2, IRBPP_CAPPED)
IRBPP_ENV_KERNEL(irbpp_env_kernel_s3, PATH_GENERIC, 3, IRBPP_CAPPED)
IRBPP_ENV_KERNEL(irbpp_env_kernel_s4, PATH_GENERIC, 4, )
IRBPP_ENV_KERNEL(irbpp_env_kernel_s5, PATH_MIXED, 5, IRBPP_CAPPED)
IRBPP_ENV_KERNEL_CHAIN(irbpp_env_kernel_chain_s1, PATH_BLOCK, 1)
#endif

#elif IRBPP_PASS == 3
extern "C" __global__ void __launch_bounds__(128)
irbpp_env_kernel_s1_w128(const Params P, const Tables T, const State S, const StepIO io, const int mode) {
    extern __shared__ __attribute__((aligned(16))) unsigned char smem[];
    IRBPP_HERE env_transition<PATH_BLOCK, 1, true>(P, T, S, io, mode, smem);
}
#else
#define IRBPP_ENV_KERNEL_512(NAME, PATH, SPEC, ATTR)                                                                    \
    extern "C" __global__ void __launch_bounds__(512) ATTR                                                             \
    NAME(const Params P, const Tables T, const State S, const StepIO io, const int mode) {                             \
        extern __shared__ __attribute__((aligned(16))) unsigned char smem[];                                           \
        IRBPP_HERE env_transition<PATH, SPEC, true>(P, T, S, io, mode, smem);                                          \
    }
IRBPP_ENV_KERNEL_512(irbpp_env_kernel_generic_w512, PATH_GENERIC, 0, )
#ifndef IRBPP_NO_SPEC
IRBPP_ENV_KERNEL_512(irbpp_env_kernel_s4_w512, PATH_GENERIC, 4, )
IRBPP_ENV_KERNEL_512(irbpp_env_kernel_s4_w512c, PATH_GENERIC, 4, __attribute__((amdgpu_waves_per_eu(8, 8))))
#endif
#endif

template <int PATH, int SPEC, bool FUSED, bool CHAIN>
__device__ __forceinline__ void env_transition(const Params& P_run, const Tables& T, const State& S, const StepIO& io,
                                               const int mode, unsigned char* smem) {
    if constexpr (!FUSED) { if (mode == MODE_STEP) return; }
    Params P_spec;
    const Params& P = SPEC == 0 ? P_run : (P_spec = specialise<SPEC>(P_run), P_spec);
    const Lds L = carve_lds(smem, P);
    const bool some = mode == MODE_RESET && io.bin_list != nullptr;
    const int slot = (int)blockIdx.x + io.block_off;
    const int b = ((mode == MODE_STEP || mode == MODE_CANDS || mode == MODE_OBSERVE) && io.use_order) ? S.order[slot] : some ? io.bin_list[slot] : slot;
    const int tid = threadIdx.x;
    if (b < 0 || b >= P.N) {
        if (tid == 0) raise_error(S, IRBPP_DEVERR_BAD_BIN);
        return;
    }
    const long long t_begin = (long long)clock64();
    double* ghm = S.hm + (size_t)b * P.Hc;
    int32_t* q = S.queue + (size_t)b * P.K;
    float* obs = io.obs ? io.obs + (size_t)(some ? slot : b) * io.obs_stride : nullptr;

    stamp(io, b, 0);
    int st_a = 0, st_item0 = -1, st_oa = 0, st_nvalid = 0, st_nrows = 0, st_cursor = 0, st_trow = 0;
    int ob_item = -1;
    if (mode == MODE_OBSERVE) ob_item = q[0];
    if (FUSED && mode == MODE_STEP) {
        st_a = io.actions[b];
        const BinState* ps0 = S.bs + b;
        st_item0 = ps0->cur_item;
        st_oa = ps0->order_action;
        st_nvalid = ps0->nvalid;
        st_nrows = ps0->nrows;
        st_cursor = ps0->cursor;
        st_trow = ps0->traj_row;
    }
    if (mode == MODE_RESET) {
        for (int i = tid; i < P.tile_words; i += BLOCK) L.hm[i] = 0.0;
        for (int i = tid; i < P.Hc; i += BLOCK) ghm[i] = 0.0;
    } else {
        if (P.tile_words > P.Hc) {
            for (int i = tid; i < P.tile_words; i += BLOCK) L.hm[i] = 0.0;
            __syncthreads();
        }
        for (int rep = 0; rep < IRBPP_REPS(5); ++rep)
        for (TileWalk w = IRBPP_HERE tile_walk_begin(P, tid); w.lin < P.Hc; tile_walk_next(w)) L.hm[tile_walk_index(P, w)] = ghm[w.lin];
    }
    uint32_t st_key = 0u;
    int st_next = -2;
    constexpr int SRW_ = sizeof(ShapeRot) / 4;
    int* const sr0 = (int*)(smem + P.o_img);
    bool ob_staged = false;
    if (mode == MODE_OBSERVE) {
        ob_staged = ob_item >= 0 && ob_item < T.n_shapes;
        if (ob_staged && tid < P.R * SRW_) L.sr[tid] = ((const int*)(T.sr + (size_t)ob_item * P.R))[tid];
    }
    if (FUSED && mode == MODE_STEP) {
        st_a += st_a < 0 ? P.S : 0;
        if (st_a < 0 || st_a >= P.S) { if (tid == 0) raise_error(S, IRBPP_DEVERR_BAD_ACTION); st_a = st_a < 0 ? 0 : P.S - 1; }
        st_key = st_a < st_nrows ? S.cand[(size_t)b * P.S + st_a] : 0u;
        if (P.K == 1) {
            const int at = T.stream ? (int)((uint32_t)st_cursor % (uint32_t)T.seq_len) : st_cursor;
            st_next = at < T.seq_len ? T.seq[(long long)st_trow * T.seq_len + at] : -1;
        }
        if (tid < P.R * SRW_) sr0[tid] = st_item0 >= 0 ? ((const int*)(T.sr + (size_t)st_item0 * P.R))[tid] : 0;
    }
    __syncthreads();

    int obs_item = -1;
    bool do_observe = true, debug_out = false, sr_staged = false;

    if (mode == MODE_POSSIBLE) {
        obs_item = io.actions[b];
        if (obs_item >= T.n_shapes) obs_item = -1;
        debug_out = true;
    } else if (mode == MODE_CANDS) {
        int oa = io.fixed_slot ? io.fixed_slot - 1 : io.actions[b];
        oa += oa < 0 ? P.K : 0;
        if (oa < 0 || oa >= P.K) { if (tid == 0) raise_error(S, IRBPP_DEVERR_BAD_ACTION); oa = oa < 0 ? 0 : P.K - 1; }
        obs_item = q[oa];
        if (tid == 0 && !io.fixed_slot) S.bs[b].order_action = oa;
    } else if (mode == MODE_OBSERVE) {
        obs_item = ob_item;
        sr_staged = ob_staged;
    } else
    if (mode == MODE_RESET) {
        if (tid == 0) {
            BinState* ps = S.bs + b;
            const int ep = (some || io.reset_next) ? ps->episode + 1 : 0;
            const int trow = trajectory_row(P, T, b, ep);
            const int c0 = T.stream ? ps->cursor : 0;
            for (int i = 0; i < P.K; ++i) q[i] = fetch_item(T, S, trow, c0 + i);
            ps->episode = ep;
            ps->traj_row = trow;
            ps->cursor = c0 + P.K;
            ps->cur_item = -1;
            ps->nvalid = 0;
            ps->order_action = 0;
            ps->item_idx = 0;
            ps->ep_len = 0;
            ps->ratio_acc = 0.0;
            ps->ep_reward = 0.0;
            if (!some) for (int i = 0; i < 4; ++i) cold_args()->S.totals[(size_t)b * 4 + i] = 0.0;
            for (int i = 0; i < P.K; ++i) L.redi[16 + i] = q[i];
        }
        __syncthreads();
    } else if constexpr (FUSED) {
        const uint32_t key = st_key;
        const int rot = key >> 16, lx = (key >> 8) & 255, ly = key & 255;
        const int item0 = st_item0;
        const int oa = st_oa;
        bool ok = item0 >= 0 && st_nvalid > 0 && rot < P.R;
        const bool have_sr = item0 >= 0 && rot < P.R;
        const ShapeRot& sr = ((const ShapeRot*)sr0)[have_sr ? rot : 0];
        double vol0 = 0.0;
        if (tid == 0 && item0 >= 0) vol0 = T.volume[item0];
        int sr_pref = 0;
        const bool pref_ok = st_next >= 0 && st_next < T.n_shapes;
        if (pref_ok && tid < P.R * SRW_) sr_pref = ((const int*)(T.sr + (size_t)st_next * P.R))[tid];
        if (ok) {
            const double tx = P_run.txs[lx & 31], ty = P_run.txs[ly & 31];
            if (round6_scaled(tx + sr.ext_x - P.bin_x) > 0.0 || round6_scaled(ty + sr.ext_y - P.bin_y) > 0.0) ok = false;
        }
        double z = 1e3;
        const bool in_grid = have_sr && lx <= P.Ax - sr.ax && ly <= P.Ay - sr.ay;
        const bool want_z = in_grid && (ok || cold_args()->S.log_meta != nullptr);
        uint32_t vword = 0u;
        double zc = 1e3;
        if (want_z) {
            vword = S.w_valid[((size_t)b * P.R + rot) * 16 + lx];
            zc = S.w_posz[((size_t)b * P.R + rot) * P.AC + lx * P.Ay + ly];
        }
        Cell tc0 = {};
        const int s_nt = ok ? sr.nt : 0, s_ot = sr.ot;
        if (tid < s_nt) tc0 = T.tcell[s_ot + tid];
        if (want_z) {
            if ((vword >> ly) & 1u) {
                z = zc;
            } else {
                if (tid == 0) {
                    const Cell* cells = T.bcell + sr.ob;
                    const int s_nb = sr.nb;
                    double m = sr.has_out ? 0.0 : -1e300;
#pragma unroll 1
                    for (int e = 0; e < s_nb; ++e) m = fmax(m, L.hm[tile_of_cell(P, lx, ly, cells[e].ij)] - cells[e].v);
                    L.redd[0] = m;
                }
                __syncthreads();
                z = L.redd[0];
                __syncthreads();
            }
        }
        if (ok) {
            const double top = z * P.scale_z + sr.ext_z * P.scale_z;
            if (round6_scaled(top - P.ibin_z) > 0.0) ok = false;
        }
        bool stable = false;
        if (P.stability != 0 && ok) {
            int* sup = L.redi + 20;
            if (tid < 8) sup[tid] = -0x40000000;
            __syncthreads();
            const Cell* cells = T.bcell + sr.ob;
            const double tol = 0.5 * P.res_z;
            int m8[8];
#pragma unroll
            for (int k = 0; k < 8; ++k) m8[k] = -0x40000000;
            for (int e = tid; e < sr.nb; e += BLOCK) {
                if (L.hm[tile_of_cell(P, lx, ly, cells[e].ij)] - cells[e].v >= z - tol) {
                    const int ci = fdiv(cells[e].pad, sr.fy, div_magic_dev(sr.fy)), cj = cells[e].pad - ci * sr.fy;
                    m8[0] = max(m8[0], ci + 1); m8[1] = max(m8[1], -ci); m8[2] = max(m8[2], cj + 1); m8[3] = max(m8[3], -cj);
                    m8[4] = max(m8[4], ci + cj + 2); m8[5] = max(m8[5], -(ci + cj));
                    m8[6] = max(m8[6], ci + 1 - cj); m8[7] = max(m8[7], cj + 1 - ci);
                }
            }
#pragma unroll
            for (int k = 0; k < 8; ++k)
                if (m8[k] > -0x40000000) atomicMax(&sup[k], m8[k]);
            __syncthreads();
            const double cx = sr.com_x, cy = sr.com_y;
            stable = cx <= sup[0] && -cx <= sup[1] && cy <= sup[2] && -cy <= sup[3] && cx + cy <= sup[4] &&
                     -(cx + cy) <= sup[5] && cx - cy <= sup[6] && cy - cx <= sup[7];
            __syncthreads();
            if (P.stability == 2 && !stable) ok = false;
        }
        if (ok) {
            const Cell* cells = T.tcell + s_ot;
            for (int rep = 0; rep < IRBPP_REPS(12); ++rep)
#pragma unroll 1
            for (int e = tid; e < s_nt; e += BLOCK) {
                const Cell tc = e == tid ? tc0 : cells[e];
                const int ij = tc.ij;
                const int row = lx * P.step + (ij & 0xFFFF), col = ly * P.step + (ij >> 16);
                const int c = tile_rc(P, row, col);
                const double h = fmax(L.hm[c], tc.v + z);
                L.hm[c] = h;
                ghm[row * P.Hy + col] = h;
            }
        } else {
            for (int i = tid; i < P.tile_words; i += BLOCK) L.hm[i] = 0.0;
            for (int i = tid; i < P.Hc; i += BLOCK) ghm[i] = 0.0;
        }
        if (tid == 0) {
            BinState* ps = S.bs + b;
            const KernArgsPtr ka = cold_args();
            if (ok) {
                const double vol = vol0;
                const double reward = (vol / P.bin_vol) * 10.0;
                const double epr = ps->ep_reward + reward;
                const int epl = ps->ep_len + 1;
                const int cursor = st_cursor;
                const int slot = ps->item_idx;
                if (ka->S.log_meta && slot < ka->S.log_cap) {
                    ka->S.log_meta[(size_t)b * ka->S.log_cap + slot] = (uint32_t)item0 | ((uint32_t)rot << 16) |
                                                                ((uint32_t)lx << 20) | ((uint32_t)ly << 24);
                    ka->S.log_z[(size_t)b * ka->S.log_cap + slot] = z;
                }
                ps->ep_reward = epr;
                ps->ep_len = epl;
                ps->item_idx += 1;
                ps->ratio_acc += vol;
                for (int i = oa; i < P.K - 1; ++i) q[i] = q[i + 1];
                int nxt = st_next;
                if (nxt == -2) nxt = fetch_item(T, S, st_trow, cursor);
                else nxt = consume_item(T, S, st_trow, cursor, nxt);
                q[P.K - 1] = nxt;
                ps->cursor = cursor + 1;
                if (ka->io.reward) ka->io.reward[b] = reward;
                if (ka->io.done) ka->io.done[b] = 0;
                if (ka->io.counter) ka->io.counter[b] = -1;
                if (ka->io.ratio) ka->io.ratio[b] = -1.0;
                if (ka->io.ep_reward) ka->io.ep_reward[b] = epr;
                if (ka->io.ep_len) ka->io.ep_len[b] = epl;
                if (ka->io.stable) ka->io.stable[b] = stable ? 1 : 0;
            } else {
                const int counter = ps->item_idx;
                const double ratio = ps->ratio_acc / P.bin_vol;
                const double epr = ps->ep_reward + 0.0;
                const int epl = ps->ep_len + 1;
                if (ka->io.stable) ka->io.stable[b] = 0;
                if (ka->io.reward) ka->io.reward[b] = 0.0;
                if (ka->io.done) ka->io.done[b] = 1;
                if (ka->io.counter) ka->io.counter[b] = counter;
                if (ka->io.ratio) ka->io.ratio[b] = ratio;
                if (ka->io.ep_reward) ka->io.ep_reward[b] = epr;
                if (ka->io.ep_len) ka->io.ep_len[b] = epl;
                if (ka->S.log_meta && counter < ka->S.log_cap) {
                    ka->S.log_meta[(size_t)b * ka->S.log_cap + counter] = (uint32_t)(item0 & 0xFFFF) | ((uint32_t)(rot & 15) << 16) |
                                                                   ((uint32_t)(lx & 15) << 20) | ((uint32_t)(ly & 15) << 24);
                    ka->S.log_z[(size_t)b * ka->S.log_cap + counter] = z;
                }
                double* tot = ka->S.totals + (size_t)b * 4;
                tot[0] += 1.0; tot[1] += ratio; tot[2] += (double)counter; tot[3] += epr;
                const int ep = ps->episode + 1;
                const int trow = trajectory_row(P, T, b, ep);
                ps->episode = ep;
                ps->traj_row = trow;
                const int c0 = T.stream ? st_cursor : 0;
                for (int i = 0; i < P.K; ++i) q[i] = fetch_item(T, S, trow, c0 + i);
                ps->cursor = c0 + P.K;
                ps->item_idx = 0;
                ps->ratio_acc = 0.0;
                ps->ep_reward = 0.0;
                ps->ep_len = 0;
            }
            for (int i = 0; i < P.K; ++i) L.redi[16 + i] = q[i];
        }
        if (ok && pref_ok) {
            if (tid < P.R * SRW_) L.sr[tid] = sr_pref;
            sr_staged = true;
        }
        __syncthreads();
    }

    if (mode == MODE_OBSERVE) stamp(io, b, 1);
    if (mode == MODE_RESET || mode == MODE_STEP) {
        stamp(io, b, 1);
        if (P.K == 1) {
            obs_item = L.redi[16];
            __syncthreads();
        } else {
            do_observe = false;
            for (int i = tid; i < P.K; i += BLOCK) obs[i] = (float)L.redi[16 + i];
            for (int i = tid; i < P.Hc; i += BLOCK) obs[P.K + i] = (float)L.hm[tile_of_linear(P, i)];
        }
    }
    if (do_observe) IRBPP_HERE observe_location<PATH, CHAIN>(P, T, S, io, L, b, obs_item, obs, debug_out, sr_staged, smem + P.lds_bytes);
}

#if IRBPP_PASS == 1
enum ApplyKey : int { KEY_CAND = 0, KEY_CELLS = 1, KEY_HEUR = 2 };

__device__ __forceinline__ uint32_t heuristic_select_wave(const Params& P, const State& S, int method, int dir, int b, int lane) {
    const int RAC = P.R * P.AC;
    const double* const zsrc = S.w_posz + (size_t)b * RAC;
    const uint32_t* const vsrc = S.w_valid + (size_t)b * P.R * P.vrow;
    const bool xf = (dir & 2) != 0, yf = (dir & 1) != 0;
    double best = 1e300;
    int best_i = 0x7fffffff;
    for (int i0 = 0; i0 < RAC; i0 += 4 * 64) {
        int X[4], Y[4];
        uint32_t vw[4];
        double z[4];
#pragma unroll
        for (int u = 0; u < 4; ++u) {
            const int idx = i0 + u * 64 + lane, ii = idx < RAC ? idx : 0;
            const int r = fdiv(ii, P.AC, P.mg_ac), c = ii - r * P.AC;
            X[u] = fdiv(c, P.Ay, P.mg_ay);
            Y[u] = c - X[u] * P.Ay;
            vw[u] = vsrc[r * P.vrow + X[u]];
        }
#pragma unroll
        for (int u = 0; u < 4; ++u) {
            const int idx = i0 + u * 64 + lane;
            z[u] = 1e3;
            if (idx < RAC && ((vw[u] >> Y[u]) & 1u)) z[u] = zsrc[idx];
        }
#pragma unroll
        for (int u = 0; u < 4; ++u) {
            const int idx = i0 + u * 64 + lane;
            if (idx >= RAC) continue;
            double sc = 1e6;
            if ((vw[u] >> Y[u]) & 1u) {
                const double cx = xf ? (double)(P.Ax - X[u]) : (double)X[u], cy = yf ? (double)(P.Ay - Y[u]) : (double)Y[u];
                const double raw = method == 1 ? z[u] : method == 2 ? (cx + cy) * P.res_a + 100.0 * z[u] : cx + cy;
                sc = round6(raw);
            }
            if (sc < best) { best = sc; best_i = idx; }
        }
    }
    for (int o = 32; o > 0; o >>= 1) {
        const double ob = __shfl_xor(best, o);
        const int oi = __shfl_xor(best_i, o);
        if (ob < best || (ob == best && oi < best_i)) { best = ob; best_i = oi; }
    }
    best_i = __builtin_amdgcn_readfirstlane(best_i);
    const int hr = fdiv(best_i, P.AC, P.mg_ac), hrem = best_i - hr * P.AC;
    const int hx = fdiv(hrem, P.Ay, P.mg_ay);
    return ((uint32_t)hr << 16) | ((uint32_t)hx << 8) | (uint32_t)(hrem - hx * P.Ay);
}

template <bool PER_WORKGROUP, int KEY = KEY_CAND>
__device__ __forceinline__ void apply_body(const Params& P, const Tables& T, const State& S, const StepIO& io) {
    const int lane = threadIdx.x & 63;
    const int slot = PER_WORKGROUP ? (int)blockIdx.x : (int)blockIdx.x * WAVES + (int)(threadIdx.x >> 6);
    if (slot >= io.n_slots) return;
    const int b = __builtin_amdgcn_readfirstlane(slot + io.block_off);
    double* const ghm = S.hm + (size_t)b * P.Hc;
    int32_t* const q = S.queue + (size_t)b * P.K;
    if (!PER_WORKGROUP || threadIdx.x < 64) {
    int a = 0, cell_r = 0, cell_x = 0, cell_y = 0;
    if constexpr (KEY == KEY_CAND) a = io.actions[b];
    if constexpr (KEY == KEY_CELLS) { cell_r = io.actions[3 * b]; cell_x = io.actions[3 * b + 1]; cell_y = io.actions[3 * b + 2]; }
    const BinState* ps0 = S.bs + b;
    const int item0 = ps0->cur_item, oa = ps0->order_action, nvalid0 = ps0->nvalid, nrows = ps0->nrows;
    const int cursor = ps0->cursor, trow = ps0->traj_row;
    uint32_t key;
    if constexpr (KEY == KEY_CAND) {
    a += a < 0 ? P.S : 0;
    if (a < 0 || a >= P.S) { if (lane == 0) raise_error(S, IRBPP_DEVERR_BAD_ACTION); a = a < 0 ? 0 : P.S - 1; }
    key = (uint32_t)__builtin_amdgcn_readfirstlane(a < nrows ? (int)S.cand[(size_t)b * P.S + a] : 0);
    } else if constexpr (KEY == KEY_CELLS) {
        if (cell_r < 0 || cell_r >= P.R || cell_x < 0 || cell_x >= P.Ax || cell_y < 0 || cell_y >= P.Ay) {
            if (lane == 0) raise_error(S, IRBPP_DEVERR_BAD_ACTION);
            cell_r = cell_r < 0 ? 0 : cell_r >= P.R ? P.R - 1 : cell_r;
            cell_x = cell_x < 0 ? 0 : cell_x >= P.Ax ? P.Ax - 1 : cell_x;
            cell_y = cell_y < 0 ? 0 : cell_y >= P.Ay ? P.Ay - 1 : cell_y;
        }
        key = (uint32_t)__builtin_amdgcn_readfirstlane((cell_r << 16) | (cell_x << 8) | cell_y);
        (void)nrows;
    } else {
        key = (item0 >= 0 && nvalid0 > 0) ? heuristic_select_wave(P, S, io.heur_method, io.heur_dir, b, lane) : 0u;
        (void)nrows;
    }
    int nxt = -2;
    if (P.K == 1) {
        const int at = T.stream ? (int)((uint32_t)cursor % (uint32_t)T.seq_len) : cursor;
        nxt = at < T.seq_len ? T.seq[(long long)trow * T.seq_len + at] : -1;
    }
    static_assert(sizeof(ShapeRot) == 112, "seven 16-byte chunks per ShapeRot");
    int4 srq = make_int4(0, 0, 0, 0);
    if (item0 >= 0 && lane < P.R * 7) srq = ((const int4*)(T.sr + (size_t)item0 * P.R))[lane];
    const double vol0 = item0 >= 0 ? T.volume[item0] : 0.0;
    const int rot = key >> 16, lx = (key >> 8) & 255, ly = key & 255;
    const bool have_sr = item0 >= 0 && rot < P.R;
    const int rot7 = have_sr ? rot * 7 : 0;
#define IRBPP_SRW(W) __builtin_amdgcn_readlane(((W) & 3) == 0 ? srq.x : ((W) & 3) == 1 ? srq.y : ((W) & 3) == 2 ? srq.z : srq.w, rot7 + ((W) >> 2))
#define IRBPP_SRI(FIELD) IRBPP_SRW(offsetof(ShapeRot, FIELD) / 4)
#define IRBPP_SRD(FIELD) __hiloint2double(IRBPP_SRW(offsetof(ShapeRot, FIELD) / 4 + 1), IRBPP_SRW(offsetof(ShapeRot, FIELD) / 4))
    const int s_ax = IRBPP_SRI(ax), s_ay = IRBPP_SRI(ay), s_nb = IRBPP_SRI(nb), s_ob = IRBPP_SRI(ob), s_has_out = IRBPP_SRI(has_out);
    const int s_ot = IRBPP_SRI(ot);
    const double ext_x = IRBPP_SRD(ext_x), ext_y = IRBPP_SRD(ext_y), ext_z = IRBPP_SRD(ext_z);
    bool ok = item0 >= 0 && nvalid0 > 0 && rot < P.R;
    if (ok) {
        const double tx = P.txs[lx & 31], ty = P.txs[ly & 31];
        if (round6_scaled(tx + ext_x - P.bin_x) > 0.0 || round6_scaled(ty + ext_y - P.bin_y) > 0.0) ok = false;
    }
    const int s_nt = ok ? IRBPP_SRI(nt) : 0;
#undef IRBPP_SRD
#undef IRBPP_SRI
#undef IRBPP_SRW
    const KernArgsPtr ka = cold_args();
    const bool in_grid = have_sr && lx <= P.Ax - s_ax && ly <= P.Ay - s_ay;
    const bool want_z = in_grid && (ok || ka->S.log_meta != nullptr);
    uint32_t vword = 0u;
    double zc = 1e3;
    if (want_z) {
        vword = S.w_valid[((size_t)b * P.R + rot) * P.vrow + lx];
        zc = S.w_posz[((size_t)b * P.R + rot) * P.AC + lx * P.Ay + ly];
    }
    const Cell* const tcells = T.tcell + s_ot;
    Cell tc0 = {};
    if (lane < s_nt) tc0 = tcells[lane];
    const int row0 = lx * P.step, col0 = ly * P.step;
    double h0 = 0.0;
    const int i0 = (row0 + (tc0.ij & 0xFFFF)) * P.Hy + col0 + (tc0.ij >> 16);
    if (lane < s_nt) h0 = ghm[i0];
    double z = 1e3;
    if (want_z) {
        if ((vword >> ly) & 1u) {
            z = zc;
        } else {
            const Cell* cells = T.bcell + s_ob;
            double m = s_has_out ? 0.0 : -1e300;
            for (int e = lane; e < s_nb; e += 64) {
                const Cell c = cells[e];
                m = fmax(m, ghm[(row0 + (c.ij & 0xFFFF)) * P.Hy + col0 + (c.ij >> 16)] - c.v);
            }
            z = wave_max_f64(m);
        }
    }
    if (ok) {
        const double top = z * P.scale_z + ext_z * P.scale_z;
        if (round6_scaled(top - P.ibin_z) > 0.0) ok = false;
    }
    if (ok) {
        if (lane < s_nt) ghm[i0] = fmax(h0, tc0.v + z);
        for (int e0 = 64; e0 < s_nt; e0 += 4 * 64) {
            Cell tc[4];
            int ix[4];
            double hv[4];
#pragma unroll
            for (int u = 0; u < 4; ++u) {
                const int e = e0 + u * 64 + lane;
                tc[u] = tcells[e < s_nt ? e : s_nt - 1];
            }
#pragma unroll
            for (int u = 0; u < 4; ++u) {
                ix[u] = (row0 + (tc[u].ij & 0xFFFF)) * P.Hy + col0 + (tc[u].ij >> 16);
                hv[u] = ghm[ix[u]];
            }
#pragma unroll
            for (int u = 0; u < 4; ++u)
                if (e0 + u * 64 + lane < s_nt) ghm[ix[u]] = fmax(hv[u], tc[u].v + z);
        }
    } else {
        for (int i = lane; i < P.Hc; i += 64) ghm[i] = 0.0;
    }
    if (lane == 0) {
        BinState* ps = S.bs + b;
        if (ok) {
            const double vol = vol0;
            const double reward = (vol / P.bin_vol) * 10.0;
            const double epr = ps->ep_reward + reward;
            const int epl = ps->ep_len + 1;
            const int slot_i = ps->item_idx;
            if (ka->S.log_meta && slot_i < ka->S.log_cap) {
                ka->S.log_meta[(size_t)b * ka->S.log_cap + slot_i] = (uint32_t)item0 | ((uint32_t)rot << 16) |
                                                              ((uint32_t)lx << 20) | ((uint32_t)ly << 24);
                ka->S.log_z[(size_t)b * ka->S.log_cap + slot_i] = z;
            }
            ps->ep_reward = epr;
            ps->ep_len = epl;
            ps->item_idx += 1;
            ps->ratio_acc += vol;
            for (int i = oa; i < P.K - 1; ++i) q[i] = q[i + 1];
            if (nxt == -2) nxt = fetch_item(T, S, trow, cursor);
            else nxt = consume_item(T, S, trow, cursor, nxt);
            q[P.K - 1] = nxt;
            ps->cursor = cursor + 1;
            if (ka->io.reward) ka->io.reward[b] = reward;
            if (ka->io.done) ka->io.done[b] = 0;
            if (ka->io.counter) ka->io.counter[b] = -1;
            if (ka->io.ratio) ka->io.ratio[b] = -1.0;
            if (ka->io.ep_reward) ka->io.ep_reward[b] = epr;
            if (ka->io.ep_len) ka->io.ep_len[b] = epl;
            if (ka->io.stable) ka->io.stable[b] = 0;
        } else {
            const int counter = ps->item_idx;
            const double ratio = ps->ratio_acc / P.bin_vol;
            const double epr = ps->ep_reward + 0.0;
            const int epl = ps->ep_len + 1;
            if (ka->io.stable) ka->io.stable[b] = 0;
            if (ka->io.reward) ka->io.reward[b] = 0.0;
            if (ka->io.done) ka->io.done[b] = 1;
            if (ka->io.counter) ka->io.counter[b] = counter;
            if (ka->io.ratio) ka->io.ratio[b] = ratio;
            if (ka->io.ep_reward) ka->io.ep_reward[b] = epr;
            if (ka->io.ep_len) ka->io.ep_len[b] = epl;
            if (ka->S.log_meta && counter < ka->S.log_cap) {
                ka->S.log_meta[(size_t)b * ka->S.log_cap + counter] = (uint32_t)(item0 & 0xFFFF) | ((uint32_t)(rot & 15) << 16) |
                                                               ((uint32_t)(lx & 15) << 20) | ((uint32_t)(ly & 15) << 24);
                ka->S.log_z[(size_t)b * ka->S.log_cap + counter] = z;
            }
            double* tot = ka->S.totals + (size_t)b * 4;
            tot[0] += 1.0; tot[1] += ratio; tot[2] += (double)counter; tot[3] += epr;
            const int ep = ps->episode + 1;
            const int trow2 = trajectory_row(P, T, b, ep);
            ps->episode = ep;
            ps->traj_row = trow2;
            const int c0 = T.stream ? cursor : 0;
            for (int i = 0; i < P.K; ++i) q[i] = fetch_item(T, S, trow2, c0 + i);
            ps->cursor = c0 + P.K;
            ps->item_idx = 0;
            ps->ratio_acc = 0.0;
            ps->ep_reward = 0.0;
            ps->ep_len = 0;
        }
    }
    }
    if (P.K > 1 && io.obs != nullptr) {
        __builtin_amdgcn_fence(__ATOMIC_RELEASE, "workgroup");
        if (PER_WORKGROUP) __syncthreads();
        __builtin_amdgcn_fence(__ATOMIC_ACQUIRE, "workgroup");
        float* const obs = io.obs + (size_t)b * io.obs_stride;
        const int t0 = PER_WORKGROUP ? (int)threadIdx.x : lane, stride = PER_WORKGROUP ? BLOCK : 64;
        for (int i = t0; i < P.K; i += stride) obs[i] = (float)q[i];
        for (int i0 = 0; i0 < P.Hc; i0 += 8 * stride) {
            double v[8];
#pragma unroll
            for (int u = 0; u < 8; ++u) { const int i = i0 + u * stride + t0; v[u] = ghm[i < P.Hc ? i : P.Hc - 1]; }
#pragma unroll
            for (int u = 0; u < 8; ++u) { const int i = i0 + u * stride + t0; if (i < P.Hc) obs[P.K + i] = (float)v[u]; }
        }
    }
}
extern "C" __global__ void __launch_bounds__(BLOCK)
irbpp_apply_kernel(const Params P, const Tables T, const State S, const StepIO io, const int mode) { apply_body<false>(P, T, S, io); }
extern "C" __global__ void __launch_bounds__(BLOCK)
irbpp_apply_wg_kernel(const Params P, const Tables T, const State S, const StepIO io, const int mode) { apply_body<true>(P, T, S, io); }
extern "C" __global__ void __launch_bounds__(BLOCK)
irbpp_apply_cells_kernel(const Params P, const Tables T, const State S, const StepIO io, const int mode) { apply_body<false, KEY_CELLS>(P, T, S, io); }
extern "C" __global__ void __launch_bounds__(BLOCK)
irbpp_apply_cells_wg_kernel(const Params P, const Tables T, const State S, const StepIO io, const int mode) { apply_body<true, KEY_CELLS>(P, T, S, io); }
extern "C" __global__ void __launch_bounds__(BLOCK)
irbpp_apply_heur_kernel(const Params P, const Tables T, const State S, const StepIO io, const int mode) { apply_body<false, KEY_HEUR>(P, T, S, io); }
extern "C" __global__ void __launch_bounds__(BLOCK)
irbpp_apply_heur_wg_kernel(const Params P, const Tables T, const State S, const StepIO io, const int mode) { apply_body<true, KEY_HEUR>(P, T, S, io); }

extern "C" __global__ void __launch_bounds__(1024)
irbpp_item_order_kernel(const Tables T, const State S, int N) {
    __shared__ int hist[1024];
    __shared__ int start[1024];
    const int tid = threadIdx.x;
    hist[tid] = 0;
    __syncthreads();
    constexpr int PER = 8;
    auto buckets_of = [&](int k0, int (&out)[PER]) {
        int cur[PER], row[PER], item[PER];
#pragma unroll
        for (int u = 0; u < PER; ++u) {
            const int bb = tid + (k0 + u) * 1024;
            const BinState* ps = S.bs + (bb < N ? bb : 0);
            cur[u] = ps->cursor;
            row[u] = ps->traj_row;
        }
#pragma unroll
        for (int u = 0; u < PER; ++u) {
            int c = cur[u];
            if (T.stream) c = (int)((uint32_t)c % (uint32_t)T.seq_len);
            item[u] = c < T.seq_len ? T.seq[(long long)row[u] * T.seq_len + c] : 0;
        }
#pragma unroll
        for (int u = 0; u < PER; ++u) {
            const int it = item[u] < 0 ? 0 : (item[u] >= T.n_shapes ? T.n_shapes - 1 : item[u]);
            out[u] = (int)(((long long)it * 1024) / T.n_shapes);
        }
    };
    int mine[PER];
    for (int k0 = 0; k0 * 1024 < N; k0 += PER) {
        int bk[PER];
        buckets_of(k0, bk);
#pragma unroll
        for (int u = 0; u < PER; ++u) {
            if (k0 == 0) mine[u] = bk[u];
            if (tid + (k0 + u) * 1024 < N) atomicAdd(&hist[bk[u]], 1);
        }
    }
    __syncthreads();
    if (tid < 64) {
        int v[16], sum = 0;
        for (int i = 0; i < 16; ++i) { v[i] = hist[tid * 16 + i]; sum += v[i]; }
        const int inc = wave_inclusive_sum(sum);
        int acc = inc - sum;
        for (int i = 0; i < 16; ++i) { start[tid * 16 + i] = acc; acc += v[i]; }
    }
    __syncthreads();
    const int chunk = N / NXCD;
    for (int k0 = 0; k0 * 1024 < N; k0 += PER) {
        int bk[PER];
        if (k0 == 0) {
#pragma unroll
            for (int u = 0; u < PER; ++u) bk[u] = mine[u];
        } else {
            buckets_of(k0, bk);
        }
#pragma unroll
        for (int u = 0; u < PER; ++u) {
            const int bb = tid + (k0 + u) * 1024;
            if (bb < N) {
// ... 218 lines not shown
```

Before: 63.81 million.

## Carry per-cell max grid and dirty windows across steps for block-path observe

Adds a persistent per-bin coarse max grid (w_cmax), raised atomically in the apply kernel, plus per-observation-buffer dirty rectangles. A new carry observe kernel loads the carried max grid instead of rebuilding it from the full LDS heightmap, and rewrites only the dirty region of the float heightmap observation. The aim is to cut the heightmap reload, plane max reduction and full observation write on each step. In exchange the apply path gains atomics and dirty bookkeeping, and correctness now depends on keeping cached state consistent across resets and buffer reuse.

```diff
diff --git a/include/irbpp.h b/include/irbpp.h
--- a/include/irbpp.h
+++ b/include/irbpp.h
@@ -60,6 +60,7 @@
 #define IRBPP_TUNE_WG128 2097152
 #define IRBPP_TUNE_RECT 4194304
 #define IRBPP_TUNE_NO_SPECIALISED 1024
+#define IRBPP_TUNE_STAGE_TILE 8388608
 
 typedef struct {
     double*  reward_dev;
diff --git a/irbpp_amd/_lib.py b/irbpp_amd/_lib.py
--- a/irbpp_amd/_lib.py
+++ b/irbpp_amd/_lib.py
@@ -23,7 +23,7 @@
 TUNE_TRACE_CPW64, TUNE_TRACE_CPW32, TUNE_TRACE_CPW16, TUNE_INLINE_POLYGON, TUNE_NO_HEAVY_FIRST = 32, 64, 128, 256, 512
 TUNE_NO_SPECIALISED, TUNE_FUSED_APPLY, TUNE_SPLIT_APPLY, TUNE_BLOCK_EMIT, TUNE_WAVE_EMIT = 1024, 2048, 4096, 8192, 16384
 TUNE_GRAPH, TUNE_WG512, TUNE_NO_WG512, TUNE_TRACE_REFILL, TUNE_NO_MIXED_PATH = 32768, 65536, 131072, 262144, 524288
-TUNE_CHAIN, TUNE_WG128, TUNE_RECT = 1048576, 2097152, 4194304
+TUNE_CHAIN, TUNE_WG128, TUNE_RECT, TUNE_STAGE_TILE = 1048576, 2097152, 4194304, 8388608
 
 
 class IrbppReplayView(C.Structure):
diff --git a/irbpp_amd/build.py b/irbpp_amd/build.py
--- a/irbpp_amd/build.py
+++ b/irbpp_amd/build.py
@@ -7,7 +7,7 @@
 PKG_DIR = os.path.dirname(os.path.abspath(__file__))
 CSRC = os.path.join(PKG_DIR, "csrc")
 LIB_PATH = os.path.join(PKG_DIR, "libirbpp_hip.so")
-SOURCES = ["irbpp_capi.hip", "irbpp_kernels.hip", "irbpp_wide.hip", "irbpp_replay.hip", "irbpp_metrics.hip", "irbpp_metrics.h", "irbpp_device.h", "contours_device.h", "irbpp_itemgen.h",
+SOURCES = ["irbpp_capi.hip", "irbpp_kernels.hip", "irbpp_wide.hip", "irbpp_replay.hip", "irbpp_metrics.hip", "irbpp_metrics.h", "irbpp_device.h", "irbpp_carry.h", "contours_device.h", "irbpp_itemgen.h",
            os.path.join("..", "..", "include", "irbpp.h")]
 HIPCC_FLAGS = ["--offload-arch=gfx950", "-O3", "-std=c++17", "-ffp-contract=off", "-fno-honor-nans",
                "-shared", "-fPIC", "-Wno-unused-value"]
diff --git a/irbpp_amd/csrc/irbpp_capi.hip b/irbpp_amd/csrc/irbpp_capi.hip
--- a/irbpp_amd/csrc/irbpp_capi.hip
+++ b/irbpp_amd/csrc/irbpp_capi.hip
@@ -44,6 +44,7 @@
     irbpp_episode_window window{};
     int32_t* heur_cells = nullptr;
     bool grids_current = false;
+    bool cmax_valid = false;
 };
 
 #define HIP_TRY(expr)                                   \
@@ -90,11 +91,11 @@
     const void* kernels[] = {(const void*)irbpp_env_kernel_wide, (const void*)irbpp_env_kernel, (const void*)irbpp_env_kernel_box,
                              (const void*)irbpp_env_kernel_box8, (const void*)irbpp_env_kernel_generic,
                              (const void*)irbpp_env_kernel_generic8, (const void*)irbpp_env_kernel_mixed8, (const void*)irbpp_hull_kernel,
-                             (const void*)irbpp_env_kernel_chain, (const void*)irbpp_wide_kernel,
+                             (const void*)irbpp_env_kernel_chain, (const void*)irbpp_wide_kernel, (const void*)irbpp_env_kernel_carry,
 #if !defined(IRBPP_NO_SPEC)
                              (const void*)irbpp_env_kernel_s1, (const void*)irbpp_env_kernel_s2, (const void*)irbpp_env_kernel_s3,
                              (const void*)irbpp_env_kernel_s4, (const void*)irbpp_env_kernel_s5, (const void*)irbpp_emit_kernel_s5,
-                             (const void*)irbpp_env_kernel_chain_s1, (const void*)wg128::irbpp_env_kernel_s1_w128,
+                             (const void*)irbpp_env_kernel_chain_s1, (const void*)irbpp_env_kernel_carry_s1, (const void*)wg128::irbpp_env_kernel_s1_w128,
                              (const void*)irbpp_emit_kernel_s1, (const void*)irbpp_emit_kernel_s2,
                              (const void*)irbpp_emit_kernel_s3, (const void*)irbpp_emit_kernel_s4,
                              (const void*)irbpp_emit_wave_kernel_s1, (const void*)irbpp_emit_wave_kernel_s2, (const void*)irbpp_emit_wave_kernel_s5,
@@ -418,6 +419,12 @@
         if (env->P.lds_bytes_full > 160 * 1024) return IRBPP_ERR_ARG;
         if (raise_lds_limits() != IRBPP_OK) return IRBPP_ERR_HIP;
     }
+    if (block_b > 0 && !mixed && env->P.K == 1 && !(env->cfg.tuning & IRBPP_TUNE_STAGE_TILE)) {
+        rc = dev_alloc(env, &env->S.w_cmax, (size_t)env->P.N * env->P.AC);
+        if (rc == IRBPP_OK) rc = dev_alloc(env, &env->S.w_dirty, (size_t)DIRTY_SLOTS * env->P.N * 2);
+        if (rc != IRBPP_OK) return rc;
+        HIP_TRY(hipMemset(env->S.w_dirty, 0xFF, (size_t)DIRTY_SLOTS * env->P.N * sizeof(DirtyRec)));
+    }
     env->item_order = (!block_b || mixed) && !box && gcell.size() * sizeof(GCell) > (size_t)8 << 20 && env->P.N % NXCD == 0 &&
                       env->P.N >= 64 * NXCD && env->P.K == 1 && !(env->cfg.tuning & IRBPP_TUNE_NO_ITEM_ORDER);
     env->shapes_loaded = true;
@@ -580,12 +587,17 @@
         io.use_order = 1;
     }
     io.obs_rows = nullptr;
+    io.dirty_mask = 0;
+    io.dirty_slot = 0;
     const bool observes = mode == MODE_CANDS || ((mode == MODE_RESET || mode == MODE_STEP) && env->P.K == 1);
-    for (auto& rb : env->obs_buffers)
-        if (rb.first == io.obs) {
-            if (observes && !(mode == MODE_RESET && io.bin_list != nullptr)) io.obs_rows = rb.second;
+    for (size_t k = 0; k < env->obs_buffers.size(); ++k) {
+        auto& rb = env->obs_buffers[k];
+        if (rb.first != nullptr) io.dirty_mask |= 1 << k;
+        if (rb.first != nullptr && rb.first == io.obs) {
+            if (observes && !(mode == MODE_RESET && io.bin_list != nullptr)) { io.obs_rows = rb.second; io.dirty_slot = (int32_t)k + 1; }
             else hipMemsetAsync(rb.second, 0xFF, (size_t)env->P.N * sizeof(int32_t), st);
         }
+    }
     if (env->P.wide) {
         int wmode = mode;
         if (mode == MODE_STEP) {
@@ -614,7 +626,13 @@
         env_mode = MODE_OBSERVE;
     }
     if (!(env_mode == MODE_OBSERVE && env->P.K > 1)) {
-        const EnvKernel ek = pick_env_kernel(env);
+        EnvKernel ek = pick_env_kernel(env);
+        if (env_mode == MODE_OBSERVE && io.carry) {
+            ek = EnvKernel{irbpp_env_kernel_carry, "irbpp_env_kernel_carry"};
+#if !defined(IRBPP_NO_SPEC) && !defined(IRBPP_ABLATE)
+            if (pick_spec(env) == 1) ek = EnvKernel{irbpp_env_kernel_carry_s1, "irbpp_env_kernel_carry_s1"};
+#endif
+        }
         hipLaunchKernelGGL(ek.fn, dim3(n), dim3(ek.threads), env->P.lds_bytes, st, env->P, env->T, env->S, io, env_mode);
     }
     if (split) {
@@ -657,9 +675,21 @@
 }
 static bool graph_wanted(const irbpp_env* env, int) { return (env->cfg.tuning & IRBPP_TUNE_GRAPH) != 0; }
 
+static bool carry_launch(const irbpp_env* env, int mode, int grid, int key) {
+    if (env->S.w_cmax == nullptr || !env->cmax_valid || mode != MODE_STEP || grid != env->P.N) return false;
+    if (chain_launch(env, grid) || !(key != KEY_CAND || split_apply(env, grid))) return false;
+    const env_kernel_fn fn = pick_env_kernel(env).fn;
+    bool block_build = fn == irbpp_env_kernel;
+#if !defined(IRBPP_NO_SPEC) && !defined(IRBPP_ABLATE)
+    block_build = block_build || fn == irbpp_env_kernel_s1;
+#endif
+    return block_build;
+}
+
 static int launch_env(irbpp_env* env, StepIO io, int mode, void* stream, int grid = 0, int key = KEY_CAND) {
     if (grid <= 0) grid = env->P.N;
     if (key == KEY_HEUR && grid != env->P.N) return IRBPP_ERR_ARG;
+    io.carry = carry_launch(env, mode, grid, key) ? 1 : 0;
     io.phase_cycles = env->phase_cycles;
     hipStream_t st = (hipStream_t)stream;
     size_t pairs = env->timing.size() / 2;
@@ -728,6 +758,8 @@
     if (hipGetLastError() != hipSuccess) return IRBPP_ERR_HIP;
     if (io.bin_list == nullptr && mode != MODE_POSSIBLE)
         env->grids_current = mode == MODE_CANDS || env->P.K == 1;
+    if (env->S.w_cmax != nullptr && io.bin_list == nullptr && grid == env->P.N && (mode == MODE_RESET || mode == MODE_STEP))
+        env->cmax_valid = true;
     return IRBPP_OK;
 }
 
@@ -876,7 +908,7 @@
     for (auto& rb : env->obs_buffers)
         if (rb.first == nullptr && rows == nullptr) { rows = rb.second; rb.first = obs_dev; }
     if (rows == nullptr) {
-        if (env->obs_buffers.size() >= 8) return IRBPP_ERR_ARG;
+        if (env->obs_buffers.size() >= (size_t)DIRTY_SLOTS) return IRBPP_ERR_ARG;
         int rc = dev_alloc(env, &rows, (size_t)env->P.N);
         if (rc != IRBPP_OK) return rc;
         env->obs_buffers.emplace_back(obs_dev, rows);
@@ -965,6 +997,9 @@
                            (hipStream_t)stream));
     HIP_TRY(hipMemsetAsync(env->S.w_valid, 0, (size_t)env->P.N * env->P.R * env->P.vrow * sizeof(uint32_t), (hipStream_t)stream));
     env->grids_current = false;
+    env->cmax_valid = false;
+    if (env->S.w_dirty != nullptr)
+        HIP_TRY(hipMemsetAsync(env->S.w_dirty, 0xFF, (size_t)DIRTY_SLOTS * env->P.N * sizeof(DirtyRec), (hipStream_t)stream));
     return IRBPP_OK;
 }
 
diff --git a/irbpp_amd/csrc/irbpp_carry.h b/irbpp_amd/csrc/irbpp_carry.h
--- /dev/null
+++ b/irbpp_amd/csrc/irbpp_carry.h
@@ -0,0 +1,61 @@
+#pragma once
+#include <stdint.h>
+
+#ifndef IRBPP_CARRY_FN
+#define IRBPP_CARRY_FN __host__ __device__ __forceinline__
+#endif
+
+namespace irbpp {
+
+IRBPP_CARRY_FN long long cmax_key(double h) {
+    union { double d; long long i; } u;
+    u.d = h;
+    return u.i;
+}
+IRBPP_CARRY_FN double cmax_value(long long key) {
+    union { double d; long long i; } u;
+    u.i = key;
+    return u.d;
+}
+IRBPP_CARRY_FN double cmax_raise(double entry, double h) {
+    const long long a = cmax_key(entry), b = cmax_key(h);
+    return cmax_value(a > b ? a : b);
+}
+
+constexpr uint32_t DIRTY_ALL = 0xFFFFFFFFu;
+constexpr uint32_t DIRTY_NONE = 0x0000FFFFu;
+constexpr int DIRTY_SLOTS = 8;
+struct DirtyRec { uint32_t a, b; };
+
+IRBPP_CARRY_FN uint32_t dirty_window(int r0, int c0, int r1, int c1) {
+    if (r0 < 0 || c0 < 0 || r1 > 254 || c1 > 254) return DIRTY_ALL;
+    if (r0 > r1 || c0 > c1) return DIRTY_NONE;
+    return (uint32_t)r0 | ((uint32_t)c0 << 8) | ((uint32_t)r1 << 16) | ((uint32_t)c1 << 24);
+}
+IRBPP_CARRY_FN int dirty_r0(uint32_t w) { return (int)(w & 255u); }
+IRBPP_CARRY_FN int dirty_c0(uint32_t w) { return (int)((w >> 8) & 255u); }
+IRBPP_CARRY_FN int dirty_r1(uint32_t w) { return (int)((w >> 16) & 255u); }
+IRBPP_CARRY_FN int dirty_c1(uint32_t w) { return (int)(w >> 24); }
+IRBPP_CARRY_FN bool dirty_inside(uint32_t x, uint32_t y) {
+    return dirty_r0(x) >= dirty_r0(y) && dirty_c0(x) >= dirty_c0(y) && dirty_r1(x) <= dirty_r1(y) && dirty_c1(x) <= dirty_c1(y);
+}
+IRBPP_CARRY_FN uint32_t dirty_box(uint32_t x, uint32_t y) {
+    const int r0 = dirty_r0(x) < dirty_r0(y) ? dirty_r0(x) : dirty_r0(y), c0 = dirty_c0(x) < dirty_c0(y) ? dirty_c0(x) : dirty_c0(y);
+    const int r1 = dirty_r1(x) > dirty_r1(y) ? dirty_r1(x) : dirty_r1(y), c1 = dirty_c1(x) > dirty_c1(y) ? dirty_c1(x) : dirty_c1(y);
+    return dirty_window(r0, c0, r1, c1);
+}
+IRBPP_CARRY_FN DirtyRec dirty_add(DirtyRec d, uint32_t w) {
+    if (d.a == DIRTY_ALL || w == DIRTY_NONE) return d;
+    if (w == DIRTY_ALL) { d.a = DIRTY_ALL; d.b = DIRTY_ALL; return d; }
+    if (d.a == DIRTY_NONE) { d.a = w; d.b = DIRTY_NONE; return d; }
+    if (dirty_inside(w, d.a)) return d;
+    if (d.b == DIRTY_NONE || d.b == DIRTY_ALL) { d.b = w; return d; }
+    if (dirty_inside(w, d.b)) return d;
+    d.a = dirty_box(d.a, d.b);
+    d.b = w;
+    return d;
+}
+IRBPP_CARRY_FN DirtyRec dirty_none() { DirtyRec d; d.a = DIRTY_NONE; d.b = DIRTY_NONE; return d; }
+IRBPP_CARRY_FN DirtyRec dirty_all() { DirtyRec d; d.a = DIRTY_ALL; d.b = DIRTY_ALL; return d; }
+
+}
diff --git a/irbpp_amd/csrc/irbpp_device.h b/irbpp_amd/csrc/irbpp_device.h
--- a/irbpp_amd/csrc/irbpp_device.h
+++ b/irbpp_amd/csrc/irbpp_device.h
@@ -1,6 +1,8 @@
 #pragma once
 #include <hip/hip_runtime.h>
 #include <stdint.h>
+
+#include "irbpp_carry.h"
 
 namespace irbpp {
 
@@ -94,6 +96,8 @@
     int32_t* w_nround;
     int32_t* w_heavy;
     int32_t* w_total;
+    double* w_cmax;
+    uint32_t* w_dirty;
 };
 
 struct Params {
@@ -292,6 +296,9 @@
     int32_t heavy_turn;
     int32_t n_slots;
     int32_t fixed_slot;
-};
-
-}
+    int32_t carry;
+    int32_t dirty_mask;
+    int32_t dirty_slot;
+};
+
+}
diff --git a/irbpp_amd/csrc/irbpp_kernels.hip b/irbpp_amd/csrc/irbpp_kernels.hip
--- a/irbpp_amd/csrc/irbpp_kernels.hip
+++ b/irbpp_amd/csrc/irbpp_kernels.hip
@@ -708,7 +708,7 @@
 }
 
 #endif
-template <int PATH>
+template <int PATH, bool CARRY = false>
 __device__ inline int overlap_test(const Params& P, const Tables& T, const State& S, const StepIO& io,
                                    const Lds& L, int b, int item, bool debug_out, double* zdst, bool sr_staged, bool dense) {
     const bool use_block = PATH == PATH_BLOCK || PATH == PATH_MIXED || (PATH == PATH_ANY && P.block_b > 0);
@@ -738,11 +738,16 @@
     for (int rep = 0; rep < IRBPP_REPS(6); ++rep) {
         if (rep) __syncthreads();
         const int planes = P.pp * P.pp, mq = P.block_b / P.step;
+        double* gcm = nullptr;
+        if constexpr (PATH == PATH_BLOCK || PATH == PATH_ANY) gcm = S.w_cmax != nullptr ? S.w_cmax + (size_t)b * AC : nullptr;
+        if constexpr (!CARRY) {
 #pragma unroll 1
         for (int t = tid; t < AC; t += BLOCK) {
             double m = L.hm[t];
             for (int pl = 1; pl < planes; ++pl) m = fmax(m, L.hm[pl * P.PL + t]);
             L.c2[t] = m;
+            if (gcm != nullptr) gcm[t] = m;
+        }
         }
         __syncthreads();
         if (rep == 0 && item >= 0) {
@@ -1112,20 +1117,61 @@
 template <int IPT>
 __device__ inline void split_handover(const Params& P, const State& S, const Lds& L, int b, int slot, int item, int nvalid);
 
-template <int PATH, bool CHAIN = false>
+template <int PATH, bool CHAIN = false, bool CARRY = false>
 __device__ inline void observe_location(const Params& P, const Tables& T, const State& S, const StepIO& io,
                                         const Lds& L, int b, int item, float* obs, bool debug_out, bool sr_staged,
-                                        unsigned char* chain_lds = nullptr) {
+                                        unsigned char* chain_lds = nullptr, bool hm_rewritten = false) {
     item = __builtin_amdgcn_readfirstlane(item);
     const int tid = threadIdx.x;
     const int R = P.R, AC = P.AC, Ax = P.Ax, Ay = P.Ay;
     const int X = fdiv(tid, Ay, P.mg_ay), Y = tid - X * Ay;
-    const int nvalid = IRBPP_HERE overlap_test<PATH>(P, T, S, io, L, b, item, debug_out, S.w_posz + (size_t)b * R * AC, sr_staged, false);
+    const int nvalid = IRBPP_HERE overlap_test<PATH, CARRY>(P, T, S, io, L, b, item, debug_out, S.w_posz + (size_t)b * R * AC, sr_staged, false);
     if (debug_out) return;
     if (tid < 9) obs[5 * P.S + tid] = tid == 0 ? (float)item : 0.0f;
+    constexpr bool CAN_CARRY = PATH == PATH_BLOCK || PATH == PATH_ANY;
+    bool tracked = false;
+    if constexpr (CAN_CARRY) tracked = S.w_dirty != nullptr && io.dirty_slot > 0 && io.obs_rows != nullptr;
+    if constexpr (CARRY) {
+        const double* const ghm = S.hm + (size_t)b * P.Hc;
+        float* const ohm = obs + 5 * P.S + 9;
+        DirtyRec d = dirty_all();
+        if (tracked) {
+            const int prev_rows = io.obs_rows[b];
+            d = ((const DirtyRec*)S.w_dirty)[(size_t)(io.dirty_slot - 1) * P.N + b];
+            if (prev_rows < 0) d = dirty_all();
+        }
+        if (d.a == DIRTY_ALL) {
+#pragma unroll 4
+            for (int i = tid; i < P.Hc; i += BLOCK) ohm[i] = (float)ghm[i];
+        } else {
+            const int tr = tid >> 4, tc = tid & 15;
+#pragma unroll 1
+            for (int k = 0; k < 2; ++k) {
+                const uint32_t w = k == 0 ? d.a : d.b;
+                if (w == DIRTY_NONE || w == DIRTY_ALL) continue;
+                const int r1 = min(dirty_r1(w), P.Hx - 1), c1 = min(dirty_c1(w), P.Hy - 1);
+#pragma unroll 1
+                for (int r = dirty_r0(w) + tr; r <= r1; r += BLOCK / 16)
+#pragma unroll 1
+                    for (int c = dirty_c0(w) + tc; c <= c1; c += 16) ohm[r * P.Hy + c] = (float)ghm[r * P.Hy + c];
+            }
+        }
+    } else {
     for (int rep = 0; rep < IRBPP_REPS(8); ++rep)
     for (TileWalk w = IRBPP_HERE tile_walk_begin(P, tid); w.lin < P.Hc; tile_walk_next(w)) obs[5 * P.S + 9 + w.lin] = (float)L.hm[tile_walk_index(P, w)];
+    }
     __syncthreads();
+    if constexpr (CAN_CARRY) {
+        if (S.w_dirty != nullptr && tid == 0 && (tracked || hm_rewritten)) {
+            DirtyRec* const recs = (DirtyRec*)S.w_dirty;
+#pragma unroll 1
+            for (int k = 0; k < DIRTY_SLOTS; ++k) {
+                if (!((io.dirty_mask >> k) & 1)) continue;
+                if (tracked && k == io.dirty_slot - 1) recs[(size_t)k * P.N + b] = dirty_none();
+                else if (hm_rewritten) recs[(size_t)k * P.N + b] = dirty_all();
+            }
+        }
+    }
     stamp(io, b, 2);
 
     if (io.phase_cycles && tid == 0)
@@ -2227,7 +2273,7 @@
 }
 
 #endif
-template <int PATH, int SPEC, bool FUSED, bool CHAIN = false>
+template <int PATH, int SPEC, bool FUSED, bool CHAIN = false, bool CARRY = false>
 __device__ __forceinline__ void env_transition(const Params& P_run, const Tables& T, const State& S, const StepIO& io,
                                                const int mode, unsigned char* smem);
 
@@ -2256,6 +2302,14 @@
         env_transition<PATH, SPEC, true, true>(P, T, S, io, mode, smem);                                               \
     }
 IRBPP_ENV_KERNEL_CHAIN(irbpp_env_kernel_chain, PATH_ANY, 0)
+#define IRBPP_ENV_KERNEL_CARRY(NAME, SPEC)                                                                              \
+    extern "C" __global__ void __launch_bounds__(BLOCK) IRBPP_CAPPED                                                   \
+    NAME(const Params P, const Tables T, const State S, const StepIO io, const int mode) {                             \
+        extern __shared__ __attribute__((aligned(16))) unsigned char smem[];                                           \
+        if (mode != MODE_OBSERVE) return;                                \
+        env_transition<PATH_BLOCK, SPEC, false, false, true>(P, T, S, io, MODE_OBSERVE, smem);                         \
+    }
+IRBPP_ENV_KERNEL_CARRY(irbpp_env_kernel_carry, 0)
 #ifndef IRBPP_NO_SPEC
 IRBPP_ENV_KERNEL(irbpp_env_kernel_s1, PATH_BLOCK, 1, IRBPP_CAPPED)
 IRBPP_ENV_KERNEL(irbpp_env_kernel_s2, PATH_BOX, 2, IRBPP_CAPPED)
@@ -2263,6 +2317,7 @@
 IRBPP_ENV_KERNEL(irbpp_env_kernel_s4, PATH_GENERIC, 4, )
 IRBPP_ENV_KERNEL(irbpp_env_kernel_s5, PATH_MIXED, 5, IRBPP_CAPPED)
 IRBPP_ENV_KERNEL_CHAIN(irbpp_env_kernel_chain_s1, PATH_BLOCK, 1)
+IRBPP_ENV_KERNEL_CARRY(irbpp_env_kernel_carry_s1, 1)
 #endif
 
 #elif IRBPP_PASS == 3
@@ -2285,7 +2340,7 @@
 #endif
 #endif
 
-template <int PATH, int SPEC, bool FUSED, bool CHAIN>
+template <int PATH, int SPEC, bool FUSED, bool CHAIN, bool CARRY>
 __device__ __forceinline__ void env_transition(const Params& P_run, const Tables& T, const State& S, const StepIO& io,
                                                const int mode, unsigned char* smem) {
     if constexpr (!FUSED) { if (mode == MODE_STEP) return; }
@@ -2319,7 +2374,12 @@
         st_cursor = ps0->cursor;
         st_trow = ps0->traj_row;
     }
-    if (mode == MODE_RESET) {
+    static_assert(!CARRY || (PATH == PATH_BLOCK && !CHAIN && !FUSED), "the carried form is the block path's observation");
+    if constexpr (CARRY) {
+        const double* const gcm = S.w_cmax + (size_t)b * P.AC;
+#pragma unroll 1
+        for (int t = tid; t < P.AC; t += BLOCK) L.c2[t] = gcm[t];
+    } else if (mode == MODE_RESET) {
         for (int i = tid; i < P.tile_words; i += BLOCK) L.hm[i] = 0.0;
         for (int i = tid; i < P.Hc; i += BLOCK) ghm[i] = 0.0;
     } else {
@@ -2568,7 +2628,8 @@
             for (int i = tid; i < P.Hc; i += BLOCK) obs[P.K + i] = (float)L.hm[tile_of_linear(P, i)];
         }
     }
-    if (do_observe) IRBPP_HERE observe_location<PATH, CHAIN>(P, T, S, io, L, b, obs_item, obs, debug_out, sr_staged, smem + P.lds_bytes);
+    if (do_observe) IRBPP_HERE observe_location<PATH, CHAIN, CARRY>(P, T, S, io, L, b, obs_item, obs, debug_out, sr_staged, smem + P.lds_bytes,
+                                                                    mode == MODE_RESET || mode == MODE_STEP);
 }
 
 #if IRBPP_PASS == 1
@@ -2673,6 +2734,7 @@
 #define IRBPP_SRD(FIELD) __hiloint2double(IRBPP_SRW(offsetof(ShapeRot, FIELD) / 4 + 1), IRBPP_SRW(offsetof(ShapeRot, FIELD) / 4))
     const int s_ax = IRBPP_SRI(ax), s_ay = IRBPP_SRI(ay), s_nb = IRBPP_SRI(nb), s_ob = IRBPP_SRI(ob), s_has_out = IRBPP_SRI(has_out);
     const int s_ot = IRBPP_SRI(ot);
+    const int s_fx = IRBPP_SRI(fx), s_fy = IRBPP_SRI(fy);
     const double ext_x = IRBPP_SRD(ext_x), ext_y = IRBPP_SRD(ext_y), ext_z = IRBPP_SRD(ext_z);
     bool ok = item0 >= 0 && nvalid0 > 0 && rot < P.R;
     if (ok) {
@@ -2696,6 +2758,13 @@
     Cell tc0 = {};
     if (lane < s_nt) tc0 = tcells[lane];
     const int row0 = lx * P.step, col0 = ly * P.step;
+    const bool carried = S.w_dirty != nullptr;
+    DirtyRec drec[DIRTY_SLOTS];
+    if (carried) {
+#pragma unroll
+        for (int k = 0; k < DIRTY_SLOTS; ++k)
+            if ((io.dirty_mask >> k) & 1) drec[k] = ((const DirtyRec*)S.w_dirty)[(size_t)k * P.N + b];
+    }
     double h0 = 0.0;
     const int i0 = (row0 + (tc0.ij & 0xFFFF)) * P.Hy + col0 + (tc0.ij >> 16);
     if (lane < s_nt) h0 = ghm[i0];
@@ -2718,7 +2787,16 @@
         if (round6_scaled(top - P.ibin_z) > 0.0) ok = false;
     }
     if (ok) {
-        if (lane < s_nt) ghm[i0] = fmax(h0, tc0.v + z);
+        long long* const gcm = S.w_cmax != nullptr ? (long long*)(S.w_cmax + (size_t)b * P.AC) : nullptr;
+        auto raise_cmax = [&](int ij, double h) {
+            const int ax = fdiv(row0 + (ij & 0xFFFF), P.step, P.mg_step), ay = fdiv(col0 + (ij >> 16), P.step, P.mg_step);
+            __hip_atomic_fetch_max(gcm + ax * P.Ay + ay, cmax_key(h), __ATOMIC_RELAXED, __HIP_MEMORY_SCOPE_AGENT);
+        };
+        if (lane < s_nt) {
+            const double h = fmax(h0, tc0.v + z);
+            ghm[i0] = h;
+            if (gcm != nullptr) raise_cmax(tc0.ij, h);
+        }
         for (int e0 = 64; e0 < s_nt; e0 += 4 * 64) {
             Cell tc[4];
             int ix[4];
@@ -2735,10 +2813,22 @@
             }
 #pragma unroll
             for (int u = 0; u < 4; ++u)
-                if (e0 + u * 64 + lane < s_nt) ghm[ix[u]] = fmax(hv[u], tc[u].v + z);
+                if (e0 + u * 64 + lane < s_nt) {
+                    const double h = fmax(hv[u], tc[u].v + z);
+                    ghm[ix[u]] = h;
+                    if (gcm != nullptr) raise_cmax(tc[u].ij, h);
+                }
         }
     } else {
         for (int i = lane; i < P.Hc; i += 64) ghm[i] = 0.0;
+        if (S.w_cmax != nullptr)
+            for (int i = lane; i < P.AC; i += 64) S.w_cmax[(size_t)b * P.AC + i] = 0.0;
+    }
+    if (carried && lane == 0) {
+        const uint32_t win = ok ? dirty_window(row0, col0, row0 + s_fx - 1, col0 + s_fy - 1) : DIRTY_ALL;
+#pragma unroll
+        for (int k = 0; k < DIRTY_SLOTS; ++k)
+            if ((io.dirty_mask >> k) & 1) ((DirtyRec*)S.w_dirty)[(size_t)k * P.N + b] = dirty_add(drec[k], win);
     }
     if (lane == 0) {
         BinState* ps = S.bs + b;
```

Result: slower. 62.34 million (-2.3%).
